# twesterhout/distributed-matvec

Measured on AMD Instinct MI355X. Metric: matvecs/sec, higher is better.
Workload: dtype f64; 1 GPU; heisenberg_chain_32: y <- H x, 601080390 basis states, 9927521280 off-diagonal non-zeros, f64 vectors, sigma/x/y resident in HBM; partitions=1, partitioning=single, exchange=none, kernel=direct-pull+staged, x=u(hash(sigma, 42)) - 0.5, exchange_bytes_per_matvec=0

## Files before the change

distributed-matvec_amd/csrc/host.c:

```c
#define _GNU_SOURCE
#include <math.h>
#include <pthread.h>
#include <stdarg.h>
#include <stdio.h>
#include <stdlib.h>
#include <string.h>

#include "../../include/ls_amd.h"
#include "../../include/ls_chpl.h"
#include "../../include/ls_hs.h"
#include "lsk.h"

static __thread char g_last_error[1024] = "";
static ls_amd_error_handler g_handler = NULL;

static int set_error(char const *fmt, ...) {
    va_list ap;
    va_start(ap, fmt);
    vsnprintf(g_last_error, sizeof(g_last_error), fmt, ap);
    va_end(ap);
    return -1;
}
static int dev_error(void) { return set_error("%s", lsk_last_error()); }
int ls_amd_internal_error(char const *fmt, ...) {
// ... 1427 lines not shown
        DEV(lsk_malloc(&p, sizeof(lsk_group) * (e->n_groups > 0 ? e->n_groups : 1)));
        DEV(lsk_h2d(p, e->groups, sizeof(lsk_group) * e->n_groups));
        e->d_groups = (lsk_group *)p;
        DEV(lsk_malloc(&p, sizeof(lsk_term) * (e->n_off > 0 ? e->n_off : 1)));
        DEV(lsk_h2d(p, e->off, sizeof(lsk_term) * e->n_off));
        e->d_off = (lsk_term *)p;
        DEV(lsk_malloc(&p, sizeof(lsk_term) * (e->n_diag > 0 ? e->n_diag : 1)));
        DEV(lsk_h2d(p, e->diag, sizeof(lsk_term) * e->n_diag));
        e->d_diag = (lsk_term *)p;
    }
    out->n_diag = e->n_diag;
    out->n_off = e->n_off;
    out->n_groups = e->n_groups;
    out->is_real = e->is_real;
    out->diag = e->d_diag;
    out->off = e->d_off;
    out->groups = e->d_groups;
    out->runs = e->runs;
    out->uni = e->is_real && e->n_groups > 0;
    out->uni_v = e->n_groups > 0 ? e->groups[0].v_re : 0.0;
    for (int g = 0; g < e->n_groups && out->uni; ++g)
        if (e->groups[g].fast != LSK_GROUP_EXCHANGE || e->groups[g].v_im != 0.0 || e->groups[g].v_re != out->uni_v ||
            __builtin_popcountll(e->groups[g].x) != 2)
            out->uni = 0;
    return 0;
}

static int operator_device(ls_hs_operator const *op, lsk_operator *out) {
    pthread_mutex_lock(&g_device_tables_lock);
    int const rc = operator_device_unlocked(op, out);
    pthread_mutex_unlock(&g_device_tables_lock);
    return rc;
}
static int basis_device(ls_hs_basis const *b, lsk_basis *out) {
    pthread_mutex_lock(&g_device_tables_lock);
    int const rc = basis_device_unlocked(b, out);
    pthread_mutex_unlock(&g_device_tables_lock);
    return rc;
}

static ls_chpl_kernels g_kernels;
void ls_hs_internal_set_chpl_kernels(ls_chpl_kernels const *kernels) { g_kernels = *kernels; }
ls_chpl_kernels const *ls_hs_internal_get_chpl_kernels(void) { return &g_kernels; }

void ls_chpl_init_kernels(void) {
    ls_chpl_kernels k;
    k.enumerate_states = (void *)ls_chpl_enumerate_representatives;
    k.operator_apply_off_diag = (void *)ls_chpl_operator_apply_off_diag;
    k.operator_apply_diag = (void *)ls_chpl_operator_apply_diag;
    k.matrix_vector_product = (void *)ls_chpl_matrix_vector_product;
    ls_hs_internal_set_chpl_kernels(&k);
}

static int g_initialised = 0;
void ls_chpl_init(void) {
    if (g_initialised) return;
    if (lsk_device_count() < 1) { halt_with("ls_chpl_init: no HIP device available"); return; }
    char const *dev = getenv("LS_AMD_DEVICE");
    if (dev && lsk_set_device(atoi(dev)) != 0) { halt_with("ls_chpl_init: %s", lsk_last_error()); return; }
    ls_chpl_init_kernels();
    g_initialised = 1;
}
void ls_chpl_finalize(void) {
    if (g_d_binom) { lsk_free(g_d_binom); g_d_binom = NULL; }
    g_initialised = 0;
}

void ls_hs_basis_build(ls_hs_basis *basis) {
    if (basis->representatives.elts) return;
    typedef void (*enum_fn)(ls_hs_basis *, uint64_t, uint64_t, chpl_external_array *);
    enum_fn f = (enum_fn)g_kernels.enumerate_states;
    if (!f) { ls_chpl_init_kernels(); f = (enum_fn)g_kernels.enumerate_states; }
    chpl_external_array arr = {NULL, 0, NULL};
    f(basis, ls_hs_min_state_estimate(basis), ls_hs_max_state_estimate(basis), &arr);
    if (!arr.elts) return;
    basis_drop_device_caches(basis);
    basis->representatives = arr;
    BEXT(basis)->owns_representatives = 1;
}

typedef struct part_state {
    int64_t count;
    uint64_t const *d_reps;
    lsk_index index;
    uint32_t *d_table;
    lsk_rankdir *d_dir;
    double *d_norms;
    int rounds;
    int64_t *send_counts;
    lsk_round_layout *d_layouts;
    int64_t max_send_bytes;
    int64_t *h_beta_off, *h_val_off;
    uint32_t *d_wtab;
    int64_t *wtab_first;
    uint32_t *d_ttab;
    int64_t *ttab_first;
    uint32_t *d_soff;
    uint32_t *h_soff;
    struct ls_amd_gtab *scatter_gt;
} part_state;

#ifndef LS_AMD_PULL_VALUES_DEFAULT
#define LS_AMD_PULL_VALUES_DEFAULT 0
#endif
enum { FAMILY_DIRECT_PUSH = 0, FAMILY_DIRECT_PULL = 1, FAMILY_TILE = 2, FAMILY_TILE_PULL = 3,
       FAMILY_REPL_DIRECT = 4, FAMILY_REPL_TILE = 5 };

struct ls_amd_plan {
    ls_hs_operator const *op;
    lsk_operator dop;
    lsk_basis dbs;
    int cplx, P, me, n_local;
    int family;
    part_state *parts;
    void *d_send;
    int64_t send_capacity;
    unsigned long long *d_cursors;
    unsigned long long *d_counts;
    int *d_err;
    int64_t nnz;
    lsk_gdir gd;
    lsk_rankdir *d_gdir;
    lsk_part_ctx *d_part_ctx;
    int part_ctx_any;
    int key_bytes;
    int streams, st_S, st_tile_rows, st_wpb, st_rounds;
    int stream_gkeys;
    void **d_send_parts;
    lsk_wsrc *d_wsrcs;
    lsk_index gindex;
    uint32_t *d_gtable;
    int64_t *d_row_gidx;
    double *d_norms_global;
    lsk_tilemap tilemap;
    void *d_tilemap;
    int has_pairs;
    int has_push_staged;
    int one_rank_full_basis;
    lsk_pairplan pairs;
    void *d_pair_recs, *d_rank_low, *d_pair_binom, *d_states32, *d_pair_rows, *d_pair_sites;
    int global_index;
    int has_hubbard;
    lsk_hubbard hubbard;
    void *d_hub[6];
    int has_chain;
    int chain_cached;
    void *d_chain_cache;
    int chain_wide;
    uint64_t *d_chain_rec;
    void *d_chain_wave;
    int chain_row_bytes;
    int chain_headed;
    int chain_headers_apply;
    int chain_paired;
    void *d_tilemap_pair, *d_chain_hdr_b;
    lsk_tilemap tilemap_pair;
    int64_t chain_pair_d, chain_pair_a0, chain_pair_rows;
    double chain_v[2];
    int64_t chain_row0;
    void *d_htab;
    uint32_t *d_slot_of;
    int htab_bits;
    void *d_xs;
    int pull_halo;
    int idx_mode;
    struct ls_amd_gtab *gtab;
    uint64_t *d_vtab;
    int64_t row_g0;
    lsk_pullbuf pbuf;
    int64_t split_rows;
    int64_t split_active;
    int slot_cache, slot_cache_valid;
    int64_t slot_cache_bytes;
    lsk_pullbuf blk_pbuf;
    int64_t blk_rows;
    lsk_tilemap blk_tilemap;
    void *d_blk_tilemap;
    void *d_blk_cols;
    void *d_gram_work;
    size_t gram_work_bytes;
    void *d_series_work;
    int series_cols;
    double *d_series_dots;
    void const *y_checked[2];
    int leaves_basis;
    int t_capacity, t_count;
    void **t_start, **t_stop;
    int st_capacity, st_count;
    void **st_start, **st_stop;
    unsigned char *st_stage;
    double st_ms[8];
    int64_t st_calls[8];
    int64_t st_matvecs;
};

typedef struct ls_amd_gtab {
    uint64_t const *reps;
    uint8_t const *masks;
    int64_t n;
    int P, L;
    lsk_gtab tab;
    uint64_t *d_entries;
    uint32_t *d_perm;
    int64_t counts[LSK_MAX_PARTS], max_count;
    uint64_t finger[8];
    int refs;
    struct ls_amd_gtab *next;
} ls_amd_gtab;
static ls_amd_gtab *g_gtabs = NULL;
static lsk_gtab no_gtab(void) { lsk_gtab t; memset(&t, 0, sizeof(t)); return t; }
static pthread_mutex_t g_gtab_lock = PTHREAD_MUTEX_INITIALIZER;

static void gtab_free(ls_amd_gtab *t) {
    if (t->d_entries) lsk_free(t->d_entries);
    if (t->d_perm) lsk_free(t->d_perm);
    free(t);
}
void ls_amd_internal_gtab_release(ls_amd_gtab *t) {
    if (!t) return;
    pthread_mutex_lock(&g_gtab_lock);
    if (--t->refs == 0) {
        for (ls_amd_gtab **q = &g_gtabs; *q; q = &(*q)->next)
            if (*q == t) { *q = t->next; break; }
        gtab_free(t);
    }
    pthread_mutex_unlock(&g_gtab_lock);
}
static int gtab_build(ls_amd_gtab *t, void *stream) {
    int64_t const n = t->n;
    int const P = t->P;
    if (t->masks) {
        DEV(lsk_mask_counts(n, t->masks, P, t->counts, stream));
        for (int p = 0; p < P; ++p) if (t->counts[p] > t->max_count) t->max_count = t->counts[p];
        if ((int64_t)P * t->max_count >= 0xffffffffLL) return set_error("indexed pull: more than 2^32 - 1 slots");
        void *pos[LSK_MAX_PARTS];
        memset(pos, 0, sizeof(pos));
        void *perm64 = NULL, *perm32 = NULL;
        int rc = lsk_malloc(&perm64, 8 * (size_t)(n > 0 ? n : 1));
        for (int p = 0; p < P && rc == 0; ++p) {
            rc = lsk_malloc(&pos[p], 8 * (size_t)(t->counts[p] > 0 ? t->counts[p] : 1));
            if (rc == 0) rc = lsk_iota_i64(t->counts[p], (int64_t)p * t->max_count, (int64_t *)pos[p], stream);
        }
        if (rc == 0) rc = lsk_hashed_to_block(n, t->masks, P, 8, (void const *const *)pos, perm64, stream);
        if (rc == 0) rc = lsk_malloc(&perm32, 4 * (size_t)(n > 0 ? n : 1));
        if (rc == 0) rc = lsk_narrow_i32(n, (int64_t const *)perm64, (int32_t *)perm32, stream);
        if (rc == 0) rc = lsk_sync(stream);
        for (int p = 0; p < P; ++p) if (pos[p]) lsk_free(pos[p]);
        if (perm64) lsk_free(perm64);
        if (rc != 0) { if (perm32) lsk_free(perm32); return dev_error(); }
        t->d_perm = (uint32_t *)perm32;
    } else {
        t->counts[0] = n;
        t->max_count = n;
    }
    int64_t const max_bytes = (int64_t)1 << 40;
    int const bb = lsk_gtab_bits(t->L, n, max_bytes);
    if (bb < 0) return set_error("indexed pull: no admissible index-table size for %lld keys of %d bits", (long long)n, t->L);
    t->tab.L = t->L; t->tab.bbits = bb; t->tab.tbits = t->L - bb;
    void *p, *flag;
    DEV(lsk_malloc(&p, (size_t)16 << bb));
    t->d_entries = (uint64_t *)p;
    t->tab.entries = t->d_entries;
    DEV(lsk_malloc(&flag, sizeof(int)));
    int zero = 0, bad = 0;
    int rc = lsk_h2d(flag, &zero, sizeof(int)) || lsk_gtab_build(t->tab, t->d_entries, n, t->reps, t->d_perm, (int *)flag, stream) ||
             lsk_sync(stream) || lsk_d2h(&bad, flag, sizeof(int));
    lsk_free(flag);
    if (rc) return dev_error();
    if (bad) return set_error("indexed pull: a key could not be placed within 255 buckets of its home");
    return 0;
}
static int gtab_fingerprint(uint64_t const *d_reps, int64_t n, void *stream, uint64_t *f) {
    memset(f, 0, 8 * sizeof(uint64_t));
    if (n <= 0) return 0;
    DEV(lsk_sync(stream));
    for (int k = 0; k < 8; ++k) DEV(lsk_d2h(&f[k], d_reps + (n - 1) * k / 7, sizeof(uint64_t)));
    return 0;
}
int ls_amd_internal_gtab_acquire(ls_amd_gtab **out, int L, uint64_t const *d_reps, int64_t n, uint8_t const *d_masks, int P,
                                 void *stream) {
    *out = NULL;
    uint64_t finger[8];
    if (gtab_fingerprint(d_reps, n, stream, finger) != 0) return -1;
    pthread_mutex_lock(&g_gtab_lock);
    for (ls_amd_gtab *t = g_gtabs; t; t = t->next)
        if (t->reps == d_reps && t->n == n && t->masks == d_masks && t->P == P && t->L == L && memcmp(t->finger, finger, sizeof(finger)) == 0) {
            ++t->refs;
            pthread_mutex_unlock(&g_gtab_lock);
            *out = t;
            return 0;
        }
    ls_amd_gtab *t = (ls_amd_gtab *)calloc(1, sizeof(*t));
    t->reps = d_reps; t->n = n; t->masks = d_masks; t->P = P; t->L = L;
    memcpy(t->finger, finger, sizeof(finger));
    if (gtab_build(t, stream) != 0) {
        gtab_free(t);
        pthread_mutex_unlock(&g_gtab_lock);
        return -1;
    }
    t->refs = 1;
    t->next = g_gtabs;
    g_gtabs = t;
    pthread_mutex_unlock(&g_gtab_lock);
    *out = t;
    return 0;
}
uint32_t const *ls_amd_internal_gtab_perm(ls_amd_gtab const *t) { return t->d_perm; }
int64_t ls_amd_internal_gtab_max_count(ls_amd_gtab const *t) { return t->max_count; }
int64_t const *ls_amd_internal_gtab_counts(ls_amd_gtab const *t) { return t->counts; }
int64_t ls_amd_internal_gtab_bytes(ls_amd_gtab const *t) { return (int64_t)16 << t->tab.bbits; }
// ... 179 lines not shown
            pl->pbuf.slots = (uint32_t *)a; pl->pbuf.rows = (uint8_t *)b; pl->pbuf.coefs = (double *)c; pl->pbuf.counts = (uint32_t *)d;
            pl->pbuf.cap = cap;
            pl->pbuf.row0 = 0;
            pl->split_rows = streams * 64 < pl->parts[0].count ? streams * 64 : pl->parts[0].count;
            return pl->split_rows;
        }
        if (a) lsk_free(a);
        if (b) lsk_free(b);
        if (c) lsk_free(c);
        if (d) lsk_free(d);
        streams = (streams / 2) & ~(int64_t)3;
    }
    return 0;
}
int64_t ls_amd_internal_plan_split_rows(ls_amd_plan const *pl) { return pl->split_rows; }
static int64_t split_rows_now(ls_amd_plan const *pl) {
    if (pl->slot_cache || pl->split_active <= 0 || pl->split_active >= pl->split_rows) return pl->split_rows;
    return pl->split_active;
}
void ls_amd_internal_plan_split_set_active(ls_amd_plan *pl, int64_t rows) {
    pl->split_active = rows <= 0 ? 0 : (rows & ~(int64_t)255);
    if (rows > 0 && pl->split_active < 256) pl->split_active = 256;
}
int64_t ls_amd_internal_plan_split_active(ls_amd_plan const *pl) { return split_rows_now(pl); }
int ls_amd_internal_plan_slot_cached(ls_amd_plan const *pl) { return pl->slot_cache != 0; }
static int64_t split_enable_exact(ls_amd_plan *pl, int64_t max_bytes) {
    split_free(pl);
    part_state *ps = &pl->parts[0];
    int64_t const streams_all = (ps->count + 63) / 64;
    int const nc = lsk_pullbuf_coef_doubles(pl->dop, pl->dbs);
    int64_t const per_packet = 4 + 1 + 8 * nc;
    void *offs = NULL;
    if (lsk_malloc(&offs, 8 * (size_t)(((streams_all + 3) & ~(int64_t)3) + 1)) != 0) return 0;
    if (lsk_tile_pull_stream_offsets(pl->dop, pl->dbs, 0, ps->count, ps->d_reps, (int64_t *)offs, NULL) != 0) { lsk_free(offs); return -1; }
    int64_t streams = streams_all;
    for (;;) {
        int64_t total = 0;
        if (lsk_d2h(&total, (char *)offs + 8 * (size_t)streams, 8) != 0) { lsk_free(offs); return -1; }
        if (max_bytes > 0 && total * per_packet + 12 * streams + 8 > max_bytes) {
            int64_t lo = 0, hi = streams / 4;
            while (hi - lo > 1) {
                int64_t const mid = lo + (hi - lo) / 2;
                int64_t t = 0;
                if (lsk_d2h(&t, (char *)offs + 8 * (size_t)(4 * mid), 8) != 0) { lsk_free(offs); return -1; }
                if (t * per_packet + 12 * 4 * mid + 8 <= max_bytes) lo = mid; else hi = mid;
            }
            streams = 4 * lo;
            if (streams <= 0) { lsk_free(offs); return 0; }
            if (lsk_d2h(&total, (char *)offs + 8 * (size_t)streams, 8) != 0) { lsk_free(offs); return -1; }
        }
        if (total >= ((int64_t)1 << 40)) { lsk_free(offs); return 0; }
        void *a = NULL, *b = NULL, *c = NULL, *d = NULL;
        if (lsk_malloc(&a, (size_t)(4 * total + 4)) == 0 && lsk_malloc(&b, (size_t)(total + 4)) == 0 &&
            (nc == 0 || lsk_malloc(&c, (size_t)(8 * nc * total + 8)) == 0) && lsk_malloc(&d, (size_t)(4 * ((streams + 3) & ~(int64_t)3))) == 0) {
            pl->pbuf.slots = (uint32_t *)a; pl->pbuf.rows = (uint8_t *)b; pl->pbuf.coefs = (double *)c; pl->pbuf.counts = (uint32_t *)d;
            pl->pbuf.offs = (int64_t const *)offs;
            pl->pbuf.cap = lsk_pullbuf_cap(pl->dop);
            pl->pbuf.row0 = 0;
            pl->split_rows = streams * 64 < ps->count ? streams * 64 : ps->count;
            pl->slot_cache_bytes = total * per_packet + 12 * streams + 8;
            return pl->split_rows;
        }
        if (a) lsk_free(a);
        if (b) lsk_free(b);
        if (c) lsk_free(c);
        if (d) lsk_free(d);
        max_bytes = (total * per_packet + 12 * streams + 8) / 4 * 3;
        if (max_bytes < ((int64_t)1 << 20)) { lsk_free(offs); return 0; }
    }
}
int64_t ls_amd_plan_cache_slots(ls_amd_plan *pl, int64_t max_bytes) {
    if (!pl || !pl->idx_mode || pl->dbs.proj != LSK_PROJ_FULL || pl->parts[0].count <= 0 ||
        (pl->family != FAMILY_TILE_PULL && pl->family != FAMILY_REPL_TILE)) return 0;
    int64_t const rows = split_enable_exact(pl, max_bytes);
    if (rows < 0) return dev_error();
    if (rows == 0) return 0;
    pl->slot_cache = 1;
    pl->slot_cache_valid = 0;
    return rows;
}
int ls_amd_plan_slot_cache_rows(ls_amd_plan const *pl, int64_t *rows, int64_t *bytes) {
    if (rows) *rows = pl->slot_cache ? pl->split_rows : 0;
    if (bytes) *bytes = pl->slot_cache ? pl->slot_cache_bytes : 0;
    return 0;
}

static int packets_wave_rings(void) {
    char const *e = getenv("LS_AMD_PACKETS");
    return !(e && strcmp(e, "block") == 0);
}
static int64_t rows_per_round_default(void) {
    char const *e = getenv("LS_AMD_ROWS_PER_ROUND");
    if (e) { long long v = atoll(e); if (v > 0) return (int64_t)v; }
    return (int64_t)1 << 24;
}

static int build_search_index(part_state *ps, int number_sites, void *stream) {
    if (ps->count >= 0xffffffffLL) return set_error("partitions with >= 2^32 states are not supported");
    int bits = 0;
    while ((1LL << (bits + 1)) <= ps->count) ++bits;
    bits -= 3;
    if (bits < 1) bits = 1;
    if (bits > 26) bits = 26;
    if (bits > number_sites) bits = number_sites;
    int shift = number_sites - bits;
    int64_t nbuckets = (int64_t)1 << bits;
    void *p;
    DEV(lsk_malloc(&p, 4 * (size_t)(nbuckets + 2)));
    ps->d_table = (uint32_t *)p;
    DEV(lsk_build_table(ps->count, ps->d_reps, shift, nbuckets, ps->d_table, stream));
    ps->index.kind = LSK_INDEX_SEARCH;
    ps->index.shift = shift;
    ps->index.table = ps->d_table;
    return 0;
}

static int upload(void **slot, void const *host, size_t bytes) {
    DEV(lsk_malloc(slot, bytes ? bytes : 8));
    DEV(lsk_h2d(*slot, host, bytes));
    return 0;
}

typedef struct { uint64_t *e; int64_t n, cap; } tile_list;
static void tile_push(tile_list *l, int64_t row, int64_t cnt) {
    if (l->n == l->cap) { l->cap = l->cap ? 2 * l->cap : 1024; l->e = (uint64_t *)realloc(l->e, sizeof(uint64_t) * (size_t)l->cap); }
    l->e[l->n++] = (uint64_t)row | ((uint64_t)cnt << 48);
}
static int tilemap_host(int64_t n, int TILE, int64_t chunk, uint64_t **out, int64_t *slots_out) {
    tile_list lists[8];
    memset(lists, 0, sizeof(lists));
    int64_t const tiles = (n + TILE - 1) / TILE;
    if (chunk > 0) {
        for (int64_t q = 0; q < tiles; ++q)
            tile_push(&lists[(q / chunk) % 8], q * TILE, n - q * TILE < TILE ? n - q * TILE : TILE);
    } else
        for (int k = 0; k < 8; ++k)
            for (int64_t q = tiles * k / 8; q < tiles * (k + 1) / 8; ++q)
                tile_push(&lists[k], q * TILE, n - q * TILE < TILE ? n - q * TILE : TILE);
    int64_t slots = 0, total = 0;
    for (int k = 0; k < 8; ++k) if (lists[k].n > slots) slots = lists[k].n;
    uint64_t *flat = (uint64_t *)calloc((size_t)(8 * slots > 0 ? 8 * slots : 1), sizeof(uint64_t));
    for (int k = 0; k < 8; ++k) {
        for (int64_t q = 0; q < lists[k].n; ++q) { flat[k * slots + q] = lists[k].e[q]; total += (int64_t)(lists[k].e[q] >> 48); }
        free(lists[k].e);
    }
    if (total != n) {
        free(flat);
        return set_error("internal error: tile map covers %lld of %lld rows", (long long)total, (long long)n);
    }
    *out = flat;
    *slots_out = slots;
    return 0;
}
static int chain_pair_range(int L, int k, int64_t *a0, int64_t *a1, int64_t *d) {
    if (L < 14 || L > 32 || k < 1 || k > L - 1) return 0;
    uint64_t C[33][33];
    memset(C, 0, sizeof(C));
    for (int n = 0; n <= 32; ++n) { C[n][0] = 1; for (int j = 1; j <= n; ++j) C[n][j] = C[n - 1][j - 1] + (j <= n - 1 ? C[n - 1][j] : 0); }
    int64_t const r01 = (int64_t)C[L - 2][k], r10 = (int64_t)C[L - 1][k];
    *d = r10 - r01;
    *a0 = (r01 + 511) & ~(int64_t)511;
    *a1 = r10 & ~(int64_t)511;
    return *a1 > *a0;
}
#define CHAIN_TILE_PLAIN 0x8000
static int tilemap_deal(tile_list const *all, int64_t chunk, uint64_t **out, int64_t *slots_out) {
    int64_t const tiles = all->n;
    int64_t per[8] = {0, 0, 0, 0, 0, 0, 0, 0}, slots = 0;
    if (chunk > 0) for (int64_t q = 0; q < tiles; ++q) ++per[(q / chunk) % 8];
    else for (int k = 0; k < 8; ++k) per[k] = tiles * (k + 1) / 8 - tiles * k / 8;
    for (int k = 0; k < 8; ++k) if (per[k] > slots) slots = per[k];
    uint64_t *flat = (uint64_t *)calloc((size_t)(8 * slots > 0 ? 8 * slots : 1), sizeof(uint64_t));
    if (!flat) return set_error("out of memory");
    int64_t fill[8] = {0, 0, 0, 0, 0, 0, 0, 0};
    int k0 = 0;
    for (int64_t q = 0; q < tiles; ++q) {
        int k;
        if (chunk > 0) k = (int)((q / chunk) % 8);
        else { while (q >= tiles * (k0 + 1) / 8) ++k0; k = k0; }
        flat[k * slots + fill[k]++] = all->e[q];
    }
    *out = flat;
    *slots_out = slots;
    return 0;
}
static int tilemap_paired_host(int64_t n, int TILE, int64_t chunk, int64_t a0, int64_t a1, int64_t d, uint64_t **rest, int64_t *rest_slots,
                               uint64_t **pairs, int64_t *pair_slots) {
    tile_list all[2];
    memset(all, 0, sizeof(all));
    int64_t const piece[3][2] = {{0, a0}, {a1, a0 + d}, {a1 + d, n}};
    int64_t total = 0;
    for (int p = 0; p < 3; ++p)
        for (int64_t pos = piece[p][0]; pos < piece[p][1];) {
            int64_t end = (pos / TILE + 1) * TILE;
            if (pos & 63) end = (pos | 63) + 1;
            if (end > piece[p][1]) end = piece[p][1];
            int const plain = (pos & 63) != 0 || ((end & 63) != 0 && end != n);
            tile_push(&all[0], pos, (end - pos) | (plain ? CHAIN_TILE_PLAIN : 0));
            total += end - pos;
            pos = end;
        }
    for (int64_t i0 = a0; i0 < a1; i0 += 512) { tile_push(&all[1], i0, 1024); total += 1024; }
    int rc = total == n ? 0 : set_error("internal error: paired tile maps cover %lld of %lld rows", (long long)total, (long long)n);
    *rest = *pairs = NULL;
    if (!rc) rc = tilemap_deal(&all[0], chunk, rest, rest_slots);
    if (!rc) rc = tilemap_deal(&all[1], chunk, pairs, pair_slots);
    if (rc) { free(*rest); free(*pairs); *rest = *pairs = NULL; }
    free(all[0].e);
    free(all[1].e);
    return rc;
}
static int build_tilemap(ls_amd_plan *pl, int64_t n, int TILE) {
    uint64_t *flat = NULL;
    int64_t slots = 0;
    char const *e = getenv("LS_AMD_TILE_CHUNK");
    int64_t const chunk = e ? atoll(e) : (TILE >= 512 ? 256 : 0);
    if (tilemap_host(n, TILE, chunk > 0 ? chunk : 0, &flat, &slots) < 0) return -1;
    int const up = upload(&pl->d_tilemap, flat, sizeof(uint64_t) * (size_t)(8 * slots > 0 ? 8 * slots : 1));
    free(flat);
    if (up) return -1;
    pl->tilemap.entries = (uint64_t const *)pl->d_tilemap;
    pl->tilemap.slots_per_xcd = slots;
    return 0;
}
int ls_amd_test_corrupt_plan(ls_amd_plan *pl) {
    if (!pl) return 0;
    if (pl->family == FAMILY_TILE_PULL && pl->n_local == 1 && pl->parts[0].d_norms && pl->parts[0].count > 0) {
        double v = 0;
        double *p = pl->parts[0].d_norms + pl->parts[0].count / 2;
        if (lsk_device_sync() != 0 || lsk_d2h(&v, p, sizeof(v)) != 0) return 0;
        v *= 2.0;
        return lsk_h2d(p, &v, sizeof(v)) == 0;
    }
    if (!pl->d_tilemap || pl->tilemap.slots_per_xcd <= 0) return 0;
    uint64_t e = 0;
    if (lsk_device_sync() != 0 || lsk_d2h(&e, pl->d_tilemap, sizeof(e)) != 0) return 0;
    uint64_t const rows = e >> 48;
    if (rows < 2) return 0;
    e = (e & 0xffffffffffffULL) | ((rows - 1) << 48);
    if (lsk_h2d(pl->d_tilemap, &e, sizeof(e)) != 0) return 0;
    return 1;
}
int ls_amd_test_window_find(uint64_t const *reps, int n, uint64_t key) { return lsk_test_window_find(reps, n, key); }
int ls_amd_test_nw_find(uint64_t const *reps, int n, uint64_t key) { return lsk_test_nw_find(reps, n, key); }
int ls_amd_test_chain_near_table(int elem, int ldsp, int16_t *out) { return lsk_test_chain_near_table(elem, ldsp, out); }
uint64_t ls_amd_test_rep_trivial_dihedral(uint64_t a, int L, int inv, int reflect) { return lsk_test_rep_trivial_dihedral(a, L, inv, reflect); }
int ls_amd_bench_k4(int L, int inv, int reflect, int variant, int64_t n, uint64_t const *d_reps, uint64_t *d_out, void *stream) {
    if (lsk_bench_k4(L, inv, reflect, variant, n, d_reps, d_out, stream) != 0) { set_error("%s", lsk_last_error()); return -1; }
    return 0;
}
int64_t ls_amd_test_tilemap(int64_t n, int tile_rows, int64_t chunk, uint64_t **entries) {
    int64_t slots = 0;
    *entries = NULL;
    if (tilemap_host(n, tile_rows, chunk, entries, &slots) < 0) return -1;
    return slots;
}
int ls_amd_test_tilemap_paired(int L, int weight, int tile_rows, int64_t chunk, uint64_t **rest, uint64_t **pairs, int64_t *out) {
    int64_t a0, a1, d, n = 1;
    *rest = *pairs = NULL;
    if (!chain_pair_range(L, weight, &a0, &a1, &d)) return 0;
    for (int j = 1; j <= weight; ++j) n = n * (L - weight + j) / j;
    if (tilemap_paired_host(n, tile_rows, chunk, a0, a1, d, rest, &out[4], pairs, &out[5]) != 0) return -1;
    out[0] = n; out[1] = a0; out[2] = a1; out[3] = d;
    return 1;
}
void ls_amd_test_free(void *p) { free(p); }
int ls_amd_test_gtab_bits(int L, int64_t n) { return lsk_gtab_bits(L, n, (int64_t)1 << 40); }
int ls_amd_test_gtab_build(int L, int bbits, int64_t n, uint64_t const *reps, uint32_t const *payload, uint64_t **entries) {
    lsk_gtab t;
    t.entries = NULL; t.L = L; t.bbits = bbits; t.tbits = L - bbits;
    *entries = (uint64_t *)malloc(sizeof(uint64_t) * ((size_t)2 << bbits));
    if (lsk_test_gtab_build_host(t, *entries, n, reps, payload) != 0) { free(*entries); *entries = NULL; return -1; }
    return 0;
}
int64_t ls_amd_test_gtab_find(int L, int bbits, uint64_t const *entries, uint64_t key) {
    lsk_gtab t;
    t.entries = NULL; t.L = L; t.bbits = bbits; t.tbits = L - bbits;
    return lsk_test_gtab_find(t, entries, key);
}

static int push_staged_eligible(ls_amd_plan const *pl) {
    ls_hs_operator const *op = pl->op;
    struct ls_amd_operator_ext const *ext = OEXT(op);
    char const *e = getenv("LS_AMD_ROW_KERNEL");
    if (e && strcmp(e, "generic") == 0) return 0;
    if (NBITS(op->basis) > 64 || op->basis->spin_inversion != 0 || pl->dbs.proj != LSK_PROJ_NONE || !ext->is_real ||
        ext->runs.n_runs <= 0 || BEXT(op->basis)->hamming_weight < 0)
        return 0;
    for (int q = 0; q < ext->runs.n_runs; ++q) if (ext->runs.cnt[q] >> 16) return 0;
    return 1;
}
static int chain_eligible(ls_amd_plan const *pl) {
    ls_hs_operator const *op = pl->op;
    struct ls_amd_operator_ext const *ext = OEXT(op);
    char const *e = getenv("LS_AMD_ROW_KERNEL");
    if (e && (strcmp(e, "generic") == 0 || strcmp(e, "pairs") == 0 || strcmp(e, "pairrows") == 0 || strcmp(e, "pairsites") == 0)) return 0;
    int const L = NBITS(op->basis);
    int const inv = op->basis->spin_inversion != 0;
    if (inv && (pl->dbs.proj != LSK_PROJ_INVERSION || pl->family != FAMILY_DIRECT_PULL || (L & 1) || BEXT(op->basis)->hamming_weight != L / 2)) return 0;
    if (L > 64 || (!inv && pl->dbs.proj != LSK_PROJ_NONE) ||
        !ext->is_real || !ext->is_hermitian || ext->runs.n_runs <= 0 || ext->n_diag <= 0)
        return 0;
    int extra = 0;
    if (inv) for (int q = 0; q < ext->runs.n_runs; ++q) if (ext->runs.lo0[q] + ext->runs.cnt[q] - 1 == L - 2) extra = 1;
    if (ext->n_groups - ext->runs.n_run_groups + extra > 2) return 0;
    for (int g = ext->runs.n_run_groups; g < ext->n_groups; ++g) {
        lsk_group const *G = &ext->groups[g];
        if (G->fast != LSK_GROUP_EXCHANGE || G->v_im != 0.0 || __builtin_popcountll(G->x) != 2) return 0;
    }
    return 1;
}
static void chain_wave_tables(int low_site, uint16_t *U, uint16_t *Rg, int *class_off) {
    int pos[13];
    uint16_t rank_in[4096];
    memset(class_off, 0, sizeof(int) * 14);
    for (int w = 0; w < 4096; ++w) ++class_off[__builtin_popcount(w) + 1];
    for (int k = 0; k < 13; ++k) { class_off[k + 1] += class_off[k]; pos[k] = class_off[k]; }
    for (int w = 0; w < 4096; ++w) {
        int const k = __builtin_popcount(w);
        rank_in[w] = (uint16_t)(pos[k] - class_off[k]);
        U[pos[k]++] = (uint16_t)w;
    }
    for (int w = 0; w < 4096; ++w) Rg[w] = low_site >= 0 ? rank_in[w ^ (1 << low_site)] : 0;
}
int ls_amd_test_chain_wave_tables(int low_site, uint16_t *U, uint16_t *Rg, int *class_off) {
    if (low_site >= 12) return set_error("ls_amd_test_chain_wave_tables: the low site lies below bit 12");
    chain_wave_tables(low_site, U, Rg, class_off);
    return 0;
}
static int setup_chain_headers(ls_amd_plan *pl, lsk_index index, int64_t n, uint64_t const *d_reps, int nc, uint64_t xmask, void *stream) {
    int const L = NBITS(pl->op->basis);
    char const *e = getenv("LS_AMD_CHAIN_RECORDS");
    int headed = L >= 13 && L <= 32 && pl->dbs.proj == LSK_PROJ_NONE && pl->chain_row0 == 0 &&
                 pl->family == FAMILY_DIRECT_PULL && pl->dbs.hamming_weight >= 0 && nc <= 1;
    int lo = -1, hi = -1;
    if (headed && nc == 1) {
        lo = __builtin_ctzll(xmask);
        hi = 63 - __builtin_clzll(xmask);
        if (lo >= 12 || hi < 12) { headed = 0; lo = hi = -1; }
    }
    pl->chain_headers_apply = headed;
    if (e && atoi(e) != 0) { headed = 0; lo = hi = -1; }
    int const words = lsk_chain_words();
    int64_t const n_hdr = (n + 63) / 64;
    uint16_t U[4096], Rg[4096];
    int class_off[14];
    uint32_t *tab = (uint32_t *)malloc(sizeof(uint32_t) * (size_t)words);
    if (!tab) return set_error("out of memory");
    chain_wave_tables(headed ? lo : -1, U, Rg, class_off);
    for (int t = 0; t < words; ++t) tab[t] = (uint32_t)U[t] | ((uint32_t)Rg[U[t]] << 16) | (lo >= 0 ? (((uint32_t)U[t] >> lo) & 1u) << 31 : 0u);
    size_t const tab_bytes = sizeof(uint32_t) * (size_t)words, hdr_bytes = 8 * (size_t)n_hdr;
    void *q;
    if (lsk_malloc(&q, tab_bytes + hdr_bytes + 8) != 0) { free(tab); return 1; }
    unsigned long long plain = 0;
    unsigned long long *d_plain = (unsigned long long *)((char *)q + tab_bytes + hdr_bytes);
    int const rc = lsk_h2d(q, tab, tab_bytes) || lsk_h2d(d_plain, &plain, 8) ||
                   lsk_chain_headers(pl->dbs, index, n, d_reps, headed, hi, (char *)q + tab_bytes, d_plain, stream) || lsk_sync(stream) ||
                   lsk_d2h(&plain, d_plain, 8);
    free(tab);
    if (rc) { lsk_free(q); return dev_error(); }
    pl->d_chain_wave = q;
    pl->chain_headed = headed;
    int const rec = pl->cplx ? 4 + 4 * nc : 8;
    pl->chain_row_bytes = headed ? (int)((8 * (uint64_t)n_hdr + 64 * (uint64_t)rec * (uint64_t)plain + (uint64_t)n - 1) / (uint64_t)n) : rec;
    return 0;
}
static int setup_chain_pairs(ls_amd_plan *pl, lsk_index index, int64_t n, uint64_t const *d_reps, int hi, void *stream) {
    char const *e = getenv("LS_AMD_CHAIN_PAIRED");
    int const L = NBITS(pl->op->basis);
    if ((e && atoi(e) == 0) || !pl->chain_headers_apply || pl->cplx || !pl->d_chain_rec || pl->chain_cached > 1 || pl->chain_row0 != 0 ||
        pl->n_local != 1 || pl->family != FAMILY_DIRECT_PULL)
        return 0;
    int top = 0;
    for (int q = 0; q < pl->dop.runs.n_runs; ++q)
        if (pl->dop.runs.lo0[q] <= L - 2 && L - 2 < pl->dop.runs.lo0[q] + pl->dop.runs.cnt[q]) top = 1;
    int64_t a0, a1, d;
    if (!top || !chain_pair_range(L, pl->dbs.hamming_weight, &a0, &a1, &d) || a1 + d > n) return 0;
    uint64_t *rest = NULL, *pairs = NULL;
    int64_t rest_slots = 0, pair_slots = 0;
    char const *ce = getenv("LS_AMD_TILE_CHUNK");
    int64_t const chunk = ce ? atoll(ce) : 256;
    if (tilemap_paired_host(n, lsk_chain_tile_rows(0), chunk > 0 ? chunk : 0, a0, a1, d, &rest, &rest_slots, &pairs, &pair_slots) != 0) return -1;
    void *d_rest = NULL, *d_pairs = NULL, *d_hdr = NULL;
    int64_t const n_b = a1 - a0;
    unsigned long long plain = 0;
    int rc = lsk_malloc(&d_rest, sizeof(uint64_t) * (size_t)(8 * rest_slots > 0 ? 8 * rest_slots : 1)) ||
             lsk_malloc(&d_pairs, sizeof(uint64_t) * (size_t)(8 * pair_slots)) || lsk_malloc(&d_hdr, 8 * (size_t)(n_b / 64) + 8);
    if (!rc) {
        unsigned long long *d_plain = (unsigned long long *)((char *)d_hdr + 8 * (size_t)(n_b / 64));
        rc = lsk_h2d(d_rest, rest, sizeof(uint64_t) * (size_t)(8 * rest_slots)) || lsk_h2d(d_pairs, pairs, sizeof(uint64_t) * (size_t)(8 * pair_slots)) ||
             lsk_h2d(d_plain, &plain, 8) || lsk_chain_headers(pl->dbs, index, n_b, d_reps + a0 + d, pl->chain_headed, hi, d_hdr, d_plain, stream) ||
             lsk_sync(stream);
        if (rc) { free(rest); free(pairs); lsk_free(d_rest); lsk_free(d_pairs); lsk_free(d_hdr); return dev_error(); }
    }
    free(rest);
    free(pairs);
    if (rc) {
        if (d_rest) lsk_free(d_rest);
        if (d_pairs) lsk_free(d_pairs);
        if (d_hdr) lsk_free(d_hdr);
        return 0;
    }
    lsk_free(pl->d_tilemap);
    pl->d_tilemap = d_rest;
    pl->tilemap.entries = (uint64_t const *)d_rest;
    pl->tilemap.slots_per_xcd = rest_slots;
    pl->d_tilemap_pair = d_pairs;
    pl->tilemap_pair.entries = (uint64_t const *)d_pairs;
    pl->tilemap_pair.slots_per_xcd = pair_slots;
    pl->d_chain_hdr_b = d_hdr;
    pl->chain_pair_d = d;
    pl->chain_pair_a0 = a0;
    pl->chain_pair_rows = 2 * (a1 - a0);
    pl->chain_paired = 1;
    return 0;
}
static int setup_chain(ls_amd_plan *pl, lsk_index index, int64_t n, uint64_t const *d_reps, void *stream) {
    struct ls_amd_operator_ext const *ext = OEXT(pl->op);
    int nc = ext->n_groups - ext->runs.n_run_groups;
    int const Ls = NBITS(pl->op->basis);
    int const inv = pl->dbs.proj == LSK_PROJ_INVERSION;
    uint64_t const top = 1ULL << (Ls - 1);
    uint64_t cx[3];
    double cv[3];
    int k = 0;
    if (inv)
        for (int q = 0; q < pl->dop.runs.n_runs; ++q)
            if (pl->dop.runs.lo0[q] + pl->dop.runs.cnt[q] - 1 == Ls - 2) {
                cx[k] = 3ULL << (Ls - 2);
                cv[k++] = pl->dop.runs.v_re[q] * (double)pl->op->basis->spin_inversion;
                if (--pl->dop.runs.cnt[q] == 0) {
                    for (int r = q; r + 1 < pl->dop.runs.n_runs; ++r) {
                        pl->dop.runs.lo0[r] = pl->dop.runs.lo0[r + 1]; pl->dop.runs.cnt[r] = pl->dop.runs.cnt[r + 1];
                        pl->dop.runs.v_re[r] = pl->dop.runs.v_re[r + 1]; pl->dop.runs.v_im[r] = pl->dop.runs.v_im[r + 1];
                    }
                    --pl->dop.runs.n_runs;
                }
                break;
            }
    for (int g = ext->runs.n_run_groups; g < ext->n_groups && k < 3; ++g) {
        cx[k] = ext->groups[g].x;
        cv[k++] = ext->groups[g].v_re * ((inv && (ext->groups[g].x & top)) ? (double)pl->op->basis->spin_inversion : 1.0);
    }
    nc = k;
    if (nc > 2) return 0;
    char const *ew = getenv("LS_AMD_CHAIN_WIDE");
    pl->chain_wide = index.count >= 0xffffffffLL || (ew && atoi(ew) != 0 && NBITS(pl->op->basis) > 32);
    size_t const es = pl->chain_wide ? sizeof(uint64_t) : sizeof(uint32_t);
    if (nc > 0 && n > 0) {
        void *q;
        if (lsk_malloc(&q, es * (size_t)nc * (size_t)n) != 0) return 0;
        pl->d_chain_cache = q;
        int zero = 0, flag = 0;
        DEV(lsk_h2d(pl->d_err, &zero, sizeof(int)));
        for (int c = 0; c < nc; ++c)
            DEV(lsk_chain_cache(pl->dbs, index, n, d_reps, cx[c],
                                (char *)pl->d_chain_cache + es * (size_t)c * (size_t)n, pl->chain_wide, pl->d_err, stream));
        DEV(lsk_sync(stream));
        DEV(lsk_d2h(&flag, pl->d_err, sizeof(int)));
        DEV(lsk_h2d(pl->d_err, &zero, sizeof(int)));
        if (flag) {
            lsk_free(pl->d_chain_cache);
            pl->d_chain_cache = NULL;
            return 0;
        }
        pl->chain_cached = nc;
        pl->chain_v[0] = cv[0];
        pl->chain_v[1] = nc > 1 ? cv[1] : 0.0;
    }
    if (build_tilemap(pl, n, lsk_chain_tile_rows(pl->cplx)) != 0) return -1;
    if (!pl->cplx && NBITS(pl->op->basis) <= 32 && !pl->chain_wide && n > 0) {
        void *q;
        if (lsk_malloc(&q, sizeof(uint64_t) * (size_t)n) != 0) {
            if (pl->d_chain_cache) { lsk_free(pl->d_chain_cache); pl->d_chain_cache = NULL; }
            if (pl->d_tilemap) { lsk_free(pl->d_tilemap); pl->d_tilemap = NULL; memset(&pl->tilemap, 0, sizeof(pl->tilemap)); }
            pl->chain_cached = 0;
            return 0;
        }
        pl->d_chain_rec = (uint64_t *)q;
        DEV(lsk_chain_pack(n, d_reps, pl->chain_cached ? pl->d_chain_cache : NULL, (uint64_t *)q, stream));
        DEV(lsk_sync(stream));
        if (pl->chain_cached <= 1 && pl->d_chain_cache) { lsk_free(pl->d_chain_cache); pl->d_chain_cache = NULL; }
    }
    if (NBITS(pl->op->basis) <= 32 && !pl->chain_wide && n > 0) {
        int const rc = setup_chain_headers(pl, index, n, d_reps, pl->chain_cached, pl->chain_cached > 0 ? cx[0] : 0, stream);
        if (rc < 0) return -1;
        if (rc > 0) {
            if (pl->d_chain_rec) { lsk_free(pl->d_chain_rec); pl->d_chain_rec = NULL; }
            if (pl->d_chain_cache) { lsk_free(pl->d_chain_cache); pl->d_chain_cache = NULL; }
            if (pl->d_tilemap) { lsk_free(pl->d_tilemap); pl->d_tilemap = NULL; memset(&pl->tilemap, 0, sizeof(pl->tilemap)); }
            pl->chain_cached = 0;
            return 0;
        }
        if (setup_chain_pairs(pl, index, n, d_reps, pl->chain_cached > 0 ? 63 - __builtin_clzll(cx[0]) : -1, stream) != 0) return -1;
    }
    pl->has_chain = 1;
    return 0;
}

static int pair_cmp(void const *pa, void const *pb) {
    lsk_pair const *a = (lsk_pair const *)pa, *b = (lsk_pair const *)pb;
    int const ca = a->j < 11 ? 0 : (a->i < 11 ? 1 : 2), cb = b->j < 11 ? 0 : (b->i < 11 ? 1 : 2);
    if (ca != cb) return ca - cb;
    if (a->i != b->i) return (int)a->i - (int)b->i;
    return (int)a->j - (int)b->j;
}
static int setup_pairs(ls_amd_plan *pl, int64_t n, uint64_t const *d_reps, void *stream) {
    ls_hs_operator const *op = pl->op;
    struct ls_amd_operator_ext const *ext = OEXT(op);
    int const L = NBITS(op->basis), hw = BEXT(op->basis)->hamming_weight;
    char const *e = getenv("LS_AMD_ROW_KERNEL");
    if (e && strcmp(e, "generic") == 0) return 0;
    int const wide = L > 32;
    if (L > 64 || hw < 0 || hw + 2 > LSK_PAIR_KC || op->basis->spin_inversion != 0 || pl->dbs.proj != LSK_PROJ_NONE || !ext->is_real ||
        !ext->is_hermitian || ext->n_groups < 1 || ext->n_groups > LSK_MAX_PAIRS || n <= 0 || n >= 0xffffffffLL ||
        ext->n_diag <= 0)
        return 0;
    int const force_sites = e && strcmp(e, "pairsites") == 0;
    int const by_row = force_sites || (e && strcmp(e, "pairrows") == 0) || (!(e && strcmp(e, "pairs") == 0) && (11 * hw < 4 * L || 11 * (L - hw) < 4 * L));
    lsk_pair recs[LSK_MAX_PAIRS];
    memset(recs, 0, sizeof(recs));
    for (int g = 0; g < ext->n_groups; ++g) {
        lsk_group const *G = &ext->groups[g];
        if (G->fast != LSK_GROUP_EXCHANGE || G->v_im != 0.0 || __builtin_popcountll(G->x) != 2) return 0;
        recs[g].i = (uint8_t)__builtin_ctzll(G->x);
        recs[g].j = (uint8_t)(63 - __builtin_clzll(G->x));
        recs[g].v = G->v_re;
    }
    double dsum = 0.0;
    for (int t = 0; t < ext->n_diag; ++t) {
        lsk_term const *T = &ext->diag[t];
        if (T->m != 0 || T->r != 0 || T->v_im != 0.0) return 0;
        int g = 0;
        while (g < ext->n_groups && ext->groups[g].x != T->s) ++g;
        if (g == ext->n_groups) return 0;
        recs[g].vz += T->v_re;
        dsum += T->v_re;
    }
    qsort(recs, (size_t)ext->n_groups, sizeof(lsk_pair), pair_cmp);
    lsk_pairplan pp;
    memset(&pp, 0, sizeof(pp));
    for (int g = 0; g < ext->n_groups; ++g) {
        if (recs[g].j < 11) ++pp.n_near; else if (recs[g].i < 11) ++pp.n_str; else ++pp.n_high;
    }
    pp.dsum = dsum;
    uint16_t rank_low[2048];
    for (int w = 0; w < 2048; ++w) {
        uint64_t r = 0;
        int k = 0;
        for (int b = 0; b < 11; ++b) if ((w >> b) & 1) r += binom(b, ++k);
        rank_low[w] = (uint16_t)r;
    }
    int const nbits = wide ? 64 : 32;
    uint32_t bin[64 * LSK_PAIR_KC];
    for (int a = 0; a < nbits; ++a) for (int k = 0; k < LSK_PAIR_KC; ++k) bin[a * LSK_PAIR_KC + k] = (uint32_t)binom(a, k);
    void *q = NULL;
    if (!wide) {
        if (lsk_malloc(&q, 4 * (size_t)n) != 0) return 0;
        pl->d_states32 = q;
    }
    if (upload(&pl->d_pair_recs, recs, sizeof(lsk_pair) * (size_t)ext->n_groups) != 0 || upload(&pl->d_rank_low, rank_low, sizeof(rank_low)) != 0 ||
        upload(&pl->d_pair_binom, bin, sizeof(uint32_t) * (size_t)nbits * LSK_PAIR_KC) != 0)
        return -1;
    if (!wide) DEV(lsk_narrow_states(n, d_reps, (uint32_t *)pl->d_states32, stream));
    if (by_row) {
        lsk_pair_row rr[LSK_MAX_PAIRS];
// ... 922 lines not shown
    *d_norms = NULL;
    if (basis_device(op->basis, &dbs) != 0) return -1;
    int64_t const cnt = gt->counts[me];
    void *reps = NULL, *nrm = NULL;
    if (lsk_malloc(&reps, 8 * (size_t)(cnt > 0 ? cnt : 1)) != 0) return dev_error();
    if (lsk_malloc(&nrm, 8 * (size_t)(cnt > 0 ? cnt : 1)) != 0) { lsk_free(reps); return dev_error(); }
    int const rc = lsk_scatter_owned(gt->n, gt->d_perm, (int64_t)me * gt->max_count, cnt, gt->reps, (uint64_t *)reps, stream) ||
                   lsk_norms(dbs, cnt, (uint64_t const *)reps, (double *)nrm, stream) || lsk_sync(stream);
    lsk_free(reps);
    if (rc) { lsk_free(nrm); return dev_error(); }
    *d_norms = (double *)nrm;
    return 0;
}

int ls_amd_matvec_replicated(ls_amd_plan *pl, void const *d_x_global, void *d_y_local, void *stream) {
    part_state *ps = &pl->parts[0];
    int slot;
    ls_amd_internal_count_matvec(pl);
    if (pl->family == FAMILY_REPL_DIRECT) {
        int const st = stage_begin(pl, ST_ROWS, stream);
        slot = timing_begin(pl, stream);
        if (pl->has_chain)
            DEV(lsk_chain(pl->dop, pl->dbs, pl->gindex, pl->cplx, pl->chain_wide, pl->d_chain_rec != NULL, pl->tilemap, ps->count,
                          pl->d_chain_rec ? pl->d_chain_rec : ps->d_reps, pl->chain_row0, pl->gindex.count, d_x_global, d_y_local,
                          pl->chain_cached, pl->d_chain_cache, pl->chain_v[0], pl->chain_v[1], pl->d_chain_wave, stream));
        else
            DEV(lsk_direct_gx(pl->dop, pl->dbs, pl->gindex, pl->cplx, pl->tilemap, ps->d_reps, pl->d_row_gidx, d_x_global,
                          d_y_local, pl->d_err, stream));
        timing_end(pl, slot, stream);
        stage_end(pl, st, stream);
        return 0;
    }
    if (pl->family == FAMILY_REPL_TILE && pl->idx_mode) {
        lsk_pullidx ix;
        ix.tab = pl->gtab->tab;
        ix.perm = pl->gtab->d_perm;
        ix.row_g0 = pl->row_g0;
        ix.vtab = NULL;
        int const st = stage_begin(pl, ST_ROWS, stream);
        slot = timing_begin(pl, stream);
        DEV(lsk_tile_pull_idx(pl->dop, pl->dbs, pl->cplx, 0, ps->count, ps->d_reps, ps->d_norms, ix, pl->gindex.reps,
                              pl->gindex.count, d_x_global, pl->pull_halo, d_y_local, pl->d_err, stream));
        timing_end(pl, slot, stream);
        stage_end(pl, st, stream);
        return 0;
    }
    if (pl->family == FAMILY_REPL_TILE) {
        void const *xg;
        if (prescaled_x(pl, pl->gindex.count, pl->gindex.reps, d_x_global, pl->d_norms_global, &xg, stream) != 0) return -1;
        int const st = stage_begin(pl, ST_ROWS, stream);
        slot = timing_begin(pl, stream);
        DEV(lsk_tile_pull(pl->dop, pl->dbs, pl->gindex, pl->cplx, 0, ps->count, ps->d_reps, ps->d_norms,
                          pl->d_norms_global, pl->d_row_gidx, xg, pl->htab_bits, pl->gindex.reps, pl->gindex.count,
                          pl->d_xs ? pl->d_xs : d_x_global, pl->pull_halo, d_x_global, d_y_local, pl->d_err, stream));
        timing_end(pl, slot, stream);
        stage_end(pl, st, stream);
        return 0;
    }
    return set_error("ls_amd_matvec_replicated: not a replicated-x plan");
}
int ls_amd_internal_plan_reach(ls_amd_plan *pl, int shift, int64_t row0, int64_t halo, int64_t nwords, uint32_t *h_bitmap, void *stream) {
    if (pl->family != FAMILY_REPL_DIRECT || pl->dbs.proj != LSK_PROJ_NONE) return 1;
    part_state *ps = &pl->parts[0];
    int64_t const n_global = pl->gindex.count;
    if (((n_global - 1) >> shift) / 32 >= nwords) return set_error("internal error: reach bitmap too small");
    memset(h_bitmap, 0, 4 * (size_t)nwords);
    if (ps->count <= 0) return 0;
    void *d = NULL;
    DEV(lsk_malloc(&d, 4 * (size_t)nwords));
    if (lsk_memset_async(d, 0, 4 * (size_t)nwords, stream) != 0 ||
        lsk_reach_blocks(pl->dop, pl->gindex, ps->count, ps->d_reps, shift, (uint32_t *)d, stream) != 0 || lsk_sync(stream) != 0 ||
        lsk_d2h(h_bitmap, d, 4 * (size_t)nwords) != 0) { lsk_free(d); return dev_error(); }
    lsk_free(d);
    int64_t g0 = row0, g1 = g0 + ps->count;
    g0 = g0 > halo ? g0 - halo : 0;
    g1 = g1 + halo < n_global ? g1 + halo : n_global;
    for (int64_t b = g0 >> shift; b <= (g1 - 1) >> shift; ++b) h_bitmap[b >> 5] |= 1u << (b & 31);
    return 0;
}

int ls_amd_internal_repl_split_begin(ls_amd_plan *pl, void *stream) {
    if (pl->family != FAMILY_REPL_TILE || !pl->idx_mode || pl->split_rows <= 0) return 0;
    if (pl->slot_cache && pl->slot_cache_valid) return 0;
    part_state *ps = &pl->parts[0];
    lsk_pullidx ix;
    ix.tab = pl->gtab->tab;
    ix.perm = pl->gtab->d_perm;
    ix.row_g0 = pl->row_g0;
    ix.vtab = NULL;
    int const st = stage_begin(pl, ST_GENERATE, stream);
    int const slot = timing_begin(pl, stream);
    DEV(lsk_tile_pull_resolve(pl->dop, pl->dbs, 0, split_rows_now(pl), ps->d_reps, ps->d_norms, ix, pl->gindex.reps, pl->gindex.count,
                              pl->pull_halo, pl->pbuf, pl->d_err, stream));
    pl->slot_cache_valid = pl->slot_cache;
    timing_end(pl, slot, stream);
    stage_end(pl, st, stream);
    return 0;
}
int ls_amd_internal_repl_split_rows(ls_amd_plan *pl, void const *d_x_global, void *d_y_local, int64_t row0, int64_t row1, int count, void *stream) {
    if (pl->family != FAMILY_REPL_TILE || !pl->idx_mode || pl->split_rows <= 0) return set_error("internal error: not a split plan");
    part_state *ps = &pl->parts[0];
    if (row1 > ps->count) row1 = ps->count;
    if (row0 < 0 || (row0 & 255) != 0 || row0 > row1) return set_error("internal error: bad row range of the split matvec");
    if (count) ls_amd_internal_count_matvec(pl);
    lsk_pullidx ix;
    ix.tab = pl->gtab->tab;
    ix.perm = pl->gtab->d_perm;
    ix.row_g0 = pl->row_g0;
    ix.vtab = NULL;
    int64_t const S = split_rows_now(pl);
    int const st = stage_begin(pl, ST_ROWS, stream);
    if (row0 < S) {
        int const slot = pl->slot_cache ? timing_begin(pl, stream) : -1;
        DEV(lsk_tile_pull_gather(pl->dop, pl->dbs, pl->cplx, row0, row1 < S ? row1 : S, ps->d_reps, ps->d_norms, ix, d_x_global, pl->pbuf, d_y_local,
                                 stream));
        if (slot >= 0) timing_end(pl, slot, stream);
    }
    if (row1 > S)
        DEV(lsk_tile_pull_idx(pl->dop, pl->dbs, pl->cplx, row0 > S ? row0 : S, row1, ps->d_reps, ps->d_norms, ix, pl->gindex.reps,
                              pl->gindex.count, d_x_global, pl->pull_halo, d_y_local, pl->d_err, stream));
    stage_end(pl, st, stream);
    return 0;
}
int ls_amd_internal_repl_split_finish(ls_amd_plan *pl, void const *d_x_global, void *d_y_local, void *stream) {
    if (pl->family != FAMILY_REPL_TILE || !pl->idx_mode || pl->split_rows <= 0) return ls_amd_matvec_replicated(pl, d_x_global, d_y_local, stream);
    return ls_amd_internal_repl_split_rows(pl, d_x_global, d_y_local, 0, pl->parts[0].count, 1, stream);
}
char const *ls_amd_plan_kernel_name(ls_amd_plan const *pl) {
    switch (pl->family) {
    case FAMILY_DIRECT_PUSH: return pl->has_push_staged ? "direct-push+staged" : "direct-push";
    case FAMILY_DIRECT_PULL:
        if (pl->has_hubbard) return "direct-pull+hubbard";
        return pl->has_chain ? "direct-pull+staged" : pl->has_pairs ? (pl->pairs.sites ? "direct-pull+pairsites" : pl->pairs.rows ? "direct-pull+pairrows" : "direct-pull+pairs") : "direct-pull";
    case FAMILY_TILE_PULL: return pl->idx_mode ? (pl->slot_cache ? "tile-pull+indexed+cached" : (pl->d_vtab ? "tile-pull+values" : "tile-pull+indexed")) : "tile-pull";
    case FAMILY_REPL_DIRECT:
        return pl->has_chain ? "replicated-direct-pull+staged" : "replicated-direct-pull";
    case FAMILY_REPL_TILE: return pl->idx_mode ? (pl->slot_cache ? "replicated-tile-pull+indexed+cached" : "replicated-tile-pull+indexed") : "replicated-tile-pull";
    default: return pl->streams ? "tile+streams" : (pl->has_push_staged ? "tile(one rank: push+staged)" : "tile");
    }
}
int ls_amd_plan_packet_bytes(ls_amd_plan const *pl) { return pl->key_bytes + (pl->cplx ? 16 : 8); }
int ls_amd_plan_row_bytes(ls_amd_plan const *pl) {
    if (pl->has_hubbard) return 0;
    if (pl->has_pairs) return pl->pairs.wide ? 8 : 4;
    if (pl->has_chain) {
        if (pl->d_chain_wave) return pl->chain_row_bytes;
        int const narrow = NBITS(pl->op->basis) <= 32 && !pl->chain_wide;
        return (narrow ? 4 : 8) + pl->chain_cached * (pl->chain_wide ? 8 : 4);
    }
    if (pl->family == FAMILY_TILE_PULL || pl->family == FAMILY_REPL_TILE) return 16;
    return 8;
}
int64_t ls_amd_plan_chain_paired_rows(ls_amd_plan const *pl) {
    return pl->has_chain && pl->chain_paired ? pl->chain_pair_rows : 0;
}
int64_t ls_amd_plan_nnz(ls_amd_plan const *pl) { return pl->nnz; }
int ls_amd_plan_send_counts(ls_amd_plan const *pl, int round, int64_t *counts) {
    if (pl->family != FAMILY_TILE) { for (int d = 0; d < pl->P; ++d) counts[d] = 0; return 0; }
    part_state const *ps = &pl->parts[0];
    if (round < 0 || round >= ps->rounds) return set_error("round out of range");
    memcpy(counts, ps->send_counts + (size_t)round * pl->P, sizeof(int64_t) * pl->P);
    return 0;
}

static int prescaled_x(ls_amd_plan *pl, int64_t n, uint64_t const *d_reps, void const *d_x, double const *d_norms,
                       void const **out, void *stream) {
    if (!pl->d_htab) {
        int bits = 4;
        while (((int64_t)1 << bits) < 2 * n) ++bits;
        if (bits > 32) return set_error("hash index: more than 2^31 representatives per table are not supported");
        pl->htab_bits = bits;
        DEV(lsk_malloc(&pl->d_htab, (size_t)(pl->cplx ? 32 : 16) << bits));
        void *p;
        DEV(lsk_malloc(&p, 4 * (size_t)(n > 0 ? n : 1)));
        pl->d_slot_of = (uint32_t *)p;
        DEV(lsk_hash_build(pl->cplx, n, d_reps, bits, pl->d_htab, pl->d_slot_of, stream));
        pl->pull_halo = pull_halo_setting(0);
        if (pl->pull_halo > 0 && pl->dbs.k4_mode != 0) DEV(lsk_malloc(&pl->d_xs, (size_t)(pl->cplx ? 16 : 8) * (size_t)(n > 0 ? n : 1)));
    }
    int const st = stage_begin(pl, ST_REFRESH, stream);
    DEV(lsk_hash_fill(pl->cplx, n, pl->d_slot_of, d_x, pl->dbs.k4_mode != 0 ? d_norms : NULL, pl->d_htab, pl->d_xs, stream));
    stage_end(pl, st, stream);
    *out = pl->d_htab;
    return 0;
}

int ls_amd_diag(ls_amd_plan *pl, void const *d_x, void *d_y, void *stream) {
    part_state *ps = &pl->parts[0];
    int const st = stage_begin(pl, ST_DIAG, stream);
    if (pl->has_push_staged) {
        if (pl->dop.n_diag > 0) DEV(lsk_memset_async(d_y, 0, (size_t)ps->count * (pl->cplx ? 16 : 8), stream));
    } else
    DEV(lsk_diag(pl->dop, pl->cplx, ps->count, ps->d_reps, d_x, d_y, stream));
    stage_end(pl, st, stream);
    return 0;
}

static int generate_round(ls_amd_plan *pl, part_state *ps, int pid, int round, void const *d_x, void *d_y,
                          void *d_send, void *stream) {
    int64_t row0 = ps->count * round / ps->rounds, row1 = ps->count * (round + 1) / ps->rounds;
    if (pl->P > 1 && !ps->d_wtab) DEV(lsk_memset_async(pl->d_cursors, 0, 8 * (size_t)pl->P, stream));
    int const st = stage_begin(pl, ST_GENERATE, stream);
    int slot = timing_begin(pl, stream);
    if (pl->has_push_staged) {
        lsk_index cix = ps->index;
        cix.kind = LSK_INDEX_COMBINADIC;
        DEV(lsk_push_staged(pl->dop, pl->dbs, cix, pl->cplx, pl->tilemap, ps->count, ps->d_reps, d_x, d_y, pl->d_err, stream));
    } else if (pl->streams) {
        uint64_t const *d_binom;
        if (device_binom(&d_binom) != 0) return -1;
        DEV(lsk_tile_st(pl->dop, pl->gd, d_binom, pl->cplx, 0, pl->P, pl->st_S, pl->st_tile_rows, row0, row1, ps->d_reps, d_x,
                        ps->d_ttab + (size_t)ps->ttab_first[round] * (size_t)(pl->P * pl->st_S), ps->d_layouts + round, d_send, pl->d_err, stream));
    } else if (ps->d_wtab)
        DEV(lsk_tile_wv(pl->dop, pl->dbs, ps->index, pl->gd, pl->cplx, 0, pl->P, pid, row0, row1, ps->d_reps, ps->d_norms, d_x, d_y,
                        ps->d_wtab + (size_t)ps->wtab_first[round] * pl->P, ps->d_layouts + round, d_send, pl->d_err,
                        ps->scatter_gt ? ps->scatter_gt->tab : no_gtab(), stream));
    else
        DEV(lsk_tile(pl->dop, pl->dbs, ps->index, pl->cplx, 0, pl->P, pid, row0, row1, ps->d_reps, ps->d_norms, d_x,
                     d_y, pl->d_cursors, ps->d_layouts + round, d_send, pl->d_counts, pl->d_err, stream));
    timing_end(pl, slot, stream);
    stage_end(pl, st, stream);
    return 0;
}

int ls_amd_generate(ls_amd_plan *pl, int round, void const *d_x, void *d_y, void *d_send, void *stream) {
    if (pl->family != FAMILY_TILE) return set_error("ls_amd_generate: the plan uses a direct kernel (P == 1)");
    if (pl->me < 0) return set_error("ls_amd_generate: plan owns all partitions; use ls_amd_matvec");
    part_state *ps = &pl->parts[0];
    if (round < 0 || round >= ps->rounds) return set_error("round out of range");
    return generate_round(pl, ps, pl->me, round, d_x, d_y, d_send, stream);
}

int ls_amd_scatter(ls_amd_plan *pl, int64_t n, uint64_t const *d_betas, void const *d_values, void *d_y,
                   void *stream) {
    part_state *ps = &pl->parts[0];
    if (pl->streams) return set_error("ls_amd_scatter: the plan writes sorted streams (consumed by windows, dist.c)");
    if (ps->index.kind == LSK_INDEX_COMBINADIC || ps->index.kind == LSK_INDEX_PRODUCT) return set_error("ls_amd_scatter: plan has no search index");
    int const st = stage_begin(pl, ST_SCATTER, stream);
    if (pl->key_bytes == 4) {
        lsk_segs sg;
        memset(&sg, 0, sizeof(sg));
        sg.n = 1; sg.start[0] = 0; sg.start[1] = n; sg.key_off[0] = 0;
        sg.val_off[0] = (int64_t)((char const *)d_values - (char const *)d_betas);
        sg.y[0] = d_y;
        DEV(lsk_scatter_idx(pl->cplx, &sg, d_betas, stream));
    } else
        DEV(lsk_scatter(ps->index, pl->cplx, n, d_betas, d_values, d_y, pl->dbs.k4_mode ? ps->d_norms : NULL, pl->d_err,
                        stream));
    stage_end(pl, st, stream);
    return 0;
}
int ls_amd_scatter_round(ls_amd_plan *pl, int num_segments, int64_t const *counts, int64_t const *offsets, void const *d_recv,
                         void *d_y, void *stream) {
    part_state *ps = &pl->parts[0];
    if (pl->streams) return set_error("ls_amd_scatter_round: the plan writes sorted streams (consumed by windows, dist.c)");
    if (ps->index.kind == LSK_INDEX_COMBINADIC || ps->index.kind == LSK_INDEX_PRODUCT) return set_error("ls_amd_scatter_round: plan has no search index");
    int const st = stage_begin(pl, ST_SCATTER, stream);
    int s = 0;
    while (s < num_segments) {
        lsk_segs sg;
        memset(&sg, 0, sizeof(sg));
        int64_t total = 0;
        for (; s < num_segments && sg.n < LSK_MAX_SEGS; ++s) {
            if (counts[s] <= 0) continue;
            sg.start[sg.n] = total;
            sg.key_off[sg.n] = offsets[s];
            sg.val_off[sg.n] = offsets[s] + segment_key_bytes(pl, counts[s]);
            sg.y[sg.n] = d_y;
            total += counts[s];
            ++sg.n;
        }
        if (sg.n == 0) break;
        sg.start[sg.n] = total;
        if (pl->key_bytes == 4) DEV(lsk_scatter_idx(pl->cplx, &sg, d_recv, stream));
        else {
            DEV(lsk_scatter_segs(ps->index, ps->scatter_gt ? ps->scatter_gt->tab : no_gtab(), pl->cplx, &sg, d_recv, pl->dbs.k4_mode ? ps->d_norms : NULL, pl->d_err, stream));
        }
    }
    stage_end(pl, st, stream);
    return 0;
}
int ls_amd_internal_plan_streams(ls_amd_plan const *pl) { return pl->streams ? pl->st_S : 0; }
uint32_t const *ls_amd_internal_plan_stream_offsets(ls_amd_plan const *pl) { return pl->streams ? pl->parts[0].h_soff : NULL; }
int ls_amd_internal_window_round(ls_amd_plan *pl, lsk_wsrc const *d_srcs, int n_src, void *d_y, void *stream) {
    if (!pl->streams || pl->me < 0) return set_error("ls_amd_internal_window_round: not a streams plan of one partition");
    lsk_wdests wd;
    memset(&wd, 0, sizeof(wd));
    int const W = lsk_window_rows(pl->cplx);
    int64_t const windows = (pl->parts[0].count + W - 1) / W;
    wd.n = 1;
    wd.count[0] = pl->parts[0].count;
    wd.y[0] = d_y;
    wd.first_block[1] = (windows + pl->st_wpb - 1) / pl->st_wpb;
    if (pl->stream_gkeys) {
        uint64_t const *d_binom;
        if (device_binom(&d_binom) != 0) return -1;
        wd.dir[0] = pl->parts[0].index.dir; wd.reps[0] = pl->parts[0].d_reps;
        wd.binom = d_binom; wd.n_ranks = pl->gd.n_ranks; wd.weight = pl->gd.weight; wd.err = pl->d_err;
    }
    int const st = stage_begin(pl, ST_SCATTER, stream);
    DEV(lsk_window(pl->cplx, &wd, d_srcs, n_src, pl->st_S, pl->st_wpb, stream));
    stage_end(pl, st, stream);
    return 0;
}
int ls_amd_plan_key_bytes(ls_amd_plan const *pl) { return pl->key_bytes; }
int64_t ls_amd_plan_segment_bytes(ls_amd_plan const *pl, int64_t count) { return segment_key_bytes(pl, count) + (pl->cplx ? 16 : 8) * count; }
int64_t ls_amd_plan_segment_value_offset(ls_amd_plan const *pl, int64_t count) { return segment_key_bytes(pl, count); }
int64_t ls_amd_plan_packet_index_bytes(ls_amd_plan const *pl) {
    return pl->d_gdir ? (int64_t)sizeof(lsk_rankdir) * ((pl->gd.n_ranks + 63) / 64) * pl->gd.P : 0;
}

int ls_amd_matvec(ls_amd_plan *pl, void const *const *d_x, void *const *d_y, void *stream) {
    if (pl->me >= 0) return set_error("ls_amd_matvec: plan owns one partition; drive it with generate/scatter");
    for (int p = 0; p < pl->n_local; ++p) if (ls_amd_internal_check_y(pl, d_y[p]) != 0) return -1;
    ls_amd_internal_count_matvec(pl);
    if (pl->family == FAMILY_TILE_PULL && pl->idx_mode) {
        part_state *ps = &pl->parts[0];
        void const *xs = d_x[0];
        if (pl->dbs.k4_mode != 0) {
            int const sr = stage_begin(pl, ST_REFRESH, stream);
            DEV(lsk_scale(pl->cplx, ps->count, d_x[0], ps->d_norms, pl->d_xs, stream));
            stage_end(pl, sr, stream);
            xs = pl->d_xs;
        }
        lsk_pullidx ix;
        ix.tab = pl->gtab->tab;
        ix.perm = NULL;
        ix.row_g0 = 0;
        ix.vtab = NULL;
        if (pl->d_vtab && (pl->slot_cache || pl->split_rows > 0)) { lsk_free(pl->d_vtab); pl->d_vtab = NULL; }
        if (pl->split_rows > 0 && pl->slot_cache) {
            lsk_pullbuf const pb = pl->pbuf;
            int st, slot;
            if (!pl->slot_cache_valid) {
                st = stage_begin(pl, ST_GENERATE, stream);
                slot = timing_begin(pl, stream);
                DEV(lsk_tile_pull_resolve(pl->dop, pl->dbs, 0, pl->split_rows, ps->d_reps, ps->d_norms, ix, ps->d_reps, ps->count, pl->pull_halo, pb,
                                          pl->d_err, stream));
                timing_end(pl, slot, stream);
                stage_end(pl, st, stream);
                pl->slot_cache_valid = 1;
            }
            st = stage_begin(pl, ST_ROWS, stream);
            slot = timing_begin(pl, stream);
            DEV(lsk_tile_pull_gather(pl->dop, pl->dbs, pl->cplx, 0, pl->split_rows, ps->d_reps, ps->d_norms, ix, xs, pb, d_y[0], stream));
            timing_end(pl, slot, stream);
            if (pl->split_rows < ps->count) {
                slot = timing_begin(pl, stream);
                DEV(lsk_tile_pull_idx(pl->dop, pl->dbs, pl->cplx, pl->split_rows, ps->count, ps->d_reps, ps->d_norms, ix, ps->d_reps, ps->count, xs,
                                      pl->pull_halo, d_y[0], pl->d_err, stream));
                timing_end(pl, slot, stream);
            }
            stage_end(pl, st, stream);
            return 0;
        }
        if (pl->split_rows > 0) {
            for (int64_t r0 = 0; r0 < ps->count; r0 += pl->split_rows) {
                int64_t const r1 = r0 + pl->split_rows < ps->count ? r0 + pl->split_rows : ps->count;
                lsk_pullbuf pb = pl->pbuf;
                pb.row0 = r0;
                int st = stage_begin(pl, ST_GENERATE, stream);
                int const slot = timing_begin(pl, stream);
                DEV(lsk_tile_pull_resolve(pl->dop, pl->dbs, r0, r1, ps->d_reps, ps->d_norms, ix, ps->d_reps, ps->count, pl->pull_halo, pb,
                                          pl->d_err, stream));
                timing_end(pl, slot, stream);
                stage_end(pl, st, stream);
                st = stage_begin(pl, ST_ROWS, stream);
                DEV(lsk_tile_pull_gather(pl->dop, pl->dbs, pl->cplx, r0, r1, ps->d_reps, ps->d_norms, ix, xs, pb, d_y[0], stream));
                stage_end(pl, st, stream);
            }
            return 0;
        }
        if (pl->d_vtab) {
            int const sr = stage_begin(pl, ST_REFRESH, stream);
            DEV(lsk_vtab_refresh(pl->gtab->tab, pl->d_vtab, xs, stream));
            stage_end(pl, sr, stream);
            ix.vtab = pl->d_vtab;
        }
        int const st = stage_begin(pl, ST_ROWS, stream);
        int slot = timing_begin(pl, stream);
        DEV(lsk_tile_pull_idx(pl->dop, pl->dbs, pl->cplx, 0, ps->count, ps->d_reps, ps->d_norms, ix, ps->d_reps, ps->count, xs,
                              pl->pull_halo, d_y[0], pl->d_err, stream));
        timing_end(pl, slot, stream);
        stage_end(pl, st, stream);
        return 0;
    }
    if (pl->family == FAMILY_TILE_PULL) {
        part_state *ps = &pl->parts[0];
        void const *xg;
        if (prescaled_x(pl, ps->count, ps->d_reps, d_x[0], ps->d_norms, &xg, stream) != 0) return -1;
        int const st = stage_begin(pl, ST_ROWS, stream);
        int slot = timing_begin(pl, stream);
        DEV(lsk_tile_pull(pl->dop, pl->dbs, ps->index, pl->cplx, 0, ps->count, ps->d_reps, ps->d_norms, ps->d_norms,
                          NULL, xg, pl->htab_bits, ps->d_reps, ps->count, pl->d_xs ? pl->d_xs : d_x[0], pl->pull_halo, d_x[0],
                          d_y[0], pl->d_err, stream));
        timing_end(pl, slot, stream);
        stage_end(pl, st, stream);
        return 0;
    }
    if (pl->has_push_staged) {
        if (pl->dop.n_diag > 0) {
            int const st = stage_begin(pl, ST_DIAG, stream);
            DEV(lsk_memset_async(d_y[0], 0, (size_t)pl->parts[0].count * (pl->cplx ? 16 : 8), stream));
            stage_end(pl, st, stream);
        }
    } else if (pl->family != FAMILY_DIRECT_PULL) {
        int const st = stage_begin(pl, ST_DIAG, stream);
        for (int p = 0; p < pl->n_local; ++p)
            DEV(lsk_diag(pl->dop, pl->cplx, pl->parts[p].count, pl->parts[p].d_reps, d_x[p], d_y[p], stream));
        stage_end(pl, st, stream);
    }
    if (pl->dop.n_groups == 0 && pl->family != FAMILY_DIRECT_PULL) return 0;
    if (pl->family != FAMILY_TILE) {
        part_state *ps = &pl->parts[0];
        int const st = stage_begin(pl, ST_ROWS, stream);
        int slot = timing_begin(pl, stream);
        if (pl->has_chain) {
            DEV(lsk_chain(pl->dop, pl->dbs, ps->index, pl->cplx, pl->chain_wide, pl->d_chain_rec != NULL, pl->tilemap, ps->count,
                          pl->d_chain_rec ? pl->d_chain_rec : ps->d_reps, 0, ps->count, d_x[0], d_y[0], pl->chain_cached,
                          pl->d_chain_cache, pl->chain_v[0], pl->chain_v[1], pl->d_chain_wave, stream));
            if (pl->chain_paired)
                DEV(lsk_chain_paired(pl->dop, pl->dbs, pl->tilemap_pair, ps->count, pl->d_chain_rec, d_x[0], d_y[0], pl->chain_cached, pl->chain_v[0],
                                     pl->d_chain_wave, pl->chain_pair_d, pl->chain_pair_a0, pl->d_chain_hdr_b, NBITS(pl->op->basis) - 2, stream));
        } else if (pl->has_pairs)
            DEV(lsk_pairs(pl->pairs, pl->dbs.hamming_weight, pl->cplx, pl->tilemap, ps->count, d_x[0], d_y[0], stream));
        else if (pl->has_hubbard)
            DEV(lsk_hubbard_apply(pl->hubbard, pl->dop, pl->cplx, pl->tilemap, d_x[0], d_y[0], stream));
        else if (pl->has_push_staged)
            DEV(lsk_push_staged(pl->dop, pl->dbs, ps->index, pl->cplx, pl->tilemap, ps->count, ps->d_reps, d_x[0], d_y[0], pl->d_err, stream));
        else
            DEV(lsk_direct(pl->dop, pl->dbs, ps->index, pl->cplx, pl->family == FAMILY_DIRECT_PULL ? (OEXT(pl->op)->is_hermitian ? 1 : 2) : 0, pl->tilemap, ps->d_reps,
                           d_x[0], d_y[0], pl->d_err, stream));
        timing_end(pl, slot, stream);
        stage_end(pl, st, stream);
        return 0;
    }
    int const P = pl->P;
    if (pl->streams) {
        uint64_t const *d_binom;
        if (device_binom(&d_binom) != 0) return -1;
        int const W = lsk_window_rows(pl->cplx);
        lsk_wdests wd;
        memset(&wd, 0, sizeof(wd));
        wd.n = P;
        for (int d = 0; d < P; ++d) {
            int64_t const windows = (pl->parts[d].count + W - 1) / W;
            wd.count[d] = pl->parts[d].count;
            wd.y[d] = d_y[d];
            wd.first_block[d + 1] = wd.first_block[d] + (windows + pl->st_wpb - 1) / pl->st_wpb;
            if (pl->stream_gkeys) { wd.dir[d] = pl->parts[d].index.dir; wd.reps[d] = pl->parts[d].d_reps; }
        }
        if (pl->stream_gkeys) { wd.binom = d_binom; wd.n_ranks = pl->gd.n_ranks; wd.weight = pl->gd.weight; wd.err = pl->d_err; }
        for (int r = 0; r < pl->st_rounds; ++r) {
            int st = stage_begin(pl, ST_GENERATE, stream);
            for (int p = 0; p < P; ++p) {
                part_state *ps = &pl->parts[p];
                int64_t row0 = ps->count * r / ps->rounds, row1 = ps->count * (r + 1) / ps->rounds;
                int const slot = timing_begin(pl, stream);
                DEV(lsk_tile_st(pl->dop, pl->gd, d_binom, pl->cplx, 0, P, pl->st_S, pl->st_tile_rows, row0, row1, ps->d_reps, d_x[p],
                                ps->d_ttab + (size_t)ps->ttab_first[r] * (size_t)(P * pl->st_S), ps->d_layouts + r, pl->d_send_parts[p],
                                pl->d_err, stream));
                timing_end(pl, slot, stream);
            }
            stage_end(pl, st, stream);
            st = stage_begin(pl, ST_SCATTER, stream);
            DEV(lsk_window(pl->cplx, &wd, pl->d_wsrcs + (size_t)r * P * P, P, pl->st_S, pl->st_wpb, stream));
            stage_end(pl, st, stream);
        }
        return 0;
    }
    for (int p = 0; p < P; ++p) {
        part_state *ps = &pl->parts[p];
        for (int r = 0; r < ps->rounds; ++r) {
            if (generate_round(pl, ps, p, r, d_x[p], d_y[p], pl->d_send, stream) != 0) return -1;
            if (pl->key_bytes == 4) {
                for (int d0 = 0; d0 < P; d0 += LSK_MAX_SEGS) {
                    lsk_segs sg;
                    memset(&sg, 0, sizeof(sg));
                    int64_t total = 0;
                    for (int d = d0; d < P && d < d0 + LSK_MAX_SEGS; ++d) {
                        int64_t const c = ps->send_counts[(size_t)r * P + d];
                        if (d == p || c == 0) continue;
                        sg.start[sg.n] = total;
                        sg.key_off[sg.n] = ps->h_beta_off[(size_t)r * P + d];
                        sg.val_off[sg.n] = ps->h_val_off[(size_t)r * P + d];
                        sg.y[sg.n] = d_y[d];
                        total += c;
                        ++sg.n;
                    }
                    if (sg.n == 0) continue;
                    sg.start[sg.n] = total;
                    int const st = stage_begin(pl, ST_SCATTER, stream);
                    DEV(lsk_scatter_idx(pl->cplx, &sg, pl->d_send, stream));
                    stage_end(pl, st, stream);
                }
                continue;
            }
            if (pl->d_part_ctx) {
                int mixed = 0;
                for (int d = 0; d < P; ++d) if ((pl->parts[d].index.dir != NULL) != (pl->parts[pl->part_ctx_any].index.dir != NULL) && pl->parts[d].count > 0) mixed = 1;
                if (!mixed) {
                    for (int d0 = 0; d0 < P; d0 += LSK_MAX_SEGS) {
                        lsk_segs sg;
                        memset(&sg, 0, sizeof(sg));
                        int64_t total = 0;
                        for (int d = d0; d < P && d < d0 + LSK_MAX_SEGS; ++d) {
                            int64_t const c = ps->send_counts[(size_t)r * P + d];
                            if (d == p || c == 0) continue;
                            sg.start[sg.n] = total;
                            sg.key_off[sg.n] = ps->h_beta_off[(size_t)r * P + d];
                            sg.val_off[sg.n] = ps->h_val_off[(size_t)r * P + d];
                            sg.y[sg.n] = d_y[d];
                            sg.part[sg.n] = (uint8_t)d;
                            total += c;
                            ++sg.n;
                        }
                        if (sg.n == 0) continue;
                        sg.start[sg.n] = total;
                        int const st = stage_begin(pl, ST_SCATTER, stream);
                        DEV(lsk_scatter_parts(pl->d_part_ctx, pl->parts[pl->part_ctx_any].index, pl->cplx, &sg, pl->d_send, pl->d_err, stream));
                        stage_end(pl, st, stream);
                    }
                    continue;
                }
            }
            for (int d = 0; d < P; ++d) {
                int64_t c = ps->send_counts[(size_t)r * P + d];
                if (d == p || c == 0) continue;
                uint64_t const *betas = (uint64_t const *)((char *)pl->d_send + ps->h_beta_off[(size_t)r * P + d]);
                void const *vals = (char *)pl->d_send + ps->h_val_off[(size_t)r * P + d];
                int const st = stage_begin(pl, ST_SCATTER, stream);
                DEV(lsk_scatter(pl->parts[d].index, pl->cplx, c, betas, vals, d_y[d],
                                pl->dbs.k4_mode ? pl->parts[d].d_norms : NULL, pl->d_err, stream));
                stage_end(pl, st, stream);
            }
        }
    }
    return 0;
}

enum { BLK_COLUMNS = 0, BLK_DIRECT = 1, BLK_PULL = 2 };
static char const *const g_blk_names[3] = { "columns", "k_direct_blk", "k_pull_gather_blk" };
static int block_kernel_of(ls_amd_plan const *pl) {
    if (pl->P != 1 || pl->me >= 0 || pl->n_local != 1) return BLK_COLUMNS;
    if (pl->family == FAMILY_TILE_PULL && pl->idx_mode && pl->dbs.proj == LSK_PROJ_FULL)
        return (!pl->cplx && lsk_pullbuf_coef_doubles(pl->dop, pl->dbs) == 2) ? BLK_COLUMNS : BLK_PULL;
    if (pl->family == FAMILY_DIRECT_PULL && pl->dbs.proj == LSK_PROJ_NONE && !pl->has_push_staged) return BLK_DIRECT;
    return BLK_COLUMNS;
}
static int block_path(ls_amd_plan const *pl, int K) {
    int const kern = block_kernel_of(pl);
    char const *e = getenv("LS_AMD_BLOCK");
    if (kern == BLK_COLUMNS || (e && strcmp(e, "columns") == 0)) return BLK_COLUMNS;
    if (e && strcmp(e, "kernel") == 0) return kern;
    if (K < 2) return BLK_COLUMNS;
    if (kern == BLK_DIRECT && (pl->has_chain || pl->has_pairs || pl->has_hubbard)) return BLK_COLUMNS;
    return kern;
}
char const *ls_amd_plan_block_kernel_name(ls_amd_plan const *pl, int K) {
    if (!pl) { set_error("ls_amd_plan_block_kernel_name: plan is NULL"); return NULL; }
    if (K < 1 || K > 64) { set_error("ls_amd_plan_block_kernel_name: K = %d is outside [1, 64]", K); return NULL; }
    return g_blk_names[block_path(pl, K)];
}

static int block_strides(char const *who, int64_t n, int K, int64_t r, int64_t c, char const *name) {
    int ok = r >= 0 && c >= 0;
    if (ok && K > 1 && n > 1) ok = (c >= 1 && r >= c * K) || (r >= 1 && c >= r * n);
    else if (ok && K > 1) ok = c >= 1;
    else if (ok && n > 1) ok = r >= 1;
    if (!ok)
        return set_error("%s: strides (row %lld, column %lld) of %s make two elements of the %lld x %d block share "
                         "storage (need non-negative strides with row >= K * column, or column >= N * row)", who, (long long)r,
                         (long long)c, name, (long long)n, K);
    return 0;
}
static int block_overlap(size_t wa, int64_t na, void const *a, int64_t ar, int64_t ac, size_t wb, int64_t nb, void const *b, int64_t br,
// ... 2909 lines not shown
```

distributed-matvec_amd/csrc/k_rows.hip:

```cpp
#include <hip/hip_runtime.h>
#include "lsk_dev.hpp"

template <bool CPLX>
__global__ __launch_bounds__(kBlock) void k_diag(lsk_runs runs, int n_diag, lsk_term const *__restrict__ diag,
                                                 int64_t n, uint64_t const *__restrict__ reps,
                                                 double const *__restrict__ x, double *__restrict__ y) {
    for (int64_t i = (int64_t)blockIdx.x * kBlock + threadIdx.x; i < n; i += (int64_t)gridDim.x * kBlock) {
        uint64_t a = reps[i];
        double dr, di;
        diag_coeff<uint64_t, false>(runs, n_diag, diag, a, dr, di);
        if (CPLX) {
            double xr = x[2 * i], xi = x[2 * i + 1];
            y[2 * i] = dr * xr - di * xi;
            y[2 * i + 1] = dr * xi + di * xr;
        } else {
            y[i] = dr * x[i];
        }
    }
}

extern "C" int lsk_diag(lsk_operator op, int cplx, int64_t n, uint64_t const *reps, void const *x, void *y,
                        void *stream) {
    if (n == 0 || op.n_diag == 0) return 0;
    dim3 g(grid_for(n)), b(kBlock);
// ... 393 lines not shown
    hipLaunchKernelGGL((k_direct_blk<CPLX, INDEX>), dim3((unsigned)gb), dim3(kBlock), 0, s, op.runs, op.n_groups, op.groups, op.off, op.n_diag,
                       op.diag, ix, weight, tm.entries, tm.slots_per_xcd, reps, K, (double const *)x, xr, xc, (double *)y, yr, yc, d_err);
    LSK_LAUNCH_CHECK();
    return 0;
}
extern "C" int lsk_direct_blk(lsk_operator op, lsk_basis bs, lsk_index ix, int cplx, lsk_tilemap tm, uint64_t const *reps, int K,
                              void const *x, int64_t xr, int64_t xc, void *y, int64_t yr, int64_t yc, int *d_err, void *stream) {
    if (tm.slots_per_xcd == 0 || K <= 0) return 0;
    if (!tm.entries) { snprintf(g_err, sizeof(g_err), "lsk_direct_blk: no tile map"); return -1; }
    if (bs.proj != LSK_PROJ_NONE) { snprintf(g_err, sizeof(g_err), "lsk_direct_blk: unprojected bases only"); return -1; }
    if (!cplx && !op.is_real) { snprintf(g_err, sizeof(g_err), "lsk_direct_blk: complex operators need c128 vectors"); return -1; }
    hipStream_t s = (hipStream_t)stream;
#define LSK_DB(IDX) (cplx ? launch_direct_blk<true, IDX>(op, ix, bs.hamming_weight, tm, reps, K, x, xr, xc, y, yr, yc, d_err, s) \
                          : launch_direct_blk<false, IDX>(op, ix, bs.hamming_weight, tm, reps, K, x, xr, xc, y, yr, yc, d_err, s))
    switch (ix.kind) {
    case LSK_INDEX_IDENTITY: return LSK_DB(LSK_INDEX_IDENTITY);
    case LSK_INDEX_COMBINADIC: return LSK_DB(LSK_INDEX_COMBINADIC);
    case LSK_INDEX_PRODUCT: return LSK_DB(LSK_INDEX_PRODUCT);
    default: return LSK_DB(LSK_INDEX_SEARCH);
    }
#undef LSK_DB
}
constexpr int kPushHalo = 512;
template <typename W, bool CPLX, int TILE>
__global__ __launch_bounds__(kBlock) void k_push_t(lsk_runs runs, int n_groups, lsk_group const *__restrict__ groups,
                                                   lsk_term const *__restrict__ off, int n_diag, lsk_term const *__restrict__ diag,
                                                   lsk_basis bs, lsk_index ix, uint64_t const *__restrict__ tilemap, int64_t slots_per_xcd,
                                                   int64_t n, uint64_t const *__restrict__ reps, double const *__restrict__ x,
                                                   double *__restrict__ y, int *err) {
    typedef typename WordTraits<W>::binom_t BT;
    typedef WordTraits<W> WT;
    constexpr int HALO = kPushHalo;
    constexpr int WINDOW = TILE + 2 * HALO;
    constexpr int NC = CPLX ? 2 : 1;
    __shared__ BT s_binom[64 * LSK_BINOM_K];
    __shared__ double s_y[WINDOW * NC];
    for (int k = threadIdx.x; k < 64 * LSK_BINOM_K; k += kBlock) s_binom[k] = (BT)ix.binom[k];
    const int xcd = blockIdx.x & 7;
    const int64_t blocks_per_xcd = gridDim.x >> 3;
    tilemap += (int64_t)xcd * slots_per_xcd;
    for (int64_t t = blockIdx.x >> 3; t < slots_per_xcd; t += blocks_per_xcd) {
        const uint64_t slot = tilemap[t];
        const int cnt = (int)(slot >> 48);
        if (cnt == 0) continue;
        const int64_t i0 = (int64_t)(slot & 0xffffffffffffULL);
        const int64_t w0 = i0 - HALO;
        __syncthreads();
        for (int j = threadIdx.x; j < WINDOW * NC; j += kBlock) s_y[j] = 0.0;
        __syncthreads();
#pragma unroll 1
        for (int sub = 0; sub < TILE / kBlock; ++sub) {
            const int r = sub * kBlock + threadIdx.x;
            if (r >= cnt) continue;
            const int64_t i = i0 + r;
            const int own = HALO + r;
            const W a = (W)__builtin_nontemporal_load(reps + i);
            double xr, xi = 0.0;
            if (CPLX) { xr = x[2 * i]; xi = x[2 * i + 1]; } else xr = x[i];
            auto add = [&](int64_t idx, double vr, double vi) {
                const int64_t o = idx - w0;
                if (o >= 0 && o < WINDOW) {
                    if (CPLX) { atomicAdd(&s_y[2 * o], vr); atomicAdd(&s_y[2 * o + 1], vi); } else atomicAdd(&s_y[o], vr);
                } else if (CPLX) { atomic_add_f64(y + 2 * idx, vr); atomic_add_f64(y + 2 * idx + 1, vi); }
                else atomic_add_f64(y + idx, vr);
            };
            if (n_diag > 0) {
                double dr, di;
                diag_coeff<W, true>(runs, n_diag, diag, a, dr, di);
                if (CPLX) { atomicAdd(&s_y[2 * own], dr * xr); atomicAdd(&s_y[2 * own + 1], dr * xi); } else atomicAdd(&s_y[own], dr * xr);
            }
            const W tdiff = a ^ (a >> 1);
            for (int q = 0; q < runs.n_runs; ++q) {
                const int lo0 = runs.lo0[q], rc = runs.cnt[q];
                const double v = runs.v_re[q];
                int k = WT::popc(a & (W)(((uint64_t)1 << lo0) - 1));
#pragma unroll 4
                for (int lo = lo0; lo < lo0 + rc; ++lo) {
                    const bool bit = (a >> lo) & 1;
                    const bool act = (tdiff >> lo) & 1;
                    const int64_t d = (int64_t)s_binom[lo * LSK_BINOM_K + k];
                    k += bit ? 1 : 0;
                    if (act) add(bit ? i + d : i - d, v * xr, v * xi);
                }
            }
            for (int g = runs.n_run_groups; g < n_groups; ++g) {
                lsk_group const G = groups[g];
                double cr, ci;
                group_coeff<true>(G, off, (uint64_t)a, cr, ci);
                if (cr == 0.0) continue;
                const W beta = a ^ (W)G.x;
                int64_t idx;
                if (G.adj >= 0 && WT::popc(a & (W)G.x) == 1) {
                    const int k = WT::popc(a & (W)(((uint64_t)1 << G.adj) - 1));
                    const int64_t d = (int64_t)s_binom[G.adj * LSK_BINOM_K + k];
                    idx = ((a >> G.adj) & 1) ? i + d : i - d;
                } else {
                    if (WT::popc(beta) != bs.hamming_weight) { atomicExch(err, 1); continue; }
                    idx = rank_combinadic_w<W, BT>(beta, s_binom);
                }
                add(idx, cr * xr, cr * xi);
            }
        }
        __syncthreads();
        for (int j = threadIdx.x; j < WINDOW; j += kBlock) {
            const int64_t row = w0 + j;
            if (row < 0 || row >= n) continue;
            if (CPLX) {
                const double vr = s_y[2 * j], vi = s_y[2 * j + 1];
                if (vr != 0.0) atomic_add_f64(y + 2 * row, vr);
                if (vi != 0.0) atomic_add_f64(y + 2 * row + 1, vi);
            } else {
                const double vr = s_y[j];
                if (vr != 0.0) atomic_add_f64(y + row, vr);
            }
        }
    }
}
extern "C" int lsk_push_tile_rows(int cplx) { return cplx ? 512 : 1024; }
extern "C" int lsk_push_staged(lsk_operator op, lsk_basis bs, lsk_index ix, int cplx, lsk_tilemap tm, int64_t n, uint64_t const *reps,
                               void const *x, void *y, int *d_err, void *stream) {
    if (n == 0 || tm.slots_per_xcd == 0) return 0;
    if (!tm.entries || ix.kind != LSK_INDEX_COMBINADIC || bs.proj != LSK_PROJ_NONE || !op.is_real) { snprintf(g_err, sizeof(g_err), "lsk_push_staged: plan out of range"); return -1; }
    const int64_t gb = tm.slots_per_xcd * 8;
    dim3 g((unsigned)gb), b(kBlock);
#define LSK_PT_ARGS op.runs, op.n_groups, op.groups, op.off, op.n_diag, op.diag, bs, ix, tm.entries, tm.slots_per_xcd, n, reps, (double const *)x, (double *)y, d_err
    if (bs.number_sites <= 32) {
        if (cplx) hipLaunchKernelGGL((k_push_t<uint32_t, true, 512>), g, b, 0, (hipStream_t)stream, LSK_PT_ARGS);
        else hipLaunchKernelGGL((k_push_t<uint32_t, false, 1024>), g, b, 0, (hipStream_t)stream, LSK_PT_ARGS);
    } else if (cplx) hipLaunchKernelGGL((k_push_t<uint64_t, true, 512>), g, b, 0, (hipStream_t)stream, LSK_PT_ARGS);
    else hipLaunchKernelGGL((k_push_t<uint64_t, false, 1024>), g, b, 0, (hipStream_t)stream, LSK_PT_ARGS);
#undef LSK_PT_ARGS
    LSK_LAUNCH_CHECK();
    return 0;
}

extern "C" int lsk_direct_gx(lsk_operator op, lsk_basis bs, lsk_index ix, int cplx, lsk_tilemap tm, uint64_t const *reps,
                             int64_t const *row_gidx, void const *x_global, void *y, int *d_err, void *stream) {
    return direct_dispatch(op, bs, ix, cplx, 1, tm, reps, x_global, y, d_err, stream, 1, row_gidx);
}

constexpr int kChainHalo = 512;
constexpr int kChainLdsPairs = 12;
constexpr int kChainFar = 12;
constexpr uint32_t kChainWords = 4096;

__device__ __forceinline__ double cx_load_nt(double const *p) { return __builtin_nontemporal_load(p); }
__device__ __forceinline__ double2 cx_load_nt(double2 const *p) {
    typedef double d2v __attribute__((ext_vector_type(2)));
    const d2v v = __builtin_nontemporal_load(reinterpret_cast<d2v const *>(p));
    return make_double2(v.x, v.y);
}
constexpr int kChainFarC = 6;

struct chain_pair_args { int64_t d, a0; uint32_t const *hdr_b; int bond; };
template <typename W, typename R, bool CPLX, int TILE, bool REC, bool PAIR>
__device__ __forceinline__ void chain_rows(lsk_runs const &runs, int n_diag, lsk_term const *__restrict__ diag,
                                                    int hamming_weight, uint4 const *__restrict__ g_img, int img16, int kc,
                                                    int near_off,
                                                    uint64_t const *__restrict__ tilemap, int64_t slots_per_xcd, int64_t n,
                                                    uint64_t const *__restrict__ reps, void const *__restrict__ x_v,
                                                    void *__restrict__ y_v, int n_cached,
                                                    R const *__restrict__ cache, double cv0, double cv1, int64_t row0,
                                                    int64_t n_x, uint32_t const *__restrict__ wave_plan, chain_pair_args const &pr) {
    typedef typename ChainX<CPLX>::type X;
    typedef WordTraits<W> WT;
    constexpr int NB = ChainTraits<W, R>::NB;
    constexpr int HALO = (CPLX || PAIR) ? 256 : kChainHalo;
    constexpr int LDSP = (CPLX || PAIR) ? 11 : kChainLdsPairs;
    constexpr int SEG = TILE / 2;
    constexpr int WSEG = SEG + 2 * HALO + 2;
    constexpr int WINDOW = PAIR ? 2 * WSEG : TILE + 2 * HALO + 2;
    static_assert(!PAIR || (REC && !CPLX && SEG % kBlock == 0 && SEG % 64 == 0), "paired tiles: f64 on fused records");
    constexpr int FAR = CPLX ? kChainFarC : kChainFar;
    constexpr R kNone = ~(R)0;
    constexpr int hb = kChainLdsPairs;
    X const *__restrict__ x = (X const *)x_v;
    X *__restrict__ y = (X *)y_v;
    const bool extra_stream = kAblate && (n_cached & 0x100);
    const int nt_from = !kAblate ? 99 : ((n_cached & 0x200) ? 20 : ((n_cached & 0x400) ? 0 : 99));
    if (kAblate) n_cached &= 0xff;
    uint64_t ex_next = 0;
    extern __shared__ uint4 s_img[];
    R const *const s_binom = reinterpret_cast<R const *>(s_img);
    uint2 const *const s_near = reinterpret_cast<uint2 const *>(reinterpret_cast<char const *>(s_img) + near_off);
    __shared__ X s_x[WINDOW + 1];
    for (int k = threadIdx.x; k < img16; k += kBlock) s_img[k] = g_img[k];
    (void)NB;
    if (threadIdx.x == 0) s_x[WINDOW] = cx_zero<X>();
    const int xcd = blockIdx.x & 7;
    const int64_t blocks_per_xcd = gridDim.x >> 3;
    const int lane = threadIdx.x & 63;
    tilemap += (int64_t)xcd * slots_per_xcd;
    uint32_t const *__restrict__ reps32 = reinterpret_cast<uint32_t const *>(reps);
    constexpr bool HDR = REC || (CPLX && sizeof(W) == 4 && sizeof(R) == 4);
    constexpr int NSUB = TILE / kBlock;
    for (int64_t t = blockIdx.x >> 3; t < slots_per_xcd; t += blocks_per_xcd) {
        const uint64_t slot = tilemap[t];
        const int cnt_slot = REC ? (int)((slot >> 48) & 0x7ffu) : (int)(slot >> 48);
        if (cnt_slot == 0) continue;
        const int cnt = PAIR ? TILE : cnt_slot;
        const int64_t i0 = (int64_t)(slot & 0xffffffffffffULL);
        const int64_t w0 = (row0 + i0 - HALO) & ~(int64_t)1;
        const int64_t w0b = PAIR ? (i0 + pr.d - HALO) & ~(int64_t)1 : 0;
        auto row_off = [&](int s) -> int { return PAIR ? (s >> 1) * (int)pr.d + (s & 1) * kBlock + (int)threadIdx.x : s * kBlock + threadIdx.x; };
        W a_next = 0;
        R t0_next = kNone, t1_next = kNone;
        auto load_row = [&](int64_t row, W &a_out, R &t0_out, R &t1_out) {
            if (REC) {
                const uint64_t rec = __builtin_nontemporal_load(reps + row);
                a_out = (W)(uint32_t)rec;
                t0_out = (R)(uint32_t)(rec >> 32);
            } else {
                if (sizeof(W) == 4) a_out = (W)__builtin_nontemporal_load(reps32 + 2 * row);
                else a_out = (W)__builtin_nontemporal_load(reps + row);
                if (n_cached > 0) t0_out = __builtin_nontemporal_load(cache + row);
            }
            if (n_cached > 1) t1_out = __builtin_nontemporal_load(cache + (size_t)n + (size_t)row);
            if (kAblate && extra_stream) ex_next = __builtin_nontemporal_load(reps + (row < (n >> 1) ? row + (n >> 1) : row - (n >> 1)));
        };
        const int wave0 = (int)(threadIdx.x & ~63u);
        uint32_t hq = ~0u;
        if (PAIR) {
            const uint32_t s = (uint32_t)lane % NSUB;
            const uint32_t wr = (threadIdx.x >> 6) + (s & 1u) * (kBlock / 64);
            const uint32_t word = ((uint32_t)lane / NSUB) % 2;
            hq = (s >> 1) ? pr.hdr_b[2 * ((uint32_t)((i0 - pr.a0) >> 6) + wr) + word] : wave_plan[kChainWords + 2 * ((uint32_t)(i0 >> 6) + wr) + word];
        } else if (HDR && !(REC && (slot >> 63))) {
            const uint32_t hw = 2 * (uint32_t)(i0 >> 6) + 2 * ((threadIdx.x >> 6) + (uint32_t)(lane % NSUB) * (kBlock / 64)) + (lane / NSUB) % 2;
            if (((int64_t)(hw >> 1) << 6) < n) hq = wave_plan[kChainWords + hw];
        }
        auto fetch_row = [&](int s, int64_t row) {
            if (HDR) {
                const uint32_t ti = (uint32_t)__builtin_amdgcn_readlane((int)hq, s) & (kChainWords - 1u);
                if (ti != kChainWords - 1u) { a_next = (W)wave_plan[ti + lane]; return; }
            }
            load_row(row, a_next, t0_next, t1_next);
        };
        if (wave0 < cnt) {
            const int64_t rr = i0 + ((int)threadIdx.x < cnt ? (int)threadIdx.x : cnt - 1);
            fetch_row(0, rr);
        }
        __syncthreads();
        if (CPLX) {
            for (int j = threadIdx.x; j < WINDOW; j += kBlock) {
                const int64_t row = w0 + j;
                s_x[j] = (row >= 0 && row < n_x) ? x[row] : cx_zero<X>();
            }
        } else {
            double const *xd = (double const *)x_v;
            double *sd = (double *)s_x;
            for (int j = 2 * threadIdx.x; j < WINDOW; j += 2 * kBlock) {
                const int64_t row = (PAIR && j >= WSEG) ? w0b + (j - WSEG) : w0 + j;
                double2 v;
                if (row >= 0 && row + 1 < n_x) v = *reinterpret_cast<double2 const *>(xd + row);
                else { v.x = (row >= 0 && row < n_x) ? xd[row] : 0.0; v.y = (row + 1 >= 0 && row + 1 < n_x) ? xd[row + 1] : 0.0; }
                sd[j] = v.x;
                sd[j + 1] = v.y;
            }
        }
        __syncthreads();
        const int own0 = (int)(row0 + i0 - w0);
        const int own0b = PAIR ? WSEG + (int)(i0 + pr.d - w0b) : 0;
        X y_pending = cx_zero<X>();
        int r_pending = -1;
#pragma unroll 1
        for (int sub = 0; sub < TILE / kBlock; ++sub) {
            const int r = row_off(sub);
            if (r_pending >= 0) cx_store_nt(y + i0 + r_pending, y_pending);
            r_pending = -1;
            W a = a_next;
            R t0 = t0_next;
            const R t1 = t1_next;
            const uint64_t ex = ex_next;
            if (PAIR) {
                if (sub + 1 < TILE / kBlock) fetch_row(sub + 1, i0 + row_off(sub + 1));
            } else if (sub + 1 < TILE / kBlock && (sub + 1) * kBlock + wave0 < cnt) {
                const int64_t in = i0 + (r + kBlock < cnt ? r + kBlock : cnt - 1);
                fetch_row(sub + 1, in);
            }
            if (!PAIR && sub * kBlock + wave0 >= cnt) continue;
            const bool ghost = !PAIR && r >= cnt;
            const int64_t i = i0 + (ghost ? cnt - 1 : r);
            const R ig = (R)(row0 + i);
            W a0;
            int ubit;
            const uint32_t h0 = HDR ? (uint32_t)__builtin_amdgcn_readlane((int)hq, sub) : ~0u;
            if (HDR && (h0 & (kChainWords - 1u)) != kChainWords - 1u) {
                const uint32_t word = (uint32_t)a;
                a0 = (W)(h0 & ~(kChainWords - 1u));
                a = a0 | (W)(word & (kChainWords - 1u));
                ubit = 0;
                const uint32_t h1 = (uint32_t)__builtin_amdgcn_readlane((int)hq, NSUB + sub);
                t0 = (int32_t)(word ^ h1) < 0 ? (R)((h1 & 0x7fffffffu) + ((word >> 16) & 0x7fffu)) : kNone;
            } else {
                a0 = readfirstlane_t<W>(a);
                const W adiff = a0 ^ readlane_t<W>(a, 63);
                ubit = adiff == 0 ? 0 : (int)(8 * sizeof(W)) - (sizeof(W) == 4 ? __clz((int)(uint32_t)adiff) : __clzll((long long)(uint64_t)adiff));
            }
            const int jl = PAIR ? (sub & 1) * kBlock + (int)threadIdx.x : 0;
            const int jr = PAIR ? ((sub >> 1) ? own0b : own0) + jl : own0 + (int)(i - i0);
            const int jp = PAIR ? ((sub >> 1) ? own0 : own0b) + jl : 0;
            const X xr = s_x[jr];
            X g0 = n_cached > 0 ? xr : cx_zero<X>(), g1 = n_cached > 1 ? xr : cx_zero<X>();
            if (t0 != kNone) g0 = x[t0];
            if (n_cached > 1 && t1 != kNone) g1 = x[t1];
            double dr, di;
            diag_coeff<W, true>(runs, n_diag, diag, a, dr, di);
            X acc = cx_scale(dr, xr);
            const W tdiff = a ^ (a >> 1);
            const R ig0 = readfirstlane_t<R>(ig);
            const uint32_t dl = (uint32_t)(ig - ig0);
            for (int q = 0; q < runs.n_runs; ++q) {
                const int lo0 = runs.lo0[q];
                int lo_end = lo0 + runs.cnt[q];
                const double vr = runs.v_re[q];
                const bool top_here = PAIR && lo0 <= pr.bond && pr.bond < lo_end;
                int k = WT::popc(a & (W)(((uint64_t)1 << lo0) - 1));
                int lo = lo0;
                const int e1 = lo_end < LDSP ? lo_end : LDSP;
                const int near_end = lo0 > e1 ? lo0 : e1;
                int split = hb == 0 ? lo_end : (hb < near_end ? near_end : (hb > lo_end ? lo_end : hb));
                if (hb != 0 && split < ubit) split = ubit < lo_end ? ubit : lo_end;
                const bool uni = split < lo_end;
                unsigned long long m = 0;
                R off = 0;
                X xv[FAR];
#pragma unroll
                for (int u = 0; u < FAR; ++u) xv[u] = cx_zero<X>();
                if (uni) {
                    const int p = split + lane;
                    const bool in_run = p < lo_end;
                    const int ps = in_run ? p : 0;
                    const W hi = a0 >> ps;
                    const bool bit = hi & 1;
                    const bool act = in_run && (((hi >> 1) & 1) != (W)bit) && !(PAIR && p == pr.bond);
                    const int kk = hamming_weight - WT::popc(hi);
                    const R d = s_binom[ps * kc + (kk < 0 ? 0 : kk)];
                    off = bit ? d : (R)(0 - d);
                    m = __builtin_amdgcn_ballot_w64(act);
#pragma unroll
                    for (int u = 0; u < FAR; ++u) {
                        if (m) {
                            const int l = __builtin_ctzll(m);
                            m &= m - 1;
                            X const *const src = x + (size_t)(R)(ig0 + readlane_t<R>(off, l)) + dl;
                            if (kAblate && split + l >= nt_from) xv[u] = cx_load_nt(src); else xv[u] = *src;
                        }
                    }
                    lo_end = split;
                }
                if (lo0 == 0 && e1 == LDSP) {
                    const uint32_t al = (uint32_t)a;
                    const uint32_t jb = (uint32_t)jr * (uint32_t)sizeof(X);
                    constexpr uint32_t ZOFF = (uint32_t)WINDOW * (uint32_t)sizeof(X);
                    char const *const sb = reinterpret_cast<char const *>(s_x);
                    const uint2 q0 = s_near[al & 31u];
                    const uint2 q1 = s_near[32 + 32 * __popc(al & 15u) + ((al >> 4) & 31u)];
                    const uint2 q2 = s_near[192 + 32 * __popc(al & 255u) + ((al >> 8) & 31u)];
                    const uint32_t wq[6] = {q0.x, q0.y, q1.x, q1.y, q2.x, q2.y};
                    constexpr int NBATCH = 2;
#pragma unroll
                    for (int p0 = 0; p0 < LDSP; p0 += NBATCH) {
                        X nv[NBATCH];
#pragma unroll
                        for (int u = 0; u < NBATCH; ++u) {
                            const int p = p0 + u;
                            const uint32_t w = wq[(p < LDSP ? p : 0) >> 1];
                            const int32_t d = (p & 1) ? ((int32_t)w >> 16) : (int32_t)(int16_t)(w & 0xffffu);
                            uint32_t o = jb + (uint32_t)d;
                            o = o < ZOFF ? o : ZOFF;
                            nv[u] = p < LDSP ? *reinterpret_cast<X const *>(sb + o) : cx_zero<X>();
                        }
#pragma unroll
                        for (int u = 0; u < NBATCH; ++u)
                            if (p0 + u < LDSP) cx_fma(vr, nv[u], acc);
                    }
                    lo = LDSP;
                    k = __popc(al & ((1u << LDSP) - 1u));
                }
#pragma unroll 4
                for (; lo < e1; ++lo) {
                    const bool bit = (a >> lo) & 1;
                    const bool act = (tdiff >> lo) & 1;
                    const int d = (int)s_binom[lo * kc + k];
                    k += bit ? 1 : 0;
                    const int j = bit ? jr + d : jr - d;
                    cx_fma(vr, s_x[act ? j : WINDOW], acc);
                }
                if (PAIR && lo == LDSP && lo < lo_end) {
                    const bool bit = (a >> LDSP) & 1;
                    const bool act = (tdiff >> LDSP) & 1;
                    const int d = (int)s_binom[LDSP * kc + k];
                    const int j = bit ? jr + d : jr - d;
                    const int sb = (sub >> 1) * WSEG;
                    if (__builtin_amdgcn_ballot_w64(act && (j < sb || j >= sb + WSEG)) == 0)
                        cx_fma(vr, s_x[act ? j : WINDOW], acc);
                    else {
                        const R idx = act ? (bit ? (R)(ig + (R)d) : (R)(ig - (R)d)) : ig;
                        cx_fma(act ? vr : 0.0, x[idx], acc);
                    }
                    k += bit ? 1 : 0;
                    ++lo;
                }
#pragma unroll
                for (int u = 0; u < FAR; ++u) cx_fma(vr, xv[u], acc);
                while (m) {
                    X xw[4];
#pragma unroll
                    for (int u = 0; u < 4; ++u) {
                        xw[u] = cx_zero<X>();
                        if (m) {
                            const int l = __builtin_ctzll(m);
                            m &= m - 1;
                            xw[u] = (x + (size_t)(R)(ig0 + readlane_t<R>(off, l)))[dl];
                        }
                    }
#pragma unroll
                    for (int u = 0; u < 4; ++u) cx_fma(vr, xw[u], acc);
                }
                if (top_here) cx_fma(vr, s_x[jp], acc);
#pragma unroll 4
                for (; lo < lo_end; ++lo) {
                    const bool bit = (a >> lo) & 1;
                    const bool act = (tdiff >> lo) & 1;
                    const R d = s_binom[lo * kc + k];
                    k += bit ? 1 : 0;
                    R idx = bit ? (R)(ig + d) : (R)(ig - d);
                    idx = act ? idx : ig;
                    cx_fma(act ? vr : 0.0, x[idx], acc);
                }
            }
            cx_fma(t0 != kNone ? cv0 : 0.0, g0, acc);
            cx_fma(t1 != kNone ? cv1 : 0.0, g1, acc);
            if (kAblate && extra_stream && ex == 0x0123456789abcdefULL) cx_fma(1.0, xr, acc);
            y_pending = acc;
            r_pending = ghost ? -1 : r;
        }
        if (r_pending >= 0) cx_store_nt(y + i0 + r_pending, y_pending);
    }
}
template <typename W, typename R, bool CPLX, int TILE, bool REC>
__global__ __launch_bounds__(kBlock, (CPLX || sizeof(R) == 8 ? 5 : (sizeof(W) == 8 ? 6 : 7))) void k_chain_t(lsk_runs runs, int n_diag, lsk_term const *__restrict__ diag,
                                                    int hamming_weight, uint4 const *__restrict__ g_img, int img16, int kc,
                                                    int near_off,
                                                    uint64_t const *__restrict__ tilemap, int64_t slots_per_xcd, int64_t n,
                                                    uint64_t const *__restrict__ reps, void const *__restrict__ x_v,
                                                    void *__restrict__ y_v, int n_cached,
                                                    R const *__restrict__ cache, double cv0, double cv1, int64_t row0,
                                                    int64_t n_x, uint32_t const *__restrict__ wave_plan) {
    chain_rows<W, R, CPLX, TILE, REC, false>(runs, n_diag, diag, hamming_weight, g_img, img16, kc, near_off, tilemap, slots_per_xcd, n, reps, x_v, y_v,
                                             n_cached, cache, cv0, cv1, row0, n_x, wave_plan, chain_pair_args{0, 0, nullptr, -1});
}
__global__ __launch_bounds__(kBlock, 7) void k_chain_pair_t(lsk_runs runs, int n_diag, lsk_term const *__restrict__ diag, int hamming_weight,
                                                            uint4 const *__restrict__ g_img, int img16, int kc, int near_off,
                                                            uint64_t const *__restrict__ tilemap, int64_t slots_per_xcd, int64_t n,
                                                            uint64_t const *__restrict__ reps, void const *__restrict__ x_v,
                                                            void *__restrict__ y_v, int n_cached, double cv0, chain_pair_args pr,
                                                            uint32_t const *__restrict__ wave_plan) {
    chain_rows<uint32_t, uint32_t, false, 1024, true, true>(runs, n_diag, diag, hamming_weight, g_img, img16, kc, near_off, tilemap, slots_per_xcd, n,
                                                            reps, x_v, y_v, n_cached, nullptr, cv0, 0.0, 0, n, wave_plan, pr);
}

template <typename W, typename R>
__global__ __launch_bounds__(kBlock) void k_chain_cache(int64_t n, uint64_t const *__restrict__ reps, uint64_t xmask, uint64_t inv_mask,
                                                        int hamming_weight, uint64_t const *__restrict__ g_binom,
                                                        R *__restrict__ out, int *__restrict__ flag) {
    constexpr int NB = ChainTraits<W, R>::NB;
    __shared__ R s_binom[NB * LSK_BINOM_K];
    for (int k = threadIdx.x; k < NB * LSK_BINOM_K; k += blockDim.x) s_binom[k] = (R)g_binom[k];
    __syncthreads();
    for (int64_t i = (int64_t)blockIdx.x * kBlock + threadIdx.x; i < n; i += (int64_t)gridDim.x * kBlock) {
        const W a = (W)reps[i];
        R t = ~(R)0;
        if (WordTraits<W>::popc(a & (W)xmask) == 1) {
            W beta = a ^ (W)xmask;
            if (inv_mask) { const W f = beta ^ (W)inv_mask; beta = f < beta ? f : beta; }
            if (WordTraits<W>::popc(beta) != hamming_weight) atomicExch(flag, 1);
            else t = (R)rank_combinadic_w<W, R>(beta, s_binom);
        }
        out[i] = t;
    }
}
extern "C" int lsk_chain_cache(lsk_basis bs, lsk_index ix, int64_t n, uint64_t const *reps, uint64_t xmask, void *out,
                               int wide_ranks, int *d_flag, void *stream) {
    if (n == 0) return 0;
    dim3 g(grid_for(n)), b(kBlock);
    hipStream_t s = (hipStream_t)stream;
    const uint64_t inv_mask = bs.proj == LSK_PROJ_INVERSION ? bs.site_mask : 0;
    if (bs.number_sites <= 32 && !wide_ranks)
        hipLaunchKernelGGL((k_chain_cache<uint32_t, uint32_t>), g, b, 0, s, n, reps, xmask, inv_mask, bs.hamming_weight, ix.binom, (uint32_t *)out, d_flag);
    else if (!wide_ranks)
        hipLaunchKernelGGL((k_chain_cache<uint64_t, uint32_t>), g, b, 0, s, n, reps, xmask, inv_mask, bs.hamming_weight, ix.binom, (uint32_t *)out, d_flag);
    else
        hipLaunchKernelGGL((k_chain_cache<uint64_t, uint64_t>), g, b, 0, s, n, reps, xmask, inv_mask, bs.hamming_weight, ix.binom, (uint64_t *)out, d_flag);
    LSK_LAUNCH_CHECK();
    return 0;
}

__global__ __launch_bounds__(kBlock) void k_chain_pack(int64_t n, uint64_t const *__restrict__ reps,
                                                       uint32_t const *__restrict__ cache, uint64_t *__restrict__ out) {
    for (int64_t i = (int64_t)blockIdx.x * kBlock + threadIdx.x; i < n; i += (int64_t)gridDim.x * kBlock)
        out[i] = (uint64_t)(uint32_t)reps[i] | ((uint64_t)(cache ? cache[i] : 0xffffffffu) << 32);
}
extern "C" int lsk_chain_pack(int64_t n, uint64_t const *reps, void const *cache, uint64_t *out, void *stream) {
    if (n == 0) return 0;
    hipLaunchKernelGGL(k_chain_pack, dim3(grid_for(n)), dim3(kBlock), 0, (hipStream_t)stream, n, reps, (uint32_t const *)cache, out);
    LSK_LAUNCH_CHECK();
    return 0;
}

__global__ __launch_bounds__(kBlock) void k_chain_headers(int64_t n, uint64_t const *__restrict__ reps, int hamming_weight, int high_site,
                                                          uint64_t const *__restrict__ g_binom, uint2 *__restrict__ out,
                                                          unsigned long long *__restrict__ n_plain) {
    const int64_t n_hdr = (n + 63) >> 6;
    for (int64_t w = (int64_t)blockIdx.x * kBlock + threadIdx.x; w < n_hdr; w += (int64_t)gridDim.x * kBlock) {
        uint2 h = make_uint2(~0u, ~0u);
        const uint32_t first = (uint32_t)reps[w << 6];
        if ((w << 6) + 63 < n && ((first ^ (uint32_t)reps[(w << 6) + 63]) >> 12) == 0) {
            const uint32_t high = first & ~(kChainWords - 1u), low = first & (kChainWords - 1u);
            const int kl = __popc(low);
            uint32_t ti = (uint32_t)rank_combinadic_w<uint32_t, uint64_t>(low, g_binom);
            for (int k = 0; k < kl; ++k) ti += (uint32_t)g_binom[12 * LSK_BINOM_K + k];
            uint32_t base = 0;
            if (high_site >= 0) {
                const uint32_t hbit = (high >> high_site) & 1u;
                const int kp = hbit ? kl + 1 : kl - 1;
                if (kp >= 0 && kp <= 12 && kp <= hamming_weight)
                    base = (uint32_t)rank_combinadic_w<uint32_t, uint64_t>((high ^ (1u << high_site)) | ((1u << kp) - 1u), g_binom);
                base |= hbit << 31;
            }
            h = make_uint2(high | ti, base);
        } else
            atomicAdd(n_plain, 1ULL);
        out[w] = h;
    }
}
extern "C" int lsk_chain_headers(lsk_basis bs, lsk_index ix, int64_t n, uint64_t const *reps, int headed, int high_site, void *out,
                                 unsigned long long *d_n_plain, void *stream) {
    if (n == 0) return 0;
    if (!headed) {
        if (hipMemsetAsync(out, 0xff, 8 * (size_t)((n + 63) >> 6), (hipStream_t)stream) != hipSuccess) { snprintf(g_err, sizeof(g_err), "lsk_chain_headers: memset failed"); return -1; }
        return 0;
    }
    if (bs.number_sites > 32 || bs.number_sites < 13 || bs.hamming_weight < 0 || high_site >= bs.number_sites || (high_site >= 0 && high_site < 12)) {
        snprintf(g_err, sizeof(g_err), "lsk_chain_headers: plan out of range");
        return -1;
    }
    hipLaunchKernelGGL(k_chain_headers, dim3(grid_for((n + 63) >> 6)), dim3(kBlock), 0, (hipStream_t)stream, n, reps, bs.hamming_weight,
                       high_site, ix.binom, (uint2 *)out, d_n_plain);
    LSK_LAUNCH_CHECK();
    return 0;
}
extern "C" int lsk_chain_words(void) { return (int)kChainWords; }

__global__ void k_binom_narrow(uint64_t const *__restrict__ in, uint32_t *__restrict__ out, int n) {
    for (int k = blockIdx.x * blockDim.x + threadIdx.x; k < n; k += gridDim.x * blockDim.x) out[k] = (uint32_t)in[k];
}
template <typename R> static R const *chain_binom(uint64_t const *g_binom, hipStream_t stream);
template <> uint64_t const *chain_binom<uint64_t>(uint64_t const *g_binom, hipStream_t) { return g_binom; }
template <> uint32_t const *chain_binom<uint32_t>(uint64_t const *g_binom, hipStream_t stream) {
    static uint64_t const *src = nullptr;
    static uint32_t *narrow = nullptr;
    static std::mutex lock;
    std::lock_guard<std::mutex> guard(lock);
    if (src != g_binom || !narrow) {
        if (!narrow && hipMalloc((void **)&narrow, sizeof(uint32_t) * 64 * LSK_BINOM_K) != hipSuccess) return nullptr;
        hipLaunchKernelGGL(k_binom_narrow, dim3(4), dim3(kBlock), 0, stream, g_binom, narrow, 64 * LSK_BINOM_K);
        src = g_binom;
    }
    return narrow;
}

static int chain_near_fill(uint64_t const (*C)[LSK_BINOM_K], int elem, int ldsp, int16_t *near) {
    int const base[3] = {0, 32, 192};
    for (int g = 0; g < 3; ++g)
        for (int kidx = 0; kidx <= 4 * g; ++kidx)
            for (int pat = 0; pat < 32; ++pat)
                for (int p = 0; p < 4; ++p) {
                    int const lo = 4 * g + p;
                    int const bit = (pat >> p) & 1, nxt = (pat >> (p + 1)) & 1;
                    int const k = kidx + __builtin_popcount(pat & ((1 << p) - 1));
                    int64_t const d = (int64_t)C[lo][k < LSK_BINOM_K ? k : 0] * elem;
                    int16_t v = 0x7000;
                    if (lo < ldsp && bit != nxt && k <= lo) {
                        if (d >= 0x7000) { snprintf(g_err, sizeof(g_err), "chain_near_fill: displacement out of range"); return -1; }
                        v = (int16_t)(bit ? d : -d);
                    }
                    near[4 * (base[g] + 32 * kidx + pat) + p] = v;
                }
    return 0;
}
static void chain_binomials(uint64_t (*C)[LSK_BINOM_K]) {
    for (int n = 0; n < 64; ++n)
        for (int k = 0; k < LSK_BINOM_K; ++k) C[n][k] = k == 0 ? 1 : (n == 0 ? 0 : C[n - 1][k - 1] + C[n - 1][k]);
}
extern "C" int lsk_test_chain_near_table(int elem, int ldsp, int16_t *out) {
    uint64_t C[64][LSK_BINOM_K];
    chain_binomials(C);
    return chain_near_fill(C, elem, ldsp, out);
}
struct ChainImage { int rsize, rows, kc, elem, ldsp, device; uint4 *dev; int bytes, near_off; };
static int chain_lds_image(int rsize, int rows, int weight, int elem, int ldsp, ChainImage *out) {
    static std::vector<ChainImage> cache;
    static std::mutex lock;
    std::lock_guard<std::mutex> guard(lock);
    int kc = (weight < 0 ? rows : weight) + 2;
    if (kc > LSK_BINOM_K) kc = LSK_BINOM_K;
    int device = 0;
    if (hipGetDevice(&device) != hipSuccess) device = 0;
    for (ChainImage const &c : cache)
        if (c.rsize == rsize && c.rows == rows && c.kc == kc && c.elem == elem && c.ldsp == ldsp && c.device == device) { *out = c; return 0; }
    uint64_t C[64][LSK_BINOM_K];
    chain_binomials(C);
    int const near_off = (rows * kc * rsize + 15) & ~15;
    int const bytes = near_off + 480 * 8;
    std::vector<unsigned char> img((size_t)bytes, 0);
    for (int n = 0; n < rows; ++n)
        for (int k = 0; k < kc; ++k) {
            if (rsize == 4) reinterpret_cast<uint32_t *>(img.data())[n * kc + k] = (uint32_t)C[n][k];
            else reinterpret_cast<uint64_t *>(img.data())[n * kc + k] = C[n][k];
        }
    if (chain_near_fill(C, elem, ldsp, reinterpret_cast<int16_t *>(img.data() + near_off)) != 0) return -1;
    ChainImage c = {rsize, rows, kc, elem, ldsp, device, nullptr, bytes, near_off};
    if (hipMalloc((void **)&c.dev, (size_t)bytes) != hipSuccess) { snprintf(g_err, sizeof(g_err), "chain_lds_image: no device memory"); return -1; }
    if (hipMemcpy(c.dev, img.data(), (size_t)bytes, hipMemcpyHostToDevice) != hipSuccess) { (void)hipFree(c.dev); snprintf(g_err, sizeof(g_err), "chain_lds_image: copy failed"); return -1; }
    cache.push_back(c);
    *out = c;
    return 0;
}

template <typename W, typename R, bool CPLX, int TILE, bool REC>
static int launch_chain(lsk_operator op, lsk_basis bs, lsk_index ix, lsk_tilemap tm, int64_t n, uint64_t const *reps,
                        int64_t row0, int64_t n_x, void const *x, void *y, int n_cached, void const *cache, double cv0,
                        double cv1, void const *wave_plan, void *stream) {
    int64_t gb = tm.slots_per_xcd * 8;
    ChainImage img;
    if (chain_lds_image((int)sizeof(R), ChainTraits<W, R>::NB, bs.hamming_weight, CPLX ? 16 : 8, CPLX ? 11 : kChainLdsPairs, &img) != 0) return -1;
    hipLaunchKernelGGL((k_chain_t<W, R, CPLX, TILE, REC>), dim3((unsigned)gb), dim3(kBlock), (size_t)img.bytes, (hipStream_t)stream, op.runs,
                       op.n_diag, op.diag, bs.hamming_weight, img.dev, img.bytes / 16, img.kc, img.near_off, tm.entries, tm.slots_per_xcd, n, reps, x, y,
                       n_cached | ((kAblate && (bs.debug_ablate & 128)) ? 0x100 : 0) | ((kAblate && (bs.debug_ablate & 4096)) ? 0x200 : 0) |
                           ((kAblate && (bs.debug_ablate & 8192)) ? 0x400 : 0), (R const *)cache, cv0, cv1, row0, n_x,
                       (uint32_t const *)wave_plan);
    LSK_LAUNCH_CHECK();
    return 0;
}

extern "C" int lsk_chain_tile_rows(int cplx) { return cplx ? 512 : 1024; }

extern "C" int lsk_chain(lsk_operator op, lsk_basis bs, lsk_index ix, int cplx, int wide_ranks, int fused_records, lsk_tilemap tm,
                         int64_t n, uint64_t const *reps, int64_t row0, int64_t n_x, void const *x, void *y, int n_cached,
                         void const *cache, double cv0, double cv1, void const *wave_plan, void *stream) {
    if (n == 0 || tm.slots_per_xcd == 0) return 0;
    const bool narrow = bs.number_sites <= 32 && !wide_ranks;
    if ((wave_plan != nullptr) != narrow) { snprintf(g_err, sizeof(g_err), "lsk_chain: 32-bit states and ranks come with wave headers, the other plans without"); return -1; }
#define LSK_CHAIN_ARGS op, bs, ix, tm, n, reps, row0, n_x, x, y, n_cached, cache, cv0, cv1, wave_plan, stream
    if (fused_records) {
        if (!narrow || cplx) { snprintf(g_err, sizeof(g_err), "lsk_chain: fused records need 32-bit states and ranks and f64 vectors"); return -1; }
        return launch_chain<uint32_t, uint32_t, false, 1024, true>(LSK_CHAIN_ARGS);
    }
    if (narrow) {
        if (!cplx) { snprintf(g_err, sizeof(g_err), "lsk_chain: 32-bit states and ranks with f64 vectors run on fused records (lsk_chain_pack)"); return -1; }
        return launch_chain<uint32_t, uint32_t, true, 512, false>(LSK_CHAIN_ARGS);
    }
    if (!wide_ranks) return cplx ? launch_chain<uint64_t, uint32_t, true, 512, false>(LSK_CHAIN_ARGS) : launch_chain<uint64_t, uint32_t, false, 1024, false>(LSK_CHAIN_ARGS);
    return cplx ? launch_chain<uint64_t, uint64_t, true, 512, false>(LSK_CHAIN_ARGS) : launch_chain<uint64_t, uint64_t, false, 1024, false>(LSK_CHAIN_ARGS);
#undef LSK_CHAIN_ARGS
}
extern "C" int lsk_chain_paired(lsk_operator op, lsk_basis bs, lsk_tilemap tm_pair, int64_t n, uint64_t const *records, void const *x, void *y,
                                int n_cached, double cv0, void const *wave_plan, int64_t d, int64_t a0, void const *hdr_b, int bond, void *stream) {
    if (n == 0 || tm_pair.slots_per_xcd == 0) return 0;
    if (bs.number_sites < 14 || bs.number_sites > 32 || bond != bs.number_sites - 2 || n_cached > 1 || !wave_plan || !hdr_b || !tm_pair.entries ||
        d < 512 || (a0 & 511) || a0 + d + 512 > n) {
        snprintf(g_err, sizeof(g_err), "lsk_chain_paired: plan out of range");
        return -1;
    }
    ChainImage img;
    if (chain_lds_image(4, ChainTraits<uint32_t, uint32_t>::NB, bs.hamming_weight, 8, 11, &img) != 0) return -1;
    chain_pair_args pr = {d, a0, (uint32_t const *)hdr_b, bond};
    hipLaunchKernelGGL(k_chain_pair_t, dim3((unsigned)(tm_pair.slots_per_xcd * 8)), dim3(kBlock), (size_t)img.bytes, (hipStream_t)stream, op.runs,
                       op.n_diag, op.diag, bs.hamming_weight, img.dev, img.bytes / 16, img.kc, img.near_off, tm_pair.entries,
                       tm_pair.slots_per_xcd, n, records, x, y, n_cached, cv0, pr, (uint32_t const *)wave_plan);
    LSK_LAUNCH_CHECK();
    return 0;
}

constexpr int kPairLowBits = 11;
constexpr int kPairHalo = 512;
constexpr int kPairFar = 8;
enum { PAIR_NEAR = 0, PAIR_STRADDLE = 1, PAIR_HIGH = 2 };

template <typename SW, bool CPLX, int TILE>
__global__ __launch_bounds__(kBlock, (CPLX ? 4 : 6)) void k_pairs_t(lsk_pairplan pp, int hamming_weight, uint64_t const *__restrict__ tilemap,
                                                              int64_t slots_per_xcd, int64_t n, void const *__restrict__ x_v,
                                                              void *__restrict__ y_v) {
    typedef typename ChainX<CPLX>::type X;
    constexpr int HALO = kPairHalo;
    constexpr int WINDOW = TILE + 2 * HALO + 2;
    constexpr int LOWMASK = (1 << kPairLowBits) - 1;
    X const *__restrict__ x = (X const *)x_v;
    X *__restrict__ y = (X *)y_v;
    __shared__ X s_x[WINDOW + 1];
    __shared__ uint16_t s_rl[1 << kPairLowBits];
    constexpr int NBITS = 8 * (int)sizeof(SW);
    constexpr SW ONE = (SW)1;
    auto popc = [](SW v) { return sizeof(SW) == 4 ? __popc((uint32_t)v) : __popcll((uint64_t)v); };
    auto ctz = [](SW v) { return sizeof(SW) == 4 ? __builtin_ctz((uint32_t)v) : __builtin_ctzll((uint64_t)v); };
    SW const *__restrict__ states = (SW const *)pp.states;
    __shared__ uint32_t s_binom[NBITS * LSK_PAIR_KC];
    __shared__ lsk_pair s_pairs[LSK_MAX_PAIRS];
    const int n_near = pp.n_near, n_str = pp.n_str, n_high = pp.n_high;
    const int kc = LSK_PAIR_KC;
    for (int k = threadIdx.x; k < (1 << kPairLowBits); k += kBlock) s_rl[k] = pp.rank_low[k];
    for (int k = threadIdx.x; k < NBITS * kc; k += kBlock) s_binom[k] = pp.binom[k];
    for (int k = threadIdx.x; k < n_near + n_str + n_high; k += kBlock) s_pairs[k] = pp.pairs[k];
    if (threadIdx.x == 0) s_x[WINDOW] = cx_zero<X>();
    const int xcd = blockIdx.x & 7;
    const int64_t blocks_per_xcd = gridDim.x >> 3;
    const int lane = threadIdx.x & 63;
    tilemap += (int64_t)xcd * slots_per_xcd;
    for (int64_t t = blockIdx.x >> 3; t < slots_per_xcd; t += blocks_per_xcd) {
        const uint64_t slot = tilemap[t];
        const int cnt = (int)(slot >> 48);
        if (cnt == 0) continue;
        const int64_t i0 = (int64_t)(slot & 0xffffffffffffULL);
        const int64_t w0 = (i0 - HALO) & ~(int64_t)1;
        __syncthreads();
        if (CPLX) {
            for (int j = threadIdx.x; j < WINDOW; j += kBlock) {
                const int64_t row = w0 + j;
                s_x[j] = (row >= 0 && row < n) ? x[row] : cx_zero<X>();
            }
        } else {
            double const *xd = (double const *)x_v;
            double *sd = (double *)s_x;
            for (int j = 2 * threadIdx.x; j < WINDOW; j += 2 * kBlock) {
                const int64_t row = w0 + j;
                double2 v;
                if (row >= 0 && row + 1 < n) v = *reinterpret_cast<double2 const *>(xd + row);
                else { v.x = (row >= 0 && row < n) ? xd[row] : 0.0; v.y = (row + 1 >= 0 && row + 1 < n) ? xd[row + 1] : 0.0; }
                sd[j] = v.x;
                sd[j + 1] = v.y;
            }
        }
        __syncthreads();
        const int own0 = (int)(i0 - w0);
        const int wave0 = (int)(threadIdx.x & ~63u);
#pragma unroll 1
        for (int sub = 0; sub < TILE / kBlock; ++sub) {
            if (sub * kBlock + wave0 >= cnt) break;
            const int r = sub * kBlock + threadIdx.x;
            const bool ghost = r >= cnt;
            const int64_t i = i0 + (ghost ? cnt - 1 : r);
            const SW a = __builtin_nontemporal_load(states + i);
            const uint32_t ig = (uint32_t)i;
            const uint32_t low = (uint32_t)a & LOWMASK;
            const SW hi = a >> kPairLowBits;
            const int jr = own0 + (int)(i - i0);
            const X xr = s_x[jr];
            X acc = cx_zero<X>();
            double dsub = 0.0;
            const int rl0 = (int)s_rl[low];
            for (int p = 0; p < n_near; ++p) {
                lsk_pair const P = s_pairs[p];
                const uint32_t m = (1u << P.i) | (1u << P.j);
                const bool act = __popc(low & m) == 1;
                const int r1 = (int)s_rl[low ^ m];
                const int o = jr + (r1 - rl0);
                cx_fma(P.v, s_x[act ? o : WINDOW], acc);
                dsub += act ? P.vz : 0.0;
            }
            unsigned long long pending = __builtin_amdgcn_ballot_w64(true);
            while (pending) {
                const int l0 = __builtin_ctzll(pending);
                const SW href = readlane_t<SW>(hi, l0);
                const bool inseg = hi == href;
                pending &= ~__builtin_amdgcn_ballot_w64(inseg);
                const int kl = hamming_weight - popc(href);
                double dz_u = 0.0;
                for (int pass = 0; pass < n_high; pass += 64) {
                    const int q = pass + lane;
                    const bool in = q < n_high;
                    lsk_pair const P = s_pairs[n_near + n_str + (in ? q : 0)];
                    const int pi = P.i - kPairLowBits, pj = P.j - kPairLowBits;
                    const uint32_t bi = (uint32_t)(href >> pi) & 1u, bj = (uint32_t)(href >> pj) & 1u;
                    const bool act = in && bi != bj;
                    int k = kl + popc(href & ((ONE << pi) - ONE));
                    SW between = href & ((ONE << pj) - ONE) & ~(((SW)2 << pi) - ONE);
                    int64_t lowcfg = (int64_t)s_binom[P.i * kc + min(k + 1, kc - 1)], highcfg = 0;
                    int tt = 0;
                    while (between) {
                        const int b = ctz(between) + kPairLowBits;
                        between &= between - ONE;
                        ++tt;
                        lowcfg += (int64_t)s_binom[b * kc + min(k + 1 + tt, kc - 1)];
                        highcfg += (int64_t)s_binom[b * kc + min(k + tt, kc - 1)];
                    }
                    highcfg += (int64_t)s_binom[P.j * kc + min(k + tt + 1, kc - 1)];
                    const int32_t delta = (int32_t)(bi ? highcfg - lowcfg : lowcfg - highcfg);
                    unsigned long long m = __builtin_amdgcn_ballot_w64(act);
                    while (m) {
                        X xv[kPairFar];
                        double vv[kPairFar];
#pragma unroll
                        for (int u = 0; u < kPairFar; ++u) {
                            xv[u] = cx_zero<X>();
                            vv[u] = 0.0;
                            if (m) {
                                const int l = __builtin_ctzll(m);
                                m &= m - 1;
                                const int32_t d = __builtin_amdgcn_readlane(delta, l);
                                vv[u] = readlane_f64(P.v, l);
                                dz_u += readlane_f64(P.vz, l);
                                xv[u] = x[inseg ? (uint32_t)(ig + (uint32_t)d) : ig];
                            }
                        }
#pragma unroll
                        for (int u = 0; u < kPairFar; ++u) cx_fma(inseg ? vv[u] : 0.0, xv[u], acc);
                    }
                }
                for (int pass = 0; pass < n_str; pass += 64) {
                    const int q = pass + lane;
                    const bool in = q < n_str;
                    lsk_pair const P = s_pairs[n_near + (in ? q : 0)];
                    const int pj = P.j - kPairLowBits;
                    const uint32_t bj = (uint32_t)(href >> pj) & 1u;
                    const SW h2 = href ^ (ONE << pj);
                    const int kl2 = bj ? kl + 1 : kl - 1;
                    uint32_t base = 0;
                    {
                        SW hb = h2;
                        int idx = kl2;
                        while (hb) {
                            const int b = ctz(hb) + kPairLowBits;
                            hb &= hb - ONE;
// ... 316 lines not shown
```

distributed-matvec_amd/csrc/lsk.h:

```cpp
#ifndef LSK_H
#define LSK_H

#include <stddef.h>
#include <stdint.h>

#ifdef __cplusplus
extern "C" {
#endif

#define LSK_BENES_STAGES 11
#define LSK_BINOM_K 34
#define LSK_MAX_PARTS 256

typedef struct lsk_term {
    double v_re, v_im;
    uint64_t m, r, s;
} lsk_term;

enum { LSK_GROUP_GENERIC = 0, LSK_GROUP_EXCHANGE = 1,
       LSK_GROUP_HOP_LO = 2, LSK_GROUP_HOP_HI = 3 };

typedef struct lsk_group {
    uint64_t x;
    double v_re, v_im;
// ... 13 lines not shown
} lsk_runs;

typedef struct lsk_operator {
    int n_diag, n_off, n_groups, is_real;
    int uni;
    double uni_v;
    lsk_term const *diag;
    lsk_term const *off;
    lsk_group const *groups;
    lsk_runs runs;
} lsk_operator;

enum { LSK_ELEM_BENES = 0, LSK_ELEM_ROT = 1, LSK_ELEM_REVROT = 2 };
enum { LSK_ELEM_LIFT = 4, LSK_ELEM_LIFT_REV = 1, LSK_ELEM_LIFT_SWAP = 2 };

typedef struct lsk_group_elem {
    int32_t kind;
    int32_t k;
    double ch_re, ch_im;
    uint64_t masks[LSK_BENES_STAGES];
} lsk_group_elem;

enum { LSK_PROJ_NONE = 0, LSK_PROJ_INVERSION = 1, LSK_PROJ_FULL = 2 };

typedef struct lsk_basis {
    int number_sites, hamming_weight, spin_inversion, n_elems, proj;
    int chars_pm1;
    int k4_mode, reflect;
    int d4_mask;
    int fermi;
    union {
        uint64_t const *trow2;
        uint64_t const *fsign;
    };
    int tw, n_cosets;
    uint64_t tcol0;
    lsk_group_elem const *cosets;
    uint32_t const *trow;
    int debug_ablate;
    uint64_t site_mask;
    double inv_order;
    lsk_group_elem const *elems;
} lsk_basis;

enum { LSK_INDEX_IDENTITY = 0, LSK_INDEX_COMBINADIC = 1, LSK_INDEX_SEARCH = 2, LSK_INDEX_PRODUCT = 3 };

typedef struct lsk_rankdir {
    uint64_t bits;
    uint32_t prefix;
    uint32_t pad;
} lsk_rankdir;

typedef struct lsk_index {
    int kind;
    int shift;
    int64_t count;
    uint64_t const *reps;
    uint32_t const *table;
    uint64_t const *binom;
    lsk_rankdir const *dir;
    int dir_sites, dir_weight;
    int prod_sites, prod_up, prod_dn;
    int64_t prod_na;
} lsk_index;
int lsk_rankdir_build(int64_t n, uint64_t const *reps, int sites, int weight, uint64_t const *d_binom, int64_t entries, lsk_rankdir *dir,
                      int *d_flag, void *stream);

typedef struct lsk_gdir {
    lsk_rankdir const *entries;
    int P, sites, weight;
    int64_t n_ranks;
} lsk_gdir;
int lsk_gdir_build(lsk_gdir gd, lsk_rankdir *entries, uint64_t const *d_binom, void *stream);
int lsk_gdir_check(lsk_gdir gd, int part, int64_t n, uint64_t const *reps, uint64_t const *d_binom, int *d_flag, void *stream);

#define LSK_MAX_SEGS 64
typedef struct lsk_segs {
    int n;
    int64_t start[LSK_MAX_SEGS + 1];
    int64_t key_off[LSK_MAX_SEGS];
    int64_t val_off[LSK_MAX_SEGS];
    void *y[LSK_MAX_SEGS];
    uint8_t part[LSK_MAX_SEGS];
} lsk_segs;
typedef struct lsk_gtab {
    uint64_t const *entries;
    int L, bbits, tbits;
} lsk_gtab;
typedef struct lsk_part_ctx {
    lsk_index ix;
    double const *norms;
    lsk_gtab gt;
} lsk_part_ctx;
int lsk_scatter_idx(int cplx, lsk_segs const *segs, void const *base, void *stream);
int lsk_scatter_parts(lsk_part_ctx const *d_parts, lsk_index any, int cplx, lsk_segs const *segs, void const *base, int *d_err, void *stream);
int lsk_scatter_segs(lsk_index ix, lsk_gtab gt, int cplx, lsk_segs const *segs, void const *base, double const *norms, int *d_err, void *stream);

typedef struct lsk_round_layout {
    int64_t beta_off[LSK_MAX_PARTS];
    int64_t val_off[LSK_MAX_PARTS];
} lsk_round_layout;

typedef struct lsk_tilemap {
    uint64_t const *entries;
    int64_t slots_per_xcd;
} lsk_tilemap;

char const *lsk_last_error(void);
int lsk_ablate_mask(void);
int lsk_device_count(void);
int lsk_set_device(int device);
int lsk_malloc(void **p, size_t bytes);
int lsk_free(void *p);
int lsk_mem_info(size_t *free_bytes, size_t *total_bytes);
int lsk_h2d(void *dst, void const *src, size_t bytes);
int lsk_d2h(void *dst, void const *src, size_t bytes);
int lsk_d2d_async(void *dst, void const *src, size_t bytes, void *stream);
int lsk_memset_async(void *p, int value, size_t bytes, void *stream);
int lsk_sync(void *stream);
int lsk_device_sync(void);
int lsk_copy_strided(int64_t n, int elt_size, void const *src, int64_t src_stride, void *dst, int64_t dst_stride, void *stream);

enum { LSK_PTR_PAGEABLE = 0, LSK_PTR_PINNED = 1, LSK_PTR_DEVICE = 2,
       LSK_PTR_MANAGED = 3  };
char const *lsk_stage_last_error(void);
int lsk_pointer_kind(void const *p);
int lsk_host_register(void *p, size_t bytes);
int lsk_host_unregister(void *p);
typedef struct lsk_stager lsk_stager;
int lsk_stager_create(lsk_stager **out, size_t chunk_bytes, int threads );
void lsk_stager_destroy(lsk_stager *st);
int lsk_stager_threads(lsk_stager const *st);
size_t lsk_stager_chunk(lsk_stager const *st);
int lsk_stage_run(lsk_stager *st, void *d_up, void const *h_up, size_t up_bytes, int up_kind, void *h_down, void const *d_down,
                  size_t down_bytes, int down_kind);

int lsk_event_create(void **ev);
int lsk_event_destroy(void *ev);
int lsk_event_record(void *ev, void *stream);
int lsk_event_elapsed_ms(void *start, void *stop, float *ms);

int lsk_fill_random(int64_t n, uint64_t const *states, uint64_t seed, int cplx, void *out, void *stream);

int lsk_diag(lsk_operator op, int cplx, int64_t n, uint64_t const *reps, void const *x, void *y,
             void *stream);
int lsk_direct_validate(lsk_operator op, lsk_basis bs, lsk_index ix, int64_t n, uint64_t const *reps, int *d_err, void *stream);
int lsk_direct(lsk_operator op, lsk_basis bs, lsk_index ix, int cplx, int pull, lsk_tilemap tm,
               uint64_t const *reps, void const *x, void *y, int *d_err, void *stream);
int lsk_chain_tile_rows(int cplx);
int lsk_chain(lsk_operator op, lsk_basis bs, lsk_index ix, int cplx, int wide_ranks, int fused_records, lsk_tilemap tm,
              int64_t n, uint64_t const *reps, int64_t row0, int64_t n_x, void const *x, void *y, int n_cached,
              void const *cache, double cv0, double cv1, void const *wave_plan, void *stream);
int lsk_chain_paired(lsk_operator op, lsk_basis bs, lsk_tilemap tm_pair, int64_t n, uint64_t const *records, void const *x, void *y,
                     int n_cached, double cv0, void const *wave_plan, int64_t d, int64_t a0, void const *hdr_b, int bond, void *stream);
#define LSK_MAX_PAIRS 128
#define LSK_PAIR_KC 20
typedef struct lsk_pair {
    uint8_t i, j, pad[6];
    double v;
    double vz;
} lsk_pair;
typedef struct lsk_pair_row {
    uint64_t between;
    double v, vz;
    int i, j;
} lsk_pair_row;
#define LSK_PAIR_SITE_MAX_DEGREE 8
#define LSK_PAIR_SITE_MAX_CLASSES 64
typedef struct lsk_pairplan {
    int n_near, n_str, n_high;
    lsk_pair const *pairs;
    uint16_t const *rank_low;
    uint32_t const *binom;
    void const *states;
    int wide;
    double dsum;
    lsk_pair_row const *rows;
    uint32_t const *sites;
    int n_sites, degree;
    int n_classes, site_words;
} lsk_pairplan;
int lsk_push_tile_rows(int cplx);
int lsk_push_staged(lsk_operator op, lsk_basis bs, lsk_index ix, int cplx, lsk_tilemap tm, int64_t n, uint64_t const *reps,
                    void const *x, void *y, int *d_err, void *stream);
int lsk_pairs_tile_rows(int cplx);
int lsk_pairs(lsk_pairplan pp, int hamming_weight, int cplx, lsk_tilemap tm, int64_t n, void const *x, void *y, void *stream);
typedef struct lsk_species {
    int64_t n;
    int deg;
    uint32_t const *words;
    uint32_t const *rank;
    double const *coef;
} lsk_species;
typedef struct lsk_hubbard {
    int L, cplx_coef;
    lsk_species up, dn;
} lsk_hubbard;
int lsk_hubbard_apply(lsk_hubbard hb, lsk_operator op, int cplx, lsk_tilemap tm, void const *x, void *y, void *stream);
int lsk_narrow_states(int64_t n, uint64_t const *reps, uint32_t *out, void *stream);

int lsk_chain_pack(int64_t n, uint64_t const *reps, void const *cache, uint64_t *out, void *stream);
int lsk_chain_headers(lsk_basis bs, lsk_index ix, int64_t n, uint64_t const *reps, int headed, int high_site, void *out,
                      unsigned long long *d_n_plain, void *stream);
int lsk_chain_words(void);
int lsk_chain_cache(lsk_basis bs, lsk_index ix, int64_t n, uint64_t const *reps, uint64_t xmask, void *out, int wide_ranks,
                    int *d_flag, void *stream);
int lsk_tile(lsk_operator op, lsk_basis bs, lsk_index ix, int cplx, int count_only, int P, int me,
             int64_t row0, int64_t row1, uint64_t const *reps, double const *norms, void const *x,
             void *y, unsigned long long *d_cursors, lsk_round_layout const *d_layout, void *d_send,
             unsigned long long *d_counts, int *d_err, void *stream);
int lsk_tile_wv_max_parts(void);
int lsk_tile_wv(lsk_operator op, lsk_basis bs, lsk_index ix, lsk_gdir gd, int cplx, int count_only, int P, int me,
                int64_t row0, int64_t row1, uint64_t const *reps, double const *norms, void const *x, void *y,
                uint32_t *d_wtab, lsk_round_layout const *d_layout, void *d_send, int *d_err, lsk_gtab own_gt, void *stream);
int lsk_tile_st_max_classes(void);
int lsk_tile_st(lsk_operator op, lsk_gdir gd, uint64_t const *d_binom, int cplx, int count_only, int P, int S, int tile_rows,
                int64_t row0, int64_t row1, uint64_t const *reps, void const *x, uint32_t *d_ttab,
                lsk_round_layout const *d_layout, void *d_send, int *d_err, void *stream);
typedef struct lsk_wsrc {
    uint32_t const *keys;
    double const *vals;
    uint32_t const *soff;
} lsk_wsrc;
typedef struct lsk_wdests {
    int n;
    int64_t count[LSK_MAX_SEGS];
    int64_t first_block[LSK_MAX_SEGS + 1];
    void *y[LSK_MAX_SEGS];
    lsk_rankdir const *dir[LSK_MAX_SEGS];
    uint64_t const *reps[LSK_MAX_SEGS];
    uint64_t const *binom;
    int64_t n_ranks;
    int weight;
    int *err;
} lsk_wdests;
int lsk_window_rows(int cplx);
int lsk_window(int cplx, lsk_wdests const *dests, lsk_wsrc const *d_srcs, int n_src, int S, int wpb, void *stream);
int lsk_direct_gx(lsk_operator op, lsk_basis bs, lsk_index ix_global, int cplx, lsk_tilemap tm,
                  uint64_t const *reps, int64_t const *row_gidx, void const *x_global, void *y, int *d_err,
                  void *stream);
int lsk_hash_build(int cplx, int64_t n, uint64_t const *reps, int bits, void *tab, uint32_t *slot_of, void *stream);
int lsk_hash_fill(int cplx, int64_t n, uint32_t const *slot_of, void const *x, double const *norms, void *tab,
                  void *xs , void *stream);
int lsk_tile_pull(lsk_operator op, lsk_basis bs, lsk_index ix_global, int cplx, int64_t row0, int64_t row1,
                  uint64_t const *reps, double const *norms_local, double const *norms_global,
                  int64_t const *row_gidx, void const *tab, int tab_bits, uint64_t const *reps_global,
                  int64_t n_global, void const *xs_global, int halo, void const *x_global, void *y,
                  int *d_err, void *stream);
int lsk_gtab_bits(int L, int64_t n, int64_t max_bytes);
int lsk_gtab_build(lsk_gtab t, uint64_t *entries, int64_t n, uint64_t const *reps, uint32_t const *payload, int *d_flag,
                   void *stream);
int64_t lsk_test_gtab_find(lsk_gtab t, uint64_t const *h_entries, uint64_t key);
int lsk_test_gtab_build_host(lsk_gtab t, uint64_t *h_entries, int64_t n, uint64_t const *reps, uint32_t const *payload);
int lsk_gtab_lookup(lsk_gtab t, int64_t n, uint64_t const *keys, uint32_t *out, void *stream);

typedef struct lsk_pullidx {
    lsk_gtab tab;
    uint32_t const *perm;
    int64_t row_g0;
    uint64_t const *vtab;
} lsk_pullidx;
int lsk_vtab_build(lsk_gtab t, uint64_t *vtab, void *stream);
int lsk_vtab_refresh(lsk_gtab t, uint64_t *vtab, void const *xsrc, void *stream);
int lsk_tile_pull_idx(lsk_operator op, lsk_basis bs, int cplx, int64_t row0, int64_t row1, uint64_t const *reps,
                      double const *norms_local, lsk_pullidx ix, uint64_t const *reps_global, int64_t n_global,
                      void const *xsrc, int halo, void *y, int *d_err, void *stream);
int lsk_pull_max_halo(void);
typedef struct lsk_pullbuf {
    uint32_t *slots;
    uint8_t *rows;
    double *coefs;
    uint32_t *counts;
    int64_t cap, row0;
    int64_t const *offs;
} lsk_pullbuf;
int lsk_tile_pull_stream_offsets(lsk_operator op, lsk_basis bs, int64_t row0, int64_t row1, uint64_t const *reps, int64_t *out,
                                 void *stream);
int64_t lsk_pullbuf_cap(lsk_operator op);
int lsk_pullbuf_coef_doubles(lsk_operator op, lsk_basis bs);
int lsk_tile_pull_resolve(lsk_operator op, lsk_basis bs, int64_t row0, int64_t row1, uint64_t const *reps,
                          double const *norms_local, lsk_pullidx ix, uint64_t const *reps_global, int64_t n_global, int halo,
                          lsk_pullbuf buf, int *d_err, void *stream);
int lsk_tile_pull_gather(lsk_operator op, lsk_basis bs, int cplx, int64_t row0, int64_t row1, uint64_t const *reps,
                         double const *norms_local, lsk_pullidx ix, void const *xsrc, lsk_pullbuf buf, void *y, void *stream);
int lsk_direct_blk(lsk_operator op, lsk_basis bs, lsk_index ix, int cplx, lsk_tilemap tm, uint64_t const *reps, int K,
                   void const *x, int64_t xr, int64_t xc, void *y, int64_t yr, int64_t yc, int *d_err, void *stream);
int lsk_pull_gather_blk(lsk_operator op, lsk_basis bs, int cplx, int64_t row0, int64_t row1, uint64_t const *reps,
                        double const *norms, lsk_pullbuf buf, int K, void const *x, int64_t xr, int64_t xc, void *y,
                        int64_t yr, int64_t yc, void *stream);
int lsk_direct_cheb(lsk_operator op, lsk_basis bs, lsk_index ix, int cplx, lsk_tilemap tm, uint64_t const *reps, int K,
                    void const *x, int64_t xr, int64_t xc, void *y, int64_t yr, int64_t yc, double alpha, double beta, double gamma,
                    double *d_dots, int *d_err, void *stream);
int lsk_pull_gather_cheb(lsk_operator op, lsk_basis bs, int cplx, int64_t row0, int64_t row1, uint64_t const *reps,
                         double const *norms, lsk_pullbuf buf, int K, void const *x, int64_t xr, int64_t xc, void *y,
                         int64_t yr, int64_t yc, double alpha, double beta, double gamma, double *d_dots, void *stream);
int lsk_axpby_dots(int cplx, int64_t n, int K, void const *w, int64_t wr, int64_t wc, void const *x, int64_t xr, int64_t xc,
                   void *y, int64_t yr, int64_t yc, double alpha, double beta, double gamma, double *d_xx, double *d_xy,
                   void *stream);
int lsk_block_gram_blocks(int64_t n, int Ka, int Kb, int cplx);
char const *lsk_block_gram_kernel_name(int mfma);
int lsk_block_gram(int cplx, int64_t n, int Ka, void const *a, int64_t a_row, int64_t a_col, int Kb, int nket, void const *b1,
                   int64_t b1_row, int64_t b1_col, void const *b2, int64_t b2_row, int64_t b2_col, int mfma, double *partial,
                   double *out, void *stream);
int lsk_direct_evolve(lsk_operator op, lsk_basis bs, lsk_index ix, int cplx, lsk_tilemap tm, uint64_t const *reps, int K,
                      void const *x, int64_t xr, int64_t xc, void *y, int64_t yr, int64_t yc, double alpha, double beta, double gamma,
                      void *z, int64_t zr, int64_t zc, int z_cplx, double c_re, double c_im, double *d_dots, int *d_err, void *stream);
int lsk_pull_gather_evolve(lsk_operator op, lsk_basis bs, int cplx, int64_t row0, int64_t row1, uint64_t const *reps,
// ... 242 lines not shown
```

include/ls_amd.h:

```cpp
#ifndef LS_AMD_H
#define LS_AMD_H

#include "ls_hs.h"

#ifdef __cplusplus
extern "C" {
#endif

typedef enum { LS_AMD_F64 = 0, LS_AMD_C128 = 1 } ls_amd_dtype;

typedef enum {
    LS_AMD_MODE_AUTO = 0,
    LS_AMD_MODE_PUSH = 1,
    LS_AMD_MODE_PULL = 2
} ls_amd_mode;

typedef struct ls_amd_plan ls_amd_plan;

char const *ls_amd_last_error(void);
typedef void (*ls_amd_error_handler)(char const *message);
void ls_amd_set_error_handler(ls_amd_error_handler handler);

int ls_amd_device_count(void);
int ls_amd_set_device(int device);
// ... 116 lines not shown
                                   void *d_gram, void *stream);
int ls_amd_matvec_block_axpby_acc(ls_amd_plan *plan, int K, void const *d_x, int64_t x_row, int64_t x_col,
                                  void *d_y, int64_t y_row, int64_t y_col, double alpha, double beta, double gamma,
                                  void *d_z, int64_t z_row, int64_t z_col, int z_cplx, double c_re, double c_im,
                                  double *d_dots, void *stream);
char const *ls_amd_plan_acc_kernel_name(ls_amd_plan const *plan, int K);
int ls_amd_block_axpby_acc(int cplx, int z_cplx, int64_t n, int K, void const *d_w, int64_t w_row, int64_t w_col, void const *d_x,
                           int64_t x_row, int64_t x_col, void *d_y, int64_t y_row, int64_t y_col, void *d_z, int64_t z_row,
                           int64_t z_col, double alpha, double beta, double gamma, double c_re, double c_im, double *d_dots,
                           void *stream);
int ls_amd_matvec_block_series(ls_amd_plan *plan, int K, int N, double const *coeffs, double lo, double hi,
                               void const *d_x, int64_t x_row, int64_t x_col, void *d_z, int64_t z_row, int64_t z_col, int z_cplx,
                               void *d_work, void *stream);
char const *ls_amd_plan_series_kernel_name(ls_amd_plan const *plan, int K);
int ls_amd_plan_check(ls_amd_plan *plan, void *stream);

int ls_amd_plan_create_replicated(ls_amd_plan **plan, ls_hs_operator const *op, ls_amd_dtype dtype,
                                  int num_partitions, int my_partition, uint64_t const *d_reps_local,
                                  int64_t count_local, uint64_t const *d_reps_global,
                                  int64_t count_global, void *stream);
int ls_amd_matvec_replicated(ls_amd_plan *plan, void const *d_x_global, void *d_y_local, void *stream);

int ls_amd_plan_enable_timing(ls_amd_plan *plan, int max_samples);
#define LS_AMD_NUM_STAGES 7
int ls_amd_plan_enable_stage_timing(ls_amd_plan *plan, int max_events);
int ls_amd_plan_stage_times(ls_amd_plan *plan, double *ms , int64_t *calls , int64_t *matvecs);
int ls_amd_plan_timing_report(ls_amd_plan *plan, char *buf, size_t capacity);
int ls_amd_plan_kernel_times(ls_amd_plan *plan, float *ms, int capacity, int *count);

int ls_amd_fill_random(int64_t n, uint64_t const *d_states, uint64_t seed, ls_amd_dtype dtype,
                       void *d_out, void *stream);

int ls_amd_diag(ls_amd_plan *plan, void const *d_x, void *d_y, void *stream);
int ls_amd_generate(ls_amd_plan *plan, int round, void const *d_x, void *d_y, void *d_send,
                    void *stream);
int ls_amd_scatter(ls_amd_plan *plan, int64_t n, uint64_t const *d_betas, void const *d_values,
                   void *d_y, void *stream);
int ls_amd_plan_key_bytes(ls_amd_plan const *plan);
int64_t ls_amd_plan_segment_bytes(ls_amd_plan const *plan, int64_t count);
int64_t ls_amd_plan_segment_value_offset(ls_amd_plan const *plan, int64_t count);
int64_t ls_amd_plan_packet_index_bytes(ls_amd_plan const *plan);
int ls_amd_scatter_round(ls_amd_plan *plan, int num_segments, int64_t const *counts, int64_t const *offsets,
                         void const *d_recv, void *d_y, void *stream);

int ls_amd_enumerate_states(ls_hs_basis const *basis, int num_locales, uint64_t **d_states,
                            uint8_t **d_masks, int64_t *count, void *stream);
int ls_amd_gather(int64_t n, void const *d_perm, int perm_is_64, int elt_size, void const *d_src, void *d_out, void *stream);
int ls_amd_mask_counts(int64_t n, uint8_t const *d_masks, int num_locales, int64_t *counts,
                       void *stream);
int ls_amd_block_to_hashed(int64_t n, uint8_t const *d_masks, int num_locales, int elt_size,
                           void const *d_src, void *const *d_dest, void *stream);
int ls_amd_hashed_to_block(int64_t n, uint8_t const *d_masks, int num_locales, int elt_size,
                           void const *const *d_src, void *d_dest, void *stream);

typedef struct ls_amd_cross ls_amd_cross;
ls_hs_operator *ls_amd_operator_adjoint(ls_hs_operator const *op);
int ls_amd_operator_maps_sector(ls_hs_operator const *op, ls_hs_basis const *target_basis);
int ls_amd_operator_maps_sector_signed(ls_hs_operator const *op, ls_hs_basis const *target_basis);
int ls_amd_cross_create(ls_amd_cross **out, ls_hs_operator const *op_on_source, ls_hs_basis const *target_basis, ls_amd_dtype dtype,
                        uint64_t const *d_src_reps, int64_t n_src, uint64_t const *d_dst_reps, int64_t n_dst, void *stream);
enum { LS_AMD_CROSS_SAME = 0, LS_AMD_CROSS_RESTRICT = 1, LS_AMD_CROSS_PROJECT = 2 };
int ls_amd_cross_create_groups(ls_amd_cross **out, ls_hs_operator const *op_on_source, ls_hs_basis const *target_basis, ls_amd_dtype dtype,
                               int mode, uint64_t const *d_src_reps, int64_t n_src, uint64_t const *d_dst_reps, int64_t n_dst, void *stream);
int ls_amd_operator_maps_subgroup_sector(ls_hs_operator const *op, ls_hs_basis const *target_basis);
int ls_amd_cross_apply(ls_amd_cross *plan, void const *d_x, void *d_y, void *stream);
int ls_amd_cross_apply_block(ls_amd_cross *plan, int K, void const *d_x, int64_t x_row, int64_t x_col,
                             void *d_y, int64_t y_row, int64_t y_col, void *stream);
char const *ls_amd_cross_block_kernel_name(ls_amd_cross const *plan, int K);
int ls_amd_cross_check(ls_amd_cross *plan, void *stream);
char const *ls_amd_cross_kernel_name(ls_amd_cross const *plan);
int64_t ls_amd_cross_nnz(ls_amd_cross const *plan);
void ls_amd_cross_destroy(ls_amd_cross *plan);

typedef struct ls_amd_csr {
    int64_t rows, cols, nnz;
    ls_amd_dtype dtype;
    int64_t *d_row_ptr, *d_col;
    void *d_val;
} ls_amd_csr;
int64_t ls_amd_cross_csr_bytes(ls_amd_cross const *plan);
int ls_amd_cross_csr(ls_amd_cross *plan, int64_t max_bytes, ls_amd_csr *out, void *stream);
void ls_amd_csr_free(ls_amd_csr *m);

typedef struct ls_amd_expand ls_amd_expand;
int ls_amd_expand_create(ls_amd_expand **out, ls_hs_basis const *basis, uint64_t const *d_reps, int64_t n, uint64_t subsystem_mask,
                         void *stream);
int ls_amd_expand_num_blocks(ls_amd_expand const *plan);
int ls_amd_expand_block(ls_amd_expand const *plan, int i, int *n_a, int64_t *rows, int64_t *cols, int64_t *offset);
int64_t ls_amd_expand_total(ls_amd_expand const *plan);
int ls_amd_expand_apply(ls_amd_expand *plan, ls_amd_dtype dtype, void const *d_psi, void *d_out, int first_block, int num_blocks,
                        void *stream);
int ls_amd_expand_check(ls_amd_expand *plan, void *stream);
char const *ls_amd_expand_kernel_name(ls_amd_expand const *plan);
void ls_amd_expand_destroy(ls_amd_expand *plan);
int ls_amd_test_expand_layout(ls_hs_basis const *basis, uint64_t subsystem_mask, int capacity, int *n_a, int64_t *rows, int64_t *cols,
                              int64_t *offsets, int64_t *total);


int ls_amd_fermi_expand_create(ls_amd_expand **out, ls_hs_basis const *basis, uint64_t const *d_reps, int64_t n, uint64_t mode_mask,
                               void *stream);
int ls_amd_fermi_expand_block(ls_amd_expand const *plan, int i, int *n_up, int *n_dn, int64_t *rows, int64_t *cols, int64_t *offset);
int ls_amd_test_fermi_expand_layout(ls_hs_basis const *basis, uint64_t mode_mask, int capacity, int *n_up, int *n_dn, int64_t *rows,
                                    int64_t *cols, int64_t *offsets, int64_t *total);
int ls_amd_test_fermi_split_parity(uint64_t mode_mask_a, int modes, uint64_t state);

typedef struct ls_amd_project ls_amd_project;
int ls_amd_project_create(ls_amd_project **out, ls_hs_basis const *basis, uint64_t const *d_reps, int64_t n, void *stream);
int64_t ls_amd_project_full_size(ls_amd_project const *plan);
int ls_amd_project_apply(ls_amd_project *plan, ls_amd_dtype dtype, int K, void const *d_phi, int64_t phi_s0, int64_t phi_s1,
                         void *d_out, int64_t out_s0, int64_t out_s1, void *stream);
int ls_amd_project_check(ls_amd_project *plan, void *stream);
char const *ls_amd_project_kernel_name(ls_amd_project const *plan);
void ls_amd_project_destroy(ls_amd_project *plan);
int64_t ls_amd_test_project_full_size(ls_hs_basis const *basis);
int64_t ls_amd_test_project_state_index(ls_hs_basis const *basis, uint64_t state);

typedef struct ls_amd_corr ls_amd_corr;
int ls_amd_corr_create(ls_amd_corr **out, ls_hs_basis const *basis, uint64_t const *d_reps, int64_t n, void *stream);
int ls_amd_corr_modes(ls_amd_corr const *plan);
int ls_amd_corr_densities(ls_amd_corr *plan, ls_amd_dtype dtype, void const *d_psi, double *h_d, double *h_dd, int symmetrize, void *stream);
int ls_amd_corr_hoppings(ls_amd_corr *plan, ls_amd_dtype dtype, void const *d_psi, double *h_g, int symmetrize, void *stream);
char const *ls_amd_corr_kernel_name(ls_amd_corr const *plan, int which);
void ls_amd_corr_destroy(ls_amd_corr *plan);
int ls_amd_test_corr_symmetrize(ls_hs_basis const *basis, int kind, double const *raw, double *out);

typedef struct ls_amd_expect ls_amd_expect;
int ls_amd_expect_create(ls_amd_expect **out, ls_hs_basis const *basis, ls_hs_operator const *const *ops, int n_ops,
                         uint64_t const *d_reps, int64_t n, void *stream);
int ls_amd_expect_values(ls_amd_expect *plan, ls_amd_dtype dtype, void const *d_psi, double *h_out, void *stream);
int ls_amd_expect_num_terms(ls_amd_expect const *plan);
int ls_amd_expect_num_groups(ls_amd_expect const *plan);
char const *ls_amd_expect_kernel_name(ls_amd_expect const *plan);
void ls_amd_expect_destroy(ls_amd_expect *plan);
int ls_amd_expect_values_block(ls_amd_expect *plan, ls_amd_dtype dtype, int K, void const *d_psi, int64_t row_stride, int64_t col_stride,
                               double *h_out, void *stream);
char const *ls_amd_expect_block_kernel_name(ls_amd_expect const *plan, int K);
int ls_amd_expect_matrix_elements(ls_amd_expect *plan, ls_amd_dtype dtype, int Ka, void const *d_bra, int64_t bra_row, int64_t bra_col,
                                  int Kb, void const *d_ket, int64_t ket_row, int64_t ket_col, double *h_out, void *stream);
char const *ls_amd_expect_matrix_kernel_name(ls_amd_expect const *plan, int Ka, int Kb);
int64_t ls_amd_test_expect_average(ls_hs_basis const *basis, ls_hs_operator const *op, int64_t cap, double *v, uint64_t *m, uint64_t *r,
                                   uint64_t *x, uint64_t *s);

int ls_amd_basis_group_order(ls_hs_basis const *basis);
int ls_amd_basis_fermion_signs(ls_hs_basis const *basis);
int ls_amd_test_fermion_sign(ls_hs_basis const *basis, int element, uint64_t state, int table);
int ls_amd_basis_spin_flip(ls_hs_basis const *basis);
int ls_amd_test_group_element_kind(ls_hs_basis const *basis, int element);
uint64_t ls_amd_basis_apply_group_element(ls_hs_basis const *basis, int element, uint64_t state);
int ls_amd_basis_group_character(ls_hs_basis const *basis, int element, double *re, double *im);

int64_t ls_amd_test_tilemap(int64_t n, int tile_rows, int64_t chunk, uint64_t **entries);
int64_t ls_amd_plan_chain_paired_rows(ls_amd_plan const *pl);
int ls_amd_test_tilemap_paired(int L, int weight, int tile_rows, int64_t chunk, uint64_t **rest, uint64_t **pairs, int64_t *out);
void ls_amd_test_free(void *p);
int ls_amd_test_window_find(uint64_t const *reps, int n, uint64_t key);
int ls_amd_test_nw_find(uint64_t const *reps, int n, uint64_t key);
int ls_amd_test_chain_near_table(int elem, int ldsp, int16_t *out);
int ls_amd_test_chain_wave_tables(int low_site, uint16_t *U, uint16_t *Rg, int *class_off);
uint64_t ls_amd_test_rep_trivial_dihedral(uint64_t a, int L, int inv, int reflect);
int ls_amd_bench_k4(int L, int inv, int reflect, int variant, int64_t n, uint64_t const *d_reps, uint64_t *d_out, void *stream);
int ls_amd_test_translation_cosets(ls_hs_basis const *basis, int *n_cosets);
uint64_t ls_amd_test_rep_by_cosets(ls_hs_basis const *basis, uint64_t state);
int ls_amd_test_d4_mask(ls_hs_basis const *basis);
int ls_amd_test_gtab_bits(int L, int64_t n);
int ls_amd_test_gtab_build(int L, int bbits, int64_t n, uint64_t const *reps, uint32_t const *payload, uint64_t **entries);
int64_t ls_amd_test_gtab_find(int L, int bbits, uint64_t const *entries, uint64_t key);
int ls_amd_test_primme_comminfo_offset(void);
int ls_amd_test_primme_sumtype_offset(void);
int ls_amd_test_primme_nlocal_offset(void);
int ls_amd_test_primme_matrix_offset(void);

#ifdef __cplusplus
}
#endif
#endif
```

Baseline: 146.4 matvecs/s.

## Generalize chain pairing to multiple bond levels with per-tile range metadata

Extends the paired-tile chain kernel from a single top-bond row range to several levels of paired ranges (bonds L-2, L-4, ...), two levels by default. Each pair tile now carries its own offset d, header index and bond in a wider tilemap entry. This lets more rows be processed as partner pairs that share staged x windows instead of doing scattered lookups. The cost is larger tilemap entries, an extra load per tile, several header-build launches at setup, and more fragmented plain tiles between ranges.

```diff
diff --git a/distributed-matvec_amd/csrc/host.c b/distributed-matvec_amd/csrc/host.c
--- a/distributed-matvec_amd/csrc/host.c
+++ b/distributed-matvec_amd/csrc/host.c
@@ -1603,10 +1603,10 @@
     int chain_row_bytes;
     int chain_headed;
     int chain_headers_apply;
-    int chain_paired;
+    int chain_paired, chain_pair_levels;
     void *d_tilemap_pair, *d_chain_hdr_b;
     lsk_tilemap tilemap_pair;
-    int64_t chain_pair_d, chain_pair_a0, chain_pair_rows;
+    int64_t chain_pair_rows[8];
     double chain_v[2];
     int64_t chain_row0;
     void *d_htab;
@@ -2092,16 +2092,36 @@
     *slots_out = slots;
     return 0;
 }
-static int chain_pair_range(int L, int k, int64_t *a0, int64_t *a1, int64_t *d) {
+#define CHAIN_MAX_PAIR_LEVELS 6
+#define CHAIN_PAIR_LEVELS_DEFAULT 2
+#define CHAIN_MAX_RANGES 63
+typedef struct { int level, bond; int64_t a0, a1, d, hdr0; } chain_range;
+static int chain_pair_ranges(int L, int k, int levels, uint64_t bonds, chain_range *out) {
     if (L < 14 || L > 32 || k < 1 || k > L - 1) return 0;
     uint64_t C[33][33];
     memset(C, 0, sizeof(C));
     for (int n = 0; n <= 32; ++n) { C[n][0] = 1; for (int j = 1; j <= n; ++j) C[n][j] = C[n - 1][j - 1] + (j <= n - 1 ? C[n - 1][j] : 0); }
-    int64_t const r01 = (int64_t)C[L - 2][k], r10 = (int64_t)C[L - 1][k];
-    *d = r10 - r01;
-    *a0 = (r01 + 511) & ~(int64_t)511;
-    *a1 = r10 & ~(int64_t)511;
-    return *a1 > *a0;
+    if (levels > CHAIN_MAX_PAIR_LEVELS) levels = CHAIN_MAX_PAIR_LEVELS;
+    int nr = 0;
+    int64_t hdr = 0;
+    for (int lv = 1; lv <= levels; ++lv) {
+        int const b = L - 2 * lv;
+        if (b < 12 || !((bonds >> b) & 1)) break;
+        for (int h = 0; h < (1 << (lv - 1)); ++h) {
+            int const m = k - 2 * __builtin_popcount((unsigned)h) - 1;
+            if (m < 0 || m > b) continue;
+            int64_t base = 0;
+            int idx = m + 1;
+            for (int t = 0; t < lv - 1; ++t)
+                if ((h >> t) & 1) { base += (int64_t)C[b + 2 * t + 2][idx + 1] + (int64_t)C[b + 2 * t + 3][idx + 2]; idx += 2; }
+            int64_t const r01 = base + (int64_t)C[b][m + 1], r10 = base + (int64_t)C[b + 1][m + 1];
+            chain_range r = {lv, b, (r01 + 511) & ~(int64_t)511, r10 & ~(int64_t)511, r10 - r01, hdr};
+            if (r.a1 <= r.a0) continue;
+            hdr += (r.a1 - r.a0) / 64;
+            out[nr++] = r;
+        }
+    }
+    return nr;
 }
 #define CHAIN_TILE_PLAIN 0x8000
 static int tilemap_deal(tile_list const *all, int64_t chunk, uint64_t **out, int64_t *slots_out) {
@@ -2124,27 +2144,45 @@
     *slots_out = slots;
     return 0;
 }
-static int tilemap_paired_host(int64_t n, int TILE, int64_t chunk, int64_t a0, int64_t a1, int64_t d, uint64_t **rest, int64_t *rest_slots,
-                               uint64_t **pairs, int64_t *pair_slots) {
+typedef struct { int64_t lo, hi; int id; } chain_span;
+static int chain_span_cmp(void const *pa, void const *pb) {
+    int64_t const a = ((chain_span const *)pa)->lo, b = ((chain_span const *)pb)->lo;
+    return a < b ? -1 : a > b;
+}
+static int tilemap_paired_host(int64_t n, int TILE, int64_t chunk, int64_t pair_chunk, chain_range const *rg, int nr, uint64_t **rest,
+                               int64_t *rest_slots, uint64_t **pairs, int64_t *pair_slots) {
     tile_list all[2];
     memset(all, 0, sizeof(all));
-    int64_t const piece[3][2] = {{0, a0}, {a1, a0 + d}, {a1 + d, n}};
-    int64_t total = 0;
-    for (int p = 0; p < 3; ++p)
-        for (int64_t pos = piece[p][0]; pos < piece[p][1];) {
+    chain_span sp[2 * CHAIN_MAX_RANGES];
+    *rest = *pairs = NULL;
+    if (nr < 1 || nr > CHAIN_MAX_RANGES) return set_error("internal error: %d paired ranges", nr);
+    for (int r = 0; r < nr; ++r) {
+        sp[2 * r] = (chain_span){rg[r].a0, rg[r].a1, r};
+        sp[2 * r + 1] = (chain_span){rg[r].a0 + rg[r].d, rg[r].a1 + rg[r].d, -1};
+    }
+    qsort(sp, (size_t)(2 * nr), sizeof(chain_span), chain_span_cmp);
+    int64_t total = 0, from = 0;
+    int rc = 0;
+    for (int q = 0; q <= 2 * nr && !rc; ++q) {
+        int64_t const to = q < 2 * nr ? sp[q].lo : n;
+        if (to < from || (q < 2 * nr && sp[q].hi > n)) { rc = set_error("internal error: paired ranges overlap"); break; }
+        for (int64_t pos = from; pos < to;) {
             int64_t end = (pos / TILE + 1) * TILE;
             if (pos & 63) end = (pos | 63) + 1;
-            if (end > piece[p][1]) end = piece[p][1];
+            if (end > to) end = to;
             int const plain = (pos & 63) != 0 || ((end & 63) != 0 && end != n);
             tile_push(&all[0], pos, (end - pos) | (plain ? CHAIN_TILE_PLAIN : 0));
             total += end - pos;
             pos = end;
         }
-    for (int64_t i0 = a0; i0 < a1; i0 += 512) { tile_push(&all[1], i0, 1024); total += 1024; }
-    int rc = total == n ? 0 : set_error("internal error: paired tile maps cover %lld of %lld rows", (long long)total, (long long)n);
-    *rest = *pairs = NULL;
+        if (q == 2 * nr) break;
+        if (sp[q].id >= 0)
+            for (int64_t i0 = sp[q].lo; i0 < sp[q].hi; i0 += 512) { tile_push(&all[1], i0 | ((int64_t)sp[q].id << 32), 1024); total += 1024; }
+        from = sp[q].hi;
+    }
+    if (!rc && total != n) rc = set_error("internal error: paired tile maps cover %lld of %lld rows", (long long)total, (long long)n);
     if (!rc) rc = tilemap_deal(&all[0], chunk, rest, rest_slots);
-    if (!rc) rc = tilemap_deal(&all[1], chunk, pairs, pair_slots);
+    if (!rc) rc = tilemap_deal(&all[1], pair_chunk, pairs, pair_slots);
     if (rc) { free(*rest); free(*pairs); *rest = *pairs = NULL; }
     free(all[0].e);
     free(all[1].e);
@@ -2196,13 +2234,34 @@
     return slots;
 }
 int ls_amd_test_tilemap_paired(int L, int weight, int tile_rows, int64_t chunk, uint64_t **rest, uint64_t **pairs, int64_t *out) {
-    int64_t a0, a1, d, n = 1;
+    int64_t n = 1;
+    chain_range r[CHAIN_MAX_RANGES];
     *rest = *pairs = NULL;
-    if (!chain_pair_range(L, weight, &a0, &a1, &d)) return 0;
+    if (chain_pair_ranges(L, weight, 1, ~0ULL, r) != 1) return 0;
     for (int j = 1; j <= weight; ++j) n = n * (L - weight + j) / j;
-    if (tilemap_paired_host(n, tile_rows, chunk, a0, a1, d, rest, &out[4], pairs, &out[5]) != 0) return -1;
-    out[0] = n; out[1] = a0; out[2] = a1; out[3] = d;
+    if (tilemap_paired_host(n, tile_rows, chunk, chunk, r, 1, rest, &out[4], pairs, &out[5]) != 0) return -1;
+    out[0] = n; out[1] = r[0].a0; out[2] = r[0].a1; out[3] = r[0].d;
     return 1;
+}
+int ls_amd_test_tilemap_pair_levels(int L, int weight, int tile_rows, int64_t chunk, int64_t pair_chunk, int levels, uint64_t **rest,
+                                    uint64_t **pairs, int64_t **ranges, int64_t *out) {
+    int64_t n = 1;
+    chain_range r[CHAIN_MAX_RANGES];
+    *rest = *pairs = NULL;
+    *ranges = NULL;
+    int const nr = levels >= 1 ? chain_pair_ranges(L, weight, levels, ~0ULL, r) : 0;
+    if (nr == 0) return 0;
+    for (int j = 1; j <= weight; ++j) n = n * (L - weight + j) / j;
+    int64_t *t = (int64_t *)malloc(sizeof(int64_t) * 6 * (size_t)nr);
+    if (!t) return set_error("out of memory");
+    if (tilemap_paired_host(n, tile_rows, chunk, pair_chunk, r, nr, rest, &out[1], pairs, &out[2]) != 0) { free(t); return -1; }
+    for (int q = 0; q < nr; ++q) {
+        int64_t const row[6] = {r[q].level, r[q].bond, r[q].a0, r[q].a1, r[q].d, r[q].hdr0};
+        memcpy(t + 6 * q, row, sizeof(row));
+    }
+    out[0] = n; out[3] = r[nr - 1].level;
+    *ranges = t;
+    return nr;
 }
 void ls_amd_test_free(void *p) { free(p); }
 int ls_amd_test_gtab_bits(int L, int64_t n) { return lsk_gtab_bits(L, n, (int64_t)1 << 40); }
@@ -2311,26 +2370,50 @@
     if ((e && atoi(e) == 0) || !pl->chain_headers_apply || pl->cplx || !pl->d_chain_rec || pl->chain_cached > 1 || pl->chain_row0 != 0 ||
         pl->n_local != 1 || pl->family != FAMILY_DIRECT_PULL)
         return 0;
-    int top = 0;
+    uint64_t bonds = 0;
     for (int q = 0; q < pl->dop.runs.n_runs; ++q)
-        if (pl->dop.runs.lo0[q] <= L - 2 && L - 2 < pl->dop.runs.lo0[q] + pl->dop.runs.cnt[q]) top = 1;
-    int64_t a0, a1, d;
-    if (!top || !chain_pair_range(L, pl->dbs.hamming_weight, &a0, &a1, &d) || a1 + d > n) return 0;
+        for (int b = pl->dop.runs.lo0[q]; b < pl->dop.runs.lo0[q] + (pl->dop.runs.cnt[q] & 0xffff) && b < 64; ++b) bonds |= 1ULL << b;
+    char const *le = getenv("LS_AMD_CHAIN_PAIR_LEVELS");
+    int levels = le ? atoi(le) : CHAIN_PAIR_LEVELS_DEFAULT;
+    if (levels < 1) levels = 1;
+    chain_range rg[CHAIN_MAX_RANGES];
+    int const nr = chain_pair_ranges(L, pl->dbs.hamming_weight, levels, bonds, rg);
+    if (nr == 0) return 0;
+    for (int r = 0; r < nr; ++r) if (rg[r].a1 + rg[r].d > n || rg[r].d < 512) return 0;
     uint64_t *rest = NULL, *pairs = NULL;
     int64_t rest_slots = 0, pair_slots = 0;
-    char const *ce = getenv("LS_AMD_TILE_CHUNK");
+    char const *ce = getenv("LS_AMD_TILE_CHUNK"), *pe = getenv("LS_AMD_PAIR_TILE_CHUNK");
     int64_t const chunk = ce ? atoll(ce) : 256;
-    if (tilemap_paired_host(n, lsk_chain_tile_rows(0), chunk > 0 ? chunk : 0, a0, a1, d, &rest, &rest_slots, &pairs, &pair_slots) != 0) return -1;
+    int64_t const pair_chunk = pe ? atoll(pe) : chunk;
+    if (tilemap_paired_host(n, lsk_chain_tile_rows(0), chunk > 0 ? chunk : 0, pair_chunk > 0 ? pair_chunk : 0, rg, nr, &rest, &rest_slots, &pairs,
+                            &pair_slots) != 0)
+        return -1;
+    int64_t const n_hdr = rg[nr - 1].hdr0 + (rg[nr - 1].a1 - rg[nr - 1].a0) / 64;
+    size_t const pair_words = 2 * (size_t)(8 * pair_slots);
+    uint64_t *wide = (uint64_t *)calloc(pair_words, sizeof(uint64_t));
+    if (!wide || n_hdr >= (1LL << 27)) { free(wide); free(rest); free(pairs); return wide ? 0 : set_error("out of memory"); }
+    for (size_t q = 0; q < pair_words / 2; ++q) {
+        uint64_t const en = pairs[q];
+        if (!(en >> 48)) continue;
+        chain_range const *r = &rg[(en >> 32) & 0xffff];
+        int64_t const i0 = (int64_t)(en & 0xffffffffULL);
+        wide[2 * q] = en;
+        wide[2 * q + 1] = (uint64_t)r->d | (uint64_t)(r->hdr0 + (i0 - r->a0) / 64) << 32 | (uint64_t)r->bond << 59;
+    }
+    free(pairs);
+    pairs = wide;
     void *d_rest = NULL, *d_pairs = NULL, *d_hdr = NULL;
-    int64_t const n_b = a1 - a0;
     unsigned long long plain = 0;
     int rc = lsk_malloc(&d_rest, sizeof(uint64_t) * (size_t)(8 * rest_slots > 0 ? 8 * rest_slots : 1)) ||
-             lsk_malloc(&d_pairs, sizeof(uint64_t) * (size_t)(8 * pair_slots)) || lsk_malloc(&d_hdr, 8 * (size_t)(n_b / 64) + 8);
+             lsk_malloc(&d_pairs, sizeof(uint64_t) * pair_words) || lsk_malloc(&d_hdr, 8 * (size_t)n_hdr + 8);
     if (!rc) {
-        unsigned long long *d_plain = (unsigned long long *)((char *)d_hdr + 8 * (size_t)(n_b / 64));
-        rc = lsk_h2d(d_rest, rest, sizeof(uint64_t) * (size_t)(8 * rest_slots)) || lsk_h2d(d_pairs, pairs, sizeof(uint64_t) * (size_t)(8 * pair_slots)) ||
-             lsk_h2d(d_plain, &plain, 8) || lsk_chain_headers(pl->dbs, index, n_b, d_reps + a0 + d, pl->chain_headed, hi, d_hdr, d_plain, stream) ||
-             lsk_sync(stream);
+        unsigned long long *d_plain = (unsigned long long *)((char *)d_hdr + 8 * (size_t)n_hdr);
+        rc = lsk_h2d(d_rest, rest, sizeof(uint64_t) * (size_t)(8 * rest_slots)) || lsk_h2d(d_pairs, pairs, sizeof(uint64_t) * pair_words) ||
+             lsk_h2d(d_plain, &plain, 8);
+        for (int r = 0; r < nr && !rc; ++r)
+            rc = lsk_chain_headers(pl->dbs, index, rg[r].a1 - rg[r].a0, d_reps + rg[r].a0 + rg[r].d, pl->chain_headed, hi,
+                                   (char *)d_hdr + 8 * (size_t)rg[r].hdr0, d_plain, stream);
+        if (!rc) rc = lsk_sync(stream);
         if (rc) { free(rest); free(pairs); lsk_free(d_rest); lsk_free(d_pairs); lsk_free(d_hdr); return dev_error(); }
     }
     free(rest);
@@ -2349,9 +2432,9 @@
     pl->tilemap_pair.entries = (uint64_t const *)d_pairs;
     pl->tilemap_pair.slots_per_xcd = pair_slots;
     pl->d_chain_hdr_b = d_hdr;
-    pl->chain_pair_d = d;
-    pl->chain_pair_a0 = a0;
-    pl->chain_pair_rows = 2 * (a1 - a0);
+    memset(pl->chain_pair_rows, 0, sizeof(pl->chain_pair_rows));
+    for (int r = 0; r < nr; ++r) pl->chain_pair_rows[rg[r].level] += 2 * (rg[r].a1 - rg[r].a0);
+    pl->chain_pair_levels = rg[nr - 1].level;
     pl->chain_paired = 1;
     return 0;
 }
@@ -3580,8 +3663,12 @@
     return 8;
 }
 int64_t ls_amd_plan_chain_paired_rows(ls_amd_plan const *pl) {
-    return pl->has_chain && pl->chain_paired ? pl->chain_pair_rows : 0;
-}
+    return pl->has_chain && pl->chain_paired ? pl->chain_pair_rows[1] : 0;
+}
+int64_t ls_amd_plan_chain_paired_rows_at(ls_amd_plan const *pl, int level) {
+    return pl->has_chain && pl->chain_paired && level >= 1 && level <= CHAIN_MAX_PAIR_LEVELS ? pl->chain_pair_rows[level] : 0;
+}
+int ls_amd_plan_chain_pair_levels(ls_amd_plan const *pl) { return pl->has_chain && pl->chain_paired ? pl->chain_pair_levels : 0; }
 int64_t ls_amd_plan_nnz(ls_amd_plan const *pl) { return pl->nnz; }
 int ls_amd_plan_send_counts(ls_amd_plan const *pl, int round, int64_t *counts) {
     if (pl->family != FAMILY_TILE) { for (int d = 0; d < pl->P; ++d) counts[d] = 0; return 0; }
@@ -3849,7 +3936,7 @@
                           pl->d_chain_cache, pl->chain_v[0], pl->chain_v[1], pl->d_chain_wave, stream));
             if (pl->chain_paired)
                 DEV(lsk_chain_paired(pl->dop, pl->dbs, pl->tilemap_pair, ps->count, pl->d_chain_rec, d_x[0], d_y[0], pl->chain_cached, pl->chain_v[0],
-                                     pl->d_chain_wave, pl->chain_pair_d, pl->chain_pair_a0, pl->d_chain_hdr_b, NBITS(pl->op->basis) - 2, stream));
+                                     pl->d_chain_wave, pl->d_chain_hdr_b, stream));
         } else if (pl->has_pairs)
             DEV(lsk_pairs(pl->pairs, pl->dbs.hamming_weight, pl->cplx, pl->tilemap, ps->count, d_x[0], d_y[0], stream));
         else if (pl->has_hubbard)
diff --git a/distributed-matvec_amd/csrc/k_rows.hip b/distributed-matvec_amd/csrc/k_rows.hip
--- a/distributed-matvec_amd/csrc/k_rows.hip
+++ b/distributed-matvec_amd/csrc/k_rows.hip
@@ -569,7 +569,7 @@
 }
 constexpr int kChainFarC = 6;
 
-struct chain_pair_args { int64_t d, a0; uint32_t const *hdr_b; int bond; };
+struct chain_pair_args { uint32_t const *hdr_b; };
 template <typename W, typename R, bool CPLX, int TILE, bool REC, bool PAIR>
 __device__ __forceinline__ void chain_rows(lsk_runs const &runs, int n_diag, lsk_term const *__restrict__ diag,
                                                     int hamming_weight, uint4 const *__restrict__ g_img, int img16, int kc,
@@ -579,6 +579,7 @@
                                                     void *__restrict__ y_v, int n_cached,
                                                     R const *__restrict__ cache, double cv0, double cv1, int64_t row0,
                                                     int64_t n_x, uint32_t const *__restrict__ wave_plan, chain_pair_args const &pr) {
+    uint32_t const *__restrict__ const pair_hdr = pr.hdr_b;
     typedef typename ChainX<CPLX>::type X;
     typedef WordTraits<W> WT;
     constexpr int NB = ChainTraits<W, R>::NB;
@@ -608,18 +609,23 @@
     const int64_t blocks_per_xcd = gridDim.x >> 3;
     const int lane = threadIdx.x & 63;
     tilemap += (int64_t)xcd * slots_per_xcd;
+    if constexpr (PAIR) tilemap += (int64_t)xcd * slots_per_xcd;
     uint32_t const *__restrict__ reps32 = reinterpret_cast<uint32_t const *>(reps);
     constexpr bool HDR = REC || (CPLX && sizeof(W) == 4 && sizeof(R) == 4);
     constexpr int NSUB = TILE / kBlock;
     for (int64_t t = blockIdx.x >> 3; t < slots_per_xcd; t += blocks_per_xcd) {
-        const uint64_t slot = tilemap[t];
+        const uint64_t slot = tilemap[PAIR ? 2 * t : t];
         const int cnt_slot = REC ? (int)((slot >> 48) & 0x7ffu) : (int)(slot >> 48);
         if (cnt_slot == 0) continue;
         const int cnt = PAIR ? TILE : cnt_slot;
-        const int64_t i0 = (int64_t)(slot & 0xffffffffffffULL);
+        const int64_t i0 = (int64_t)(slot & (PAIR ? 0xffffffffULL : 0xffffffffffffULL));
+        const uint64_t slot1 = PAIR ? tilemap[2 * t + 1] : 0;
+        const int64_t pr_d = PAIR ? (int64_t)(uint32_t)slot1 : 0;
+        const uint32_t pr_hdr = PAIR ? (uint32_t)(slot1 >> 32) & 0x7ffffffu : 0u;
+        const int pr_bond = PAIR ? (int)(slot1 >> 59) : -1;
         const int64_t w0 = (row0 + i0 - HALO) & ~(int64_t)1;
-        const int64_t w0b = PAIR ? (i0 + pr.d - HALO) & ~(int64_t)1 : 0;
-        auto row_off = [&](int s) -> int { return PAIR ? (s >> 1) * (int)pr.d + (s & 1) * kBlock + (int)threadIdx.x : s * kBlock + threadIdx.x; };
+        const int64_t w0b = PAIR ? (i0 + pr_d - HALO) & ~(int64_t)1 : 0;
+        auto row_off = [&](int s) -> int { return PAIR ? (s >> 1) * (int)pr_d + (s & 1) * kBlock + (int)threadIdx.x : s * kBlock + threadIdx.x; };
         W a_next = 0;
         R t0_next = kNone, t1_next = kNone;
         auto load_row = [&](int64_t row, W &a_out, R &t0_out, R &t1_out) {
@@ -641,7 +647,8 @@
             const uint32_t s = (uint32_t)lane % NSUB;
             const uint32_t wr = (threadIdx.x >> 6) + (s & 1u) * (kBlock / 64);
             const uint32_t word = ((uint32_t)lane / NSUB) % 2;
-            hq = (s >> 1) ? pr.hdr_b[2 * ((uint32_t)((i0 - pr.a0) >> 6) + wr) + word] : wave_plan[kChainWords + 2 * ((uint32_t)(i0 >> 6) + wr) + word];
+            hq = (s >> 1) ? pair_hdr[2u * (pr_hdr + wr) + word]
+                          : wave_plan[kChainWords + 2 * ((uint32_t)(i0 >> 6) + wr) + word];
         } else if (HDR && !(REC && (slot >> 63))) {
             const uint32_t hw = 2 * (uint32_t)(i0 >> 6) + 2 * ((threadIdx.x >> 6) + (uint32_t)(lane % NSUB) * (kBlock / 64)) + (lane / NSUB) % 2;
             if (((int64_t)(hw >> 1) << 6) < n) hq = wave_plan[kChainWords + hw];
@@ -677,7 +684,7 @@
         }
         __syncthreads();
         const int own0 = (int)(row0 + i0 - w0);
-        const int own0b = PAIR ? WSEG + (int)(i0 + pr.d - w0b) : 0;
+        const int own0b = PAIR ? WSEG + (int)(i0 + pr_d - w0b) : 0;
         X y_pending = cx_zero<X>();
         int r_pending = -1;
 #pragma unroll 1
@@ -731,7 +738,7 @@
                 const int lo0 = runs.lo0[q];
                 int lo_end = lo0 + runs.cnt[q];
                 const double vr = runs.v_re[q];
-                const bool top_here = PAIR && lo0 <= pr.bond && pr.bond < lo_end;
+                const bool bond_here = PAIR && lo0 <= pr_bond && pr_bond < lo_end;
                 int k = WT::popc(a & (W)(((uint64_t)1 << lo0) - 1));
                 int lo = lo0;
                 const int e1 = lo_end < LDSP ? lo_end : LDSP;
@@ -750,7 +757,7 @@
                     const int ps = in_run ? p : 0;
                     const W hi = a0 >> ps;
                     const bool bit = hi & 1;
-                    const bool act = in_run && (((hi >> 1) & 1) != (W)bit) && !(PAIR && p == pr.bond);
+                    const bool act = in_run && (((hi >> 1) & 1) != (W)bit) && !(PAIR && p == pr_bond);
                     const int kk = hamming_weight - WT::popc(hi);
                     const R d = s_binom[ps * kc + (kk < 0 ? 0 : kk)];
                     off = bit ? d : (R)(0 - d);
@@ -835,7 +842,7 @@
 #pragma unroll
                     for (int u = 0; u < 4; ++u) cx_fma(vr, xw[u], acc);
                 }
-                if (top_here) cx_fma(vr, s_x[jp], acc);
+                if (bond_here) cx_fma(vr, s_x[jp], acc);
 #pragma unroll 4
                 for (; lo < lo_end; ++lo) {
                     const bool bit = (a >> lo) & 1;
@@ -866,16 +873,16 @@
                                                     R const *__restrict__ cache, double cv0, double cv1, int64_t row0,
                                                     int64_t n_x, uint32_t const *__restrict__ wave_plan) {
     chain_rows<W, R, CPLX, TILE, REC, false>(runs, n_diag, diag, hamming_weight, g_img, img16, kc, near_off, tilemap, slots_per_xcd, n, reps, x_v, y_v,
-                                             n_cached, cache, cv0, cv1, row0, n_x, wave_plan, chain_pair_args{0, 0, nullptr, -1});
+                                             n_cached, cache, cv0, cv1, row0, n_x, wave_plan, chain_pair_args{nullptr});
 }
 __global__ __launch_bounds__(kBlock, 7) void k_chain_pair_t(lsk_runs runs, int n_diag, lsk_term const *__restrict__ diag, int hamming_weight,
                                                             uint4 const *__restrict__ g_img, int img16, int kc, int near_off,
                                                             uint64_t const *__restrict__ tilemap, int64_t slots_per_xcd, int64_t n,
                                                             uint64_t const *__restrict__ reps, void const *__restrict__ x_v,
-                                                            void *__restrict__ y_v, int n_cached, double cv0, chain_pair_args pr,
+                                                            void *__restrict__ y_v, int n_cached, double cv0, uint32_t const *__restrict__ pair_hdr,
                                                             uint32_t const *__restrict__ wave_plan) {
     chain_rows<uint32_t, uint32_t, false, 1024, true, true>(runs, n_diag, diag, hamming_weight, g_img, img16, kc, near_off, tilemap, slots_per_xcd, n,
-                                                            reps, x_v, y_v, n_cached, nullptr, cv0, 0.0, 0, n, wave_plan, pr);
+                                                            reps, x_v, y_v, n_cached, nullptr, cv0, 0.0, 0, n, wave_plan, chain_pair_args{pair_hdr});
 }
 
 template <typename W, typename R>
@@ -1084,19 +1091,17 @@
 #undef LSK_CHAIN_ARGS
 }
 extern "C" int lsk_chain_paired(lsk_operator op, lsk_basis bs, lsk_tilemap tm_pair, int64_t n, uint64_t const *records, void const *x, void *y,
-                                int n_cached, double cv0, void const *wave_plan, int64_t d, int64_t a0, void const *hdr_b, int bond, void *stream) {
+                                int n_cached, double cv0, void const *wave_plan, void const *hdr_b, void *stream) {
     if (n == 0 || tm_pair.slots_per_xcd == 0) return 0;
-    if (bs.number_sites < 14 || bs.number_sites > 32 || bond != bs.number_sites - 2 || n_cached > 1 || !wave_plan || !hdr_b || !tm_pair.entries ||
-        d < 512 || (a0 & 511) || a0 + d + 512 > n) {
+    if (bs.number_sites < 14 || bs.number_sites > 32 || n_cached > 1 || !wave_plan || !hdr_b || !tm_pair.entries || n >= 0xffffffffLL) {
         snprintf(g_err, sizeof(g_err), "lsk_chain_paired: plan out of range");
         return -1;
     }
     ChainImage img;
     if (chain_lds_image(4, ChainTraits<uint32_t, uint32_t>::NB, bs.hamming_weight, 8, 11, &img) != 0) return -1;
-    chain_pair_args pr = {d, a0, (uint32_t const *)hdr_b, bond};
     hipLaunchKernelGGL(k_chain_pair_t, dim3((unsigned)(tm_pair.slots_per_xcd * 8)), dim3(kBlock), (size_t)img.bytes, (hipStream_t)stream, op.runs,
                        op.n_diag, op.diag, bs.hamming_weight, img.dev, img.bytes / 16, img.kc, img.near_off, tm_pair.entries,
-                       tm_pair.slots_per_xcd, n, records, x, y, n_cached, cv0, pr, (uint32_t const *)wave_plan);
+                       tm_pair.slots_per_xcd, n, records, x, y, n_cached, cv0, (uint32_t const *)hdr_b, (uint32_t const *)wave_plan);
     LSK_LAUNCH_CHECK();
     return 0;
 }
diff --git a/distributed-matvec_amd/csrc/lsk.h b/distributed-matvec_amd/csrc/lsk.h
--- a/distributed-matvec_amd/csrc/lsk.h
+++ b/distributed-matvec_amd/csrc/lsk.h
@@ -189,7 +189,7 @@
               int64_t n, uint64_t const *reps, int64_t row0, int64_t n_x, void const *x, void *y, int n_cached,
               void const *cache, double cv0, double cv1, void const *wave_plan, void *stream);
 int lsk_chain_paired(lsk_operator op, lsk_basis bs, lsk_tilemap tm_pair, int64_t n, uint64_t const *records, void const *x, void *y,
-                     int n_cached, double cv0, void const *wave_plan, int64_t d, int64_t a0, void const *hdr_b, int bond, void *stream);
+                     int n_cached, double cv0, void const *wave_plan, void const *hdr_b, void *stream);
 #define LSK_MAX_PAIRS 128
 #define LSK_PAIR_KC 20
 typedef struct lsk_pair {
diff --git a/include/ls_amd.h b/include/ls_amd.h
--- a/include/ls_amd.h
+++ b/include/ls_amd.h
@@ -292,6 +292,10 @@
 int64_t ls_amd_test_tilemap(int64_t n, int tile_rows, int64_t chunk, uint64_t **entries);
 int64_t ls_amd_plan_chain_paired_rows(ls_amd_plan const *pl);
 int ls_amd_test_tilemap_paired(int L, int weight, int tile_rows, int64_t chunk, uint64_t **rest, uint64_t **pairs, int64_t *out);
+int64_t ls_amd_plan_chain_paired_rows_at(ls_amd_plan const *pl, int level);
+int ls_amd_plan_chain_pair_levels(ls_amd_plan const *pl);
+int ls_amd_test_tilemap_pair_levels(int L, int weight, int tile_rows, int64_t chunk, int64_t pair_chunk, int levels, uint64_t **rest,
+                                    uint64_t **pairs, int64_t **ranges, int64_t *out);
 void ls_amd_test_free(void *p);
 int ls_amd_test_window_find(uint64_t const *reps, int n, uint64_t key);
 int ls_amd_test_nw_find(uint64_t const *reps, int n, uint64_t key);
```

New measurement: 148.0 matvecs/s (median of 6 runs). 1.1% higher.
